# maschad/lodestar

Measured on AMD Instinct MI355X. Metric: BLS signature sets verified/sec (node), higher is better.
Workload: dtype u32; 1 GPU; C4 range-sync segment: 32 epochs = 1024 blocks x 98 sets (95 att k=128, sync k=512, 2 singles), 1M-validator table in HBM; sets=100352, pubkey_refs=12978176, table_validators=1048576, jobs=1024, inflight=3

## Files before the change

### include/bgv.h

```cpp
#ifndef BGV_H
#define BGV_H

#include <stdint.h>
#include <stddef.h>

#ifdef __cplusplus
extern "C" {
#endif

#define BGV_ABI_VERSION 4

enum bgv_status {
  BGV_OK = 0,
  BGV_E_INVALID_ARG = -1,
  BGV_E_HIP = -2,
  BGV_E_NO_DEVICE = -3,
  BGV_E_TABLE_RANGE = -4,
  BGV_E_EMPTY_SET = -5,
  BGV_E_BAD_PUBKEY = -6,
  BGV_E_STATE = -7,
};

enum bgv_set_code {
  BGV_SET_OK = 0,
// ... 123 lines not shown

typedef struct bgv_sm_agg {
  const uint8_t* take;
  const uint8_t* prev_sig96;
  uint8_t* agg_sig96;
  uint32_t* agg_count;
  int32_t* agg_code;
} bgv_sm_agg;
int bgv_verify_same_message_aggregate(bgv_ctx* ctx, const bgv_sm_batch* batch, const bgv_sm_agg* agg, uint8_t* set_valid,
                                      int32_t* set_code, bgv_sm_stats* stats);
int bgv_sm_agg_check(const bgv_sm_batch* batch, const bgv_sm_agg* agg);
int bgv_sm_agg_ms(bgv_ctx* ctx, float* ms);

typedef struct bgv_sma_batch {
  uint32_t n_sets;
  uint32_t n_groups;
  const uint32_t* group_offsets;
  const uint32_t* pk_offsets;
  const uint32_t* pk_indices;
  const uint8_t* raw_pks;
  uint32_t n_raw;
  const uint8_t* msgs;
  const uint8_t* sigs;
  const uint32_t* sig_len;
  const uint64_t* scalars;
  uint32_t on_device;
} bgv_sma_batch;

int bgv_verify_same_message_agg(bgv_ctx* ctx, const bgv_sma_batch* batch, uint8_t* set_valid, int32_t* set_code,
                                bgv_sm_stats* stats);
int bgv_sma_check(const bgv_sma_batch* batch);
int bgv_debug_same_message_agg(bgv_ctx* ctx, const bgv_sma_batch* batch, uint8_t* set_valid, int32_t* set_code,
                               bgv_sm_stats* stats, uint8_t* pk_set96, uint8_t* p_group96, uint8_t* s_group192,
                               uint8_t* h_group192);

#define BGV_MAX_INDEX_LISTS 8
int bgv_index_list_set(bgv_ctx* ctx, uint32_t list_id, const uint32_t* indices , uint32_t n);
int bgv_index_list_len(bgv_ctx* ctx, uint32_t list_id, uint32_t* n);

#define BGV_SRC_EXPLICIT 0xffffffffu
typedef struct bgv_set_src { uint32_t list, off, len, bits_off; } bgv_set_src;
typedef struct bgv_bits_batch {
  uint32_t n_sets, n_jobs;
  const uint32_t* job_offsets;
  const bgv_set_src* src;
  const uint8_t* bits;
  uint32_t bits_len;
  const uint32_t* pk_indices;
  uint32_t n_indices;
  const uint8_t* raw_pks;
  uint32_t n_raw;
  const uint8_t* msgs;
  const uint8_t* sigs;
  const uint32_t* sig_len;
  const uint64_t* scalars;
  uint32_t on_device;
} bgv_bits_batch;
int bgv_verify_bits(bgv_ctx* ctx, const bgv_bits_batch* batch, int32_t* job_result, int32_t* set_code, bgv_stats* stats);
int bgv_bits_check(const bgv_bits_batch* batch, const uint32_t* list_len );
int bgv_debug_bits_expand(bgv_ctx* ctx, const bgv_bits_batch* batch, uint32_t* pk_offsets ,
                          uint32_t* pk_indices, uint32_t cap, uint32_t* total);
int bgv_bits_expand_ms(bgv_ctx* ctx, float* ms);

int bgv_index_list_sums(bgv_ctx* ctx, uint32_t list_id, uint32_t enable);
int bgv_index_list_has_sums(bgv_ctx* ctx, uint32_t list_id, uint32_t* has);
int bgv_index_list_sums_ms(bgv_ctx* ctx, float* ms);
typedef struct bgv_bits_path {
  uint32_t sets_complement, keys_expanded, keys_gathered;
} bgv_bits_path;
int bgv_bits_path_stats(bgv_ctx* ctx, bgv_bits_path* out);
typedef struct bgv_hash_path {
  uint32_t sets, hashes, dedup;
} bgv_hash_path;
int bgv_hash_stats(bgv_ctx* ctx, bgv_hash_path* out);
typedef struct bgv_miller_path {
  uint32_t steps, slice_sets, items;
} bgv_miller_path;
int bgv_miller_path_stats(bgv_ctx* ctx, bgv_miller_path* out);
int bgv_pair_merge(bgv_ctx* ctx, int32_t mode);
typedef struct bgv_pair_path {
  uint32_t sets, pairs, merged, fallback;
} bgv_pair_path;
int bgv_pair_stats(bgv_ctx* ctx, bgv_pair_path* out);
int bgv_debug_pair_classes(bgv_ctx* ctx, const bgv_batch* batch, int32_t* job_result, int32_t* set_code, uint32_t* cls,
                           uint32_t* class_off, uint8_t* p_class96, uint8_t* job_fe, uint8_t* batch_fe);
int bgv_bits_plan(const bgv_bits_batch* batch, const uint32_t* list_len, const uint8_t* list_has_sums,
                  uint8_t* path , uint64_t* keys_gathered);
int bgv_debug_bits_keys(bgv_ctx* ctx, const bgv_bits_batch* batch, uint8_t* pk_agg96, uint8_t* path, int32_t* pk_code);
int bgv_debug_index_list_sums(bgv_ctx* ctx, uint32_t list_id, uint32_t first, uint32_t n, uint8_t* out96);

typedef struct bgv_smb_batch {
  uint32_t n_sets, n_groups;
  const uint32_t* group_offsets;
  const bgv_set_src* src;
  const uint8_t* bits;
  uint32_t bits_len;
  const uint32_t* pk_indices;
  uint32_t n_indices;
  const uint8_t* raw_pks;
  uint32_t n_raw;
  const uint8_t* msgs;
  const uint8_t* sigs;
  const uint32_t* sig_len;
  const uint64_t* scalars;
  uint32_t on_device;
} bgv_smb_batch;
int bgv_verify_same_message_bits(bgv_ctx* ctx, const bgv_smb_batch* batch, uint8_t* set_valid, int32_t* set_code,
                                 bgv_sm_stats* stats);
int bgv_smb_check(const bgv_smb_batch* batch, const uint32_t* list_len );
int bgv_debug_same_message_bits(bgv_ctx* ctx, const bgv_smb_batch* batch, uint8_t* set_valid, int32_t* set_code,
                                bgv_sm_stats* stats, uint8_t* pk_set96, uint8_t* path, uint8_t* p_group96,
                                uint8_t* s_group192, uint8_t* h_group192);

int bgv_partial(bgv_ctx* ctx, const bgv_batch* batch, uint8_t* miller576, int32_t* set_code, int32_t* job_result,
                int32_t* ok_out);
int bgv_partial_finish(bgv_ctx* ctx, int32_t* job_result, bgv_stats* stats);
int bgv_combine_final(bgv_ctx* ctx, const uint8_t* millers576, uint32_t n, int32_t* is_one);

typedef struct bgv_debug {
  uint8_t* sig_aff;
  uint8_t* h_aff;
  uint8_t* pk_agg;
  uint8_t* rpk_aff;
  uint8_t* s_aff;
  uint8_t* pair_fe;
  uint8_t* job_fe;
  uint8_t* batch_fe;
} bgv_debug;
int bgv_debug_stages(bgv_ctx* ctx, const bgv_batch* batch, int32_t* job_result, int32_t* set_code, bgv_debug* out);

int bgv_gen_keys(bgv_ctx* ctx, uint32_t first_index, uint32_t n, uint64_t seed);
int bgv_gen_sign(bgv_ctx* ctx, const bgv_batch* batch, uint8_t* sigs_out192);

#define BGV_FP_OPS_N 13
int bgv_debug_fp_ops(bgv_ctx* ctx, const uint32_t* ab_in, uint32_t n, uint32_t* out);
int bgv_debug_g2_decode(bgv_ctx* ctx, const uint8_t* sigs192, const uint32_t* sig_len, uint32_t n, uint8_t* out192,
                        int32_t* codes);

int bgv_bench_fpmul(bgv_ctx* ctx, uint32_t lanes, uint32_t iters, float* ms);
int bgv_bench_mad(bgv_ctx* ctx, uint32_t lanes, uint32_t iters, float* ms);

#ifdef __cplusplus
}
#endif
#endif
```

### lodestar_amd/csrc/bgv_api.hip

```cpp
#include <sys/random.h>
#include <string.h>
#include <stdio.h>
#include <stdarg.h>
#include <stdlib.h>
#include <atomic>
#include <chrono>
#include <optional>
#include <vector>
#include <string>

#include "bgv_internal.h"
#include "msm_g1.h"
#include "sig_agg.h"
#include "pair_merge.h"
#include "../../include/bgv.h"

using namespace bgv;

static thread_local std::string g_err;

static int fail(int code, const char* fmt, ...) {
  char buf[512];
  va_list ap;
  va_start(ap, fmt);
// ... 56 lines not shown
  uint8_t* pin_in = nullptr;
  uint8_t* pin_out = nullptr;
  size_t pin_in_cap = 0, pin_out_cap = 0;
  hipEvent_t ev_staged = nullptr;
  bool staged_pending = false;
  dbuf<uint8_t> raw_in, gen_out;
  dbuf<g1a> pk_tmp;
  dbuf<int32_t> pk_codes;
  std::vector<int32_t> pk_codes_host;
  std::vector<uint32_t> jo_host;
  uint32_t pk_total = 0;
  bool partial_pending = false;
  dev_batch part_d;
  dev_work part_w;
  dbuf<g1a> pk_agg;
  dbuf<fp12_t> dbg_fe, dbg_f;
  dbuf<uint8_t> dbg_out;
  dbuf<uint64_t> scalars;
  dbuf<g1a> raw_conv;
  dbuf<g2a> sig_aff, h_aff;
  dbuf<uint32_t> sig_inf, flags;
  dbuf<int32_t> sig_code, pk_code, job_code, job_result, set_code;
  dbuf<g1a> rpk_aff;
  dbuf<uint32_t> chunk_off, chunk_set;
  dbuf<g1j> pk_part;
  dbuf<g2j> rsig, q_part;
  dbuf<uint32_t> sig_grp;
  dbuf<fp2_t> lines;
  uint32_t lines_idle = 0;
  dbuf<fp12_t> f_step;
  bgv_miller_path miller_path = {};
  dbuf<fp12_t> f_set, f_job, f_batch, f_tmp, f_part;
  dbuf<uint32_t> set_job, s_inf, item_off, item_job;
  dbuf<g2a> s_aff;
  dbuf<g2j> msm_bucket, msm_win;
  dbuf<uint32_t> msm_mask;
  dbuf<uint32_t> sm_skip, sm_list;
  dbuf<int32_t> sm_zero, sm_seg_code;
  dbuf<g1j> sm_win;
  dbuf<g2a> sm_hg, sm_sg;
  dbuf<g1a> sm_pg;
  dbuf<uint8_t> sm_retry;
  dbuf<g1j> sma_pk;
  dbuf<int32_t> sma_pk_code;
  dbuf<g1a> sma_aff;
  dbuf<g2j> sag_seg;
  dbuf<uint32_t> sag_cnt;
  dbuf<int32_t> sag_code;
  dbuf<uint8_t> sag_out;
  dbuf<uint8_t> sag_valid;
  dbuf<g2a> sag_sig;
  hipEvent_t ev_sag[2] = {};
  bool sag_timed = false;
  uint32_t* idx_list[BGV_MAX_INDEX_LISTS] = {};
  uint32_t idx_list_n[BGV_MAX_INDEX_LISTS] = {};
  dbuf<uint32_t> bits_off, bits_idx;
  g1j* idx_sums[BGV_MAX_INDEX_LISTS] = {};
  float sums_build_ms = 0.f;
  uint32_t idx_list_max[BGV_MAX_INDEX_LISTS] = {};
  dbuf<pk_window> bits_win;
  bool bits_any_sums = false;
  bool bits_on_device = false;
  bgv_bits_path bits_path = {};
  uint32_t bits_n = 0;
  uint32_t bits_extra_chunks = 0;
  hipEvent_t ev_bits[2] = {};
  bool bits_timed = false;
  dbuf<uint32_t> msg_rep, msg_uniq, msg_tab, msg_cnt;
  msg_classes mc = {};
  bgv_hash_path hash_path = {};
  bool hash_pending = false;
  int32_t pair_merge = 0;
  bool pm_entry = false;
  bool pm_call = false;
  dbuf<uint64_t> pm_tab;
  dbuf<uint32_t> pm_slot, pm_slot_idx, pm_off, pm_cls, pm_head, pm_next, pm_job, pm_rep, pm_item_off, pm_item_job;
  dbuf<g1a> pm_p;
  dbuf<int32_t> pm_code;
  dbuf<g2a> pm_h;
  pair_classes pc = {};
  bgv_pair_path pair_path = {};
  bool pair_pending = false;
  bool pair_redo = false;
  dbuf<fp_t> mb_fp;
  dbuf<uint64_t> mb_u64;
};


int bgv_abi_version(void) { return BGV_ABI_VERSION; }
#ifndef BGV_SRC_HASH
#define BGV_SRC_HASH "unhashed"
#endif
const char* bgv_build_id(void) { return BGV_SRC_HASH; }
const char* bgv_last_error(void) { return g_err.c_str(); }

const char* bgv_set_code_name(int code) {
  switch (code) {
    case 0: return "BLST_SUCCESS";
    case 1: return "BLST_BAD_ENCODING";
    case 2: return "BLST_POINT_NOT_ON_CURVE";
    case 3: return "BLST_POINT_NOT_IN_GROUP";
    case 4: return "BLST_AGGR_TYPE_MISMATCH";
    case 5: return "BLST_VERIFY_FAIL";
    case 6: return "BLST_PK_IS_INFINITY";
    case 7: return "BLST_BAD_SCALAR";
    case 8: return "BLST_INVALID_SIZE";
    case 9: return "BGV_INDEX_RANGE";
    case 10: return "EMPTY_SIGNATURE_SET";
    default: return "BGV_UNKNOWN";
  }
}

const char* bgv_stage_name(int stage) {
  static const char* names[ST_COUNT] = {"sig_decode_subgroup", "hash_to_g2",       "pk_gather",
                                        "pk_aggregate_scale",  "sig_scale",        "sig_sum_tree",
                                        "miller_loop",         "miller_loop_jobs", "miller_product_tree",
                                        "batch_product",       "batch_final_exp",  "job_final_exp",
                                        "set_codes"};
  return (stage >= 0 && stage < ST_COUNT) ? names[stage] : "unknown";
}

void bgv_cfg_default(bgv_cfg* cfg) {
  if (!cfg) return;
  memset(cfg, 0, sizeof *cfg);
  cfg->struct_size = sizeof *cfg;
  cfg->split = cfg->miller = cfg->msm = cfg->prefold = cfg->lines = cfg->defer_pct = cfg->timing = cfg->clear_lanes = -1;
  cfg->miller_kv = cfg->hash_dedup = cfg->miller_steps = -1;
  cfg->job_lanes = cfg->pairs = cfg->cu_split = 0;
}

int bgv_open(int device, bgv_ctx** out) { return bgv_open_cfg(device, nullptr, out); }

int bgv_open_cfg(int device, const bgv_cfg* cfg, bgv_ctx** out) {
  if (!out) return fail(BGV_E_INVALID_ARG, "out is NULL");
  *out = nullptr;
  bgv_cfg k;
  bgv_cfg_default(&k);
  if (cfg) {
    if (cfg->struct_size != sizeof k) return fail(BGV_E_INVALID_ARG, "bgv_cfg.struct_size %u, expected %zu", cfg->struct_size, sizeof k);
    k = *cfg;
    auto lanes_ok = [](int v) { return v == 6 || v == 18 || v == 36; };
    if (k.miller != -1 && k.miller != 1 && k.miller != 2 && k.miller != 4 && !lanes_ok(k.miller)) return fail(BGV_E_INVALID_ARG, "bgv_cfg.miller %d", k.miller);
    if (k.job_lanes != 0 && !lanes_ok(k.job_lanes)) return fail(BGV_E_INVALID_ARG, "bgv_cfg.job_lanes %d", k.job_lanes);
    if (k.pairs < 0 || k.pairs == 3 || k.pairs > 4) return fail(BGV_E_INVALID_ARG, "bgv_cfg.pairs %d", k.pairs);
    if (k.msm < -1 || k.msm > 4) return fail(BGV_E_INVALID_ARG, "bgv_cfg.msm %d", k.msm);
    if (k.clear_lanes != -1 && k.clear_lanes != 1 && k.clear_lanes != 3 && k.clear_lanes != 9)
      return fail(BGV_E_INVALID_ARG, "bgv_cfg.clear_lanes %d", k.clear_lanes);
    if (k.miller_kv != -1 && k.miller_kv != 0 && k.miller_kv != 2 && k.miller_kv != 3 && k.miller_kv != 6 && k.miller_kv != 9)
      return fail(BGV_E_INVALID_ARG, "bgv_cfg.miller_kv %d", k.miller_kv);
    if (k.defer_pct < -1 || k.defer_pct > 100) return fail(BGV_E_INVALID_ARG, "bgv_cfg.defer_pct %d", k.defer_pct);
    auto tri_ok = [](int v) { return v >= -1 && v <= 1; };
    if (!tri_ok(k.split)) return fail(BGV_E_INVALID_ARG, "bgv_cfg.split %d", k.split);
    if (!tri_ok(k.prefold)) return fail(BGV_E_INVALID_ARG, "bgv_cfg.prefold %d", k.prefold);
    if (!tri_ok(k.lines)) return fail(BGV_E_INVALID_ARG, "bgv_cfg.lines %d", k.lines);
    if (!tri_ok(k.timing)) return fail(BGV_E_INVALID_ARG, "bgv_cfg.timing %d", k.timing);
    if (!tri_ok(k.hash_dedup)) return fail(BGV_E_INVALID_ARG, "bgv_cfg.hash_dedup %d", k.hash_dedup);
    if (!tri_ok(k.miller_steps)) return fail(BGV_E_INVALID_ARG, "bgv_cfg.miller_steps %d", k.miller_steps);
    if (k.cu_split < -64 || k.cu_split > 64) return fail(BGV_E_INVALID_ARG, "bgv_cfg.cu_split %d (|N| <= 64 CUs)", k.cu_split);
    if (k.pairs >= 2 && k.miller != -1 && k.miller != 1)
      return fail(BGV_E_INVALID_ARG, "bgv_cfg.pairs 2 needs the one-lane Miller loop (miller %d)", k.miller);
  }
  int n = 0;
  if (hipGetDeviceCount(&n) != hipSuccess || n <= 0) return fail(BGV_E_NO_DEVICE, "no HIP device visible");
  if (device < 0 || device >= n) return fail(BGV_E_NO_DEVICE, "device %d out of range (%d devices)", device, n);
  HIPCHK(hipSetDevice(device));
  std::vector<uint32_t> mask;
// ... 15 lines not shown
    }
  }
  bgv_ctx* c = new bgv_ctx();
  c->device = device;
  c->cfg = k;
  struct guard_t {
    bgv_ctx*& c;
    ~guard_t() { if (c) bgv_close(c); }
  } guard{c};
  int prio_lo = 0, prio_hi = 0;
  HIPCHK(hipDeviceGetStreamPriorityRange(&prio_lo, &prio_hi));
  if (k.cu_split == 0) {
    HIPCHK(hipStreamCreateWithPriority(&c->st, hipStreamNonBlocking, prio_lo));
    HIPCHK(hipStreamCreateWithPriority(&c->st_hash, hipStreamNonBlocking, prio_hi));
    HIPCHK(hipStreamCreateWithPriority(&c->st_pk, hipStreamNonBlocking, prio_hi));
    HIPCHK(hipStreamCreateWithPriority(&c->st_chk, hipStreamNonBlocking, prio_lo));
  } else {
    hipStream_t* sts[4] = {&c->st, &c->st_hash, &c->st_pk, &c->st_chk};
    for (hipStream_t* p : sts) HIPCHK(hipExtStreamCreateWithCUMask(p, (uint32_t)mask.size(), mask.data()));
  }
  for (auto& e : c->ev) HIPCHK(hipEventCreate(&e));
  for (auto& e : c->ev_end) HIPCHK(hipEventCreate(&e));
  HIPCHK(hipEventCreate(&c->ev_fork));
  HIPCHK(hipEventCreateWithFlags(&c->ev_staged, hipEventDisableTiming));
  for (auto& e : c->ev_dep) HIPCHK(hipEventCreateWithFlags(&e, hipEventDisableTiming));
  HIPCHK(hipEventCreateWithFlags(&c->ev_prep, hipEventDisableTiming));
  HIPCHK(hipEventCreateWithFlags(&c->ev_sigdec, hipEventDisableTiming));
  HIPCHK(hipEventCreateWithFlags(&c->ev_grp, hipEventDisableTiming));
  HIPCHK(hipEventCreateWithFlags(&c->ev_maps, hipEventDisableTiming));
  HIPCHK(hipEventCreateWithFlags(&c->ev_chk, hipEventDisableTiming));
  for (auto& e : c->ev_bits) HIPCHK(hipEventCreate(&e));
  for (auto& e : c->ev_sag) HIPCHK(hipEventCreate(&e));
  *out = c;
  c = nullptr;
  return BGV_OK;
}

int bgv_close(bgv_ctx* c) {
  if (!c) return BGV_OK;
  (void)hipSetDevice(c->device);
  (void)hipStreamSynchronize(c->st);
  (void)hipStreamSynchronize(c->st_hash);
  (void)hipStreamSynchronize(c->st_pk);
  (void)hipStreamSynchronize(c->st_chk);
  for (auto& e : c->ev) (void)hipEventDestroy(e);
  for (auto& e : c->ev_end) (void)hipEventDestroy(e);
  (void)hipEventDestroy(c->ev_fork);
  (void)hipEventDestroy(c->ev_staged);
  for (auto& e : c->ev_dep) (void)hipEventDestroy(e);
  (void)hipEventDestroy(c->ev_prep);
  (void)hipEventDestroy(c->ev_sigdec);
  (void)hipEventDestroy(c->ev_grp);
  (void)hipEventDestroy(c->ev_maps);
  (void)hipEventDestroy(c->ev_chk);
  for (auto& e : c->ev_bits) (void)hipEventDestroy(e);
  for (auto& e : c->ev_sag) (void)hipEventDestroy(e);
  for (auto& l : c->idx_list)
    if (l) (void)hipFree(l);
  for (auto& l : c->idx_sums)
    if (l) (void)hipFree(l);
  c->bits_off.release(); c->bits_idx.release(); c->bits_win.release();
  c->msg_rep.release(); c->msg_uniq.release(); c->msg_tab.release(); c->msg_cnt.release();
  c->pm_tab.release(); c->pm_slot.release(); c->pm_slot_idx.release(); c->pm_off.release(); c->pm_cls.release();
  c->pm_head.release(); c->pm_next.release(); c->pm_job.release(); c->pm_rep.release(); c->pm_item_off.release();
  c->pm_item_job.release(); c->pm_p.release(); c->pm_code.release(); c->pm_h.release();
  if (c->pin_in) (void)hipHostFree(c->pin_in);
  if (c->pin_out) (void)hipHostFree(c->pin_out);
  if (c->table) (void)hipFree(c->table);
  c->sk.release();
  c->stage_dev.release();
  c->raw_in.release(); c->gen_out.release(); c->pk_tmp.release(); c->pk_codes.release();
  c->pk_agg.release(); c->dbg_fe.release(); c->dbg_f.release(); c->dbg_out.release();
  c->scalars.release(); c->raw_conv.release();
  c->sig_aff.release(); c->h_aff.release(); c->sig_inf.release(); c->flags.release();
  c->sig_code.release(); c->pk_code.release(); c->job_code.release(); c->job_result.release(); c->set_code.release();
  c->rpk_aff.release(); c->chunk_off.release(); c->chunk_set.release(); c->pk_part.release(); c->rsig.release(); c->q_part.release(); c->sig_grp.release(); c->lines.release(); c->f_step.release(); c->f_set.release(); c->f_job.release(); c->f_batch.release(); c->f_tmp.release(); c->f_part.release();
  c->msm_bucket.release(); c->msm_win.release(); c->msm_mask.release();
  c->set_job.release(); c->s_inf.release(); c->item_off.release(); c->item_job.release(); c->s_aff.release();
  c->sm_skip.release(); c->sm_list.release(); c->sm_zero.release(); c->sm_seg_code.release(); c->sm_win.release();
  c->sm_hg.release(); c->sm_sg.release(); c->sm_pg.release(); c->sm_retry.release();
  c->sma_pk.release(); c->sma_pk_code.release(); c->sma_aff.release();
  c->sag_seg.release(); c->sag_cnt.release(); c->sag_code.release(); c->sag_out.release(); c->sag_valid.release();
  c->sag_sig.release();
  c->mb_fp.release(); c->mb_u64.release();
  (void)hipStreamDestroy(c->st);
  (void)hipStreamDestroy(c->st_hash);
  (void)hipStreamDestroy(c->st_pk);
  (void)hipStreamDestroy(c->st_chk);
  delete c;
  return BGV_OK;
}

static int ctx_drain(bgv_ctx* c) {
  HIPCHK(hipStreamSynchronize(c->st));
  HIPCHK(hipStreamSynchronize(c->st_hash));
  HIPCHK(hipStreamSynchronize(c->st_pk));
  HIPCHK(hipStreamSynchronize(c->st_chk));
  return 0;
}

static int sums_drop(bgv_ctx* c, uint32_t id) {
  if (!c->idx_sums[id]) return 0;
  if (int r = ctx_drain(c)) return r;
  (void)hipFree(c->idx_sums[id]);
  c->idx_sums[id] = nullptr;
  return 0;
}
static int sums_drop_all(bgv_ctx* c) {
  for (uint32_t k = 0; k < BGV_MAX_INDEX_LISTS; k++)
    if (int r = sums_drop(c, k)) return r;
  return 0;
}

static int table_reserve(bgv_ctx* c, uint32_t n) {
  if (n <= c->table_cap) return 0;
  uint32_t cap = c->table_cap ? c->table_cap : 1024;
  while (cap < n) cap = cap * 2u > cap ? cap * 2u : n;
  g1a* t = nullptr;
  HIPCHK(hipMalloc((void**)&t, (size_t)cap * sizeof(g1a)));
  HIPCHK(hipMemsetAsync(t, 0, (size_t)cap * sizeof(g1a), c->st));
  if (c->table) {
    HIPCHK(hipMemcpyAsync(t, c->table, (size_t)c->table_n * sizeof(g1a), hipMemcpyDeviceToDevice, c->st));
    HIPCHK(hipStreamSynchronize(c->st));
    HIPCHK(hipFree(c->table));
  }
  c->table = t;
  c->table_cap = cap;
  return 0;
}

static const uint32_t TABLE_MAX = 0x7fffffffu;

int bgv_pubkeys_set(bgv_ctx* c, uint32_t first, uint32_t n, const uint8_t* data, uint32_t fmt) {
  if (!c || (!data && n)) return fail(BGV_E_INVALID_ARG, "null argument");
  if (fmt != BGV_PK_COMPRESSED_48 && fmt != BGV_PK_UNCOMPRESSED_96) return fail(BGV_E_INVALID_ARG, "bad format %u", fmt);
  c->partial_pending = false;
  if (n == 0) return BGV_OK;
  if ((uint64_t)first + n > TABLE_MAX) return fail(BGV_E_TABLE_RANGE, "rows [%u, %llu) exceed the table limit 2^31 - 1", first, (unsigned long long)first + n);
  if (first > c->table_n)
    return fail(BGV_E_TABLE_RANGE, "row %u would leave a gap after the %u rows of the table (append-only, pubkeyCache.ts:56-77)", first, c->table_n);
  HIPCHK(hipSetDevice(c->device));
  if (int r = table_reserve(c, first + n)) return r;
  const size_t w = fmt == BGV_PK_COMPRESSED_48 ? 48 : 96;
  if (int r = c->raw_in.ensure((size_t)n * w)) return r;
  if (int r = c->pk_tmp.ensure(n)) return r;
  if (int r = c->pk_codes.ensure(n)) return r;
  HIPCHK(hipMemcpyAsync(c->raw_in.p, data, (size_t)n * w, hipMemcpyHostToDevice, c->st));
  if (fmt == BGV_PK_COMPRESSED_48) launch_table_from_compressed(c->st, c->raw_in.p, c->pk_tmp.p, n, c->pk_codes.p);
  else launch_table_from_uncompressed(c->st, c->raw_in.p, c->pk_tmp.p, n, c->pk_codes.p);
  HIPCHK(hipGetLastError());
  c->pk_codes_host.resize(n);
  HIPCHK(hipMemcpyAsync(c->pk_codes_host.data(), c->pk_codes.p, (size_t)n * 4, hipMemcpyDeviceToHost, c->st));
  HIPCHK(hipStreamSynchronize(c->st));
  for (uint32_t i = 0; i < n; i++)
    if (c->pk_codes_host[i] != 0)
      return fail(BGV_E_BAD_PUBKEY, "pubkey %u: BLST_ERROR: %s", first + i, bgv_set_code_name(c->pk_codes_host[i]));
  if (first < c->table_n)
    if (int r = sums_drop_all(c)) return r;
  HIPCHK(hipMemcpyAsync(c->table + first, c->pk_tmp.p, (size_t)n * sizeof(g1a), hipMemcpyDeviceToDevice, c->st));
  HIPCHK(hipStreamSynchronize(c->st));
  if (first + n > c->table_n) c->table_n = first + n;
  return BGV_OK;
}

int bgv_pubkeys_count(bgv_ctx* c, uint32_t* count) {
  if (!c || !count) return fail(BGV_E_INVALID_ARG, "null argument");
// ... 244 lines not shown
    d.prefold_log2 = on ? (d.span_log2 + 1) / 2 : 0u;
  }
  d.miller_coop = k.miller >= 0 ? (k.miller == 1 ? 0u : (uint32_t)k.miller)
                                : (n < MILLER18_MIN ? 36u : n < MILLER4_MIN ? 18u : n < MILLER2_MIN ? 4u
                                   : n < MILLER1_MIN ? 2u : 0u);
  {
    const uint32_t auto_kv = n >= KV6_MIN && n < KV3_MIN ? 6u : (n >= KV3_MIN && n < KV_MAX ? 3u : 0u);
    d.miller_kv = k.miller_kv >= 0 ? (uint32_t)k.miller_kv : auto_kv;
    if (!d.split) d.miller_kv = 0;
    if (d.miller_kv) d.pairs_per_item = 2;
    else if (d.miller_coop) d.pairs_per_item = 1;
  }
  d.job_lanes = k.job_lanes ? (uint32_t)k.job_lanes : 36u;
  if (scalars_staged) {
  } else if (scalars) {
    d.scalars = scalars;
  } else {
    uint32_t kn[11];
    random_bytes(kn, sizeof kn);
    if (int r = ensure_or_release_lines(c, c->scalars, n ? n : 1)) return r;
    launch_gen_scalars(c->st, kn, kn + 8, c->scalars.p, n);
    HIPCHK(hipGetLastError());
    d.scalars = c->scalars.p;
  }
  d.lines = (uint32_t)(!d.split && !d.miller_coop && (k.lines >= 0 ? k.lines : d.pairs_per_item >= 2));
  if (d.lines) {
    const size_t need = (size_t)3 * MILLER_STEPS * n * sizeof(fp2_t);
    size_t free_b = 0, total_b = 0;
    if (need > c->lines.cap * sizeof(fp2_t) &&
        (hipMemGetInfo(&free_b, &total_b) != hipSuccess || need > free_b / 4))
      d.lines = 0;
  }
  if (d.pairs_per_item == 4 && !d.lines) d.pairs_per_item = 2;
  {
    const bool can = !d.split && !d.miller_coop && !d.miller_kv && d.lines;
    const bool want = k.miller_steps >= 0 ? k.miller_steps != 0 : (k.pairs == 0 && d.pairs_per_item >= 2 && d.span_log2 <= 8);
    d.steps_slice = can && want ? STEPS_SLICE : 0u;
    if (d.steps_slice) {
      const size_t need = (size_t)miller_items_bound(d, d.steps_slice) * MILLER_STEPS * sizeof(fp12_t);
      size_t free_b = 0, total_b = 0;
      if (need > c->f_step.cap * sizeof(fp12_t) && (hipMemGetInfo(&free_b, &total_b) != hipSuccess || need > free_b / 4))
        d.steps_slice = 0;
    }
    const uint32_t per = d.steps_slice ? d.steps_slice : (d.miller_coop && !d.miller_kv ? 0u : d.pairs_per_item);
    uint32_t items = 0;
    if (per && c->jo_host.size() == (size_t)d.n_jobs + 1)
      for (uint32_t j = 0; j < d.n_jobs; j++) items += miller_item_count(c->jo_host[j + 1] - c->jo_host[j], per);
    c->miller_path = {d.steps_slice ? 1u : 0u, per, items};
  }
  return 0;
}

static int work_alloc_once(bgv_ctx* c, const dev_batch& d, dev_work& w);

static bool pair_merge_on(const bgv_ctx* c, const dev_batch& d) {
  return c->pm_call && !d.split && !d.miller_coop && !d.miller_kv && !d.steps_dbg && d.pairs_per_item >= 1 && d.n_jobs > 0 &&
         d.n_sets > 0 && d.n_sets <= (1u << 30);
}
static bool hash_dedup_on(const bgv_ctx* c, const dev_batch& d) {
  return !d.split && (c->cfg.hash_dedup == 1 || pair_merge_on(c, d)) && d.n_sets > 0 && d.n_sets <= (1u << 30);
}

static int work_alloc(bgv_ctx* c, const dev_batch& d, dev_work& w) {
  int r = work_alloc_once(c, d, w);
  if (r && !d.lines && c->lines.cap) {
    c->lines.release();
    c->f_step.release();
    c->lines_idle = 0;
    r = work_alloc_once(c, d, w);
  }
  return r;
}

static int work_alloc_once(bgv_ctx* c, const dev_batch& d, dev_work& w) {
  const uint32_t n = d.n_sets, J = d.n_jobs;
  const size_t ns = n ? n : 1, nj = J ? J : 1;
  int r = 0;
  if ((r = c->chunk_off.ensure(ns + 1)) || (r = c->chunk_set.ensure((size_t)d.chunk_bound + 1)) ||
      (r = c->pk_part.ensure((size_t)d.chunk_bound + 1)))
    return r;
  w.chunk_off = c->chunk_off.p; w.chunk_set = c->chunk_set.p; w.pk_part = c->pk_part.p;
  if ((r = c->sig_aff.ensure(ns)) || (r = c->h_aff.ensure(ns)) || (r = c->sig_inf.ensure(ns)) ||
      (r = c->sig_code.ensure(ns)) || (r = c->pk_code.ensure(ns)) || (r = c->rpk_aff.ensure(ns)) ||
      (r = c->rsig.ensure(ns)) || (r = c->f_set.ensure(ns + nj)) || (r = c->set_code.ensure(ns)) ||
      (r = c->set_job.ensure(ns)) || (r = c->item_off.ensure(nj + 1)) || (r = c->item_job.ensure(ns + nj + 1)) || (r = c->f_job.ensure(nj)) || (r = c->f_batch.ensure(nj)) || (r = c->f_tmp.ensure(nj / 8 + 1)) ||
      (r = c->s_aff.ensure(nj)) || (r = c->s_inf.ensure(nj)) || (r = c->job_code.ensure(nj)) ||
      (r = c->job_result.ensure(nj)) || (r = c->f_part.ensure(4)) || (r = c->flags.ensure(8)))
    return r;
  w.sig_aff = c->sig_aff.p; w.h_aff = c->h_aff.p; w.sig_inf = c->sig_inf.p; w.sig_code = c->sig_code.p;
  w.pk_code = c->pk_code.p; w.rpk_aff = c->rpk_aff.p; w.rsig = c->rsig.p; w.f_set = c->f_set.p;
  w.set_code = c->set_code.p; w.f_job = c->f_job.p; w.job_code = c->job_code.p; w.job_result = c->job_result.p;
  w.f_part = c->f_part.p; w.flags = c->flags.p;
  w.item_off = c->item_off.p; w.item_job = c->item_job.p;
  w.set_job = c->set_job.p; w.f_batch = c->f_batch.p; w.f_tmp = c->f_tmp.p; w.s_aff = c->s_aff.p; w.s_inf = c->s_inf.p;
  w.q_part = nullptr; w.sig_grp = nullptr; w.pk_agg = nullptr;
  if (d.split) {
    if ((r = c->q_part.ensure(2 * ns)) || (r = c->sig_grp.ensure(ns))) return r;
    w.q_part = c->q_part.p; w.sig_grp = c->sig_grp.p;
  } else if (d.defer_grp) {
    if ((r = c->sig_grp.ensure(ns))) return r;
    w.sig_grp = c->sig_grp.p;
  }
  static const uint32_t LINES_KEEP = 64;
  w.lines = nullptr;
  if (d.lines) {
    c->lines_idle = 0;
    if ((r = c->lines.ensure((size_t)3 * MILLER_STEPS * ns))) return r;
    w.lines = c->lines.p;
  } else if ((c->lines.cap || c->f_step.cap) && ++c->lines_idle >= LINES_KEEP) {
    c->lines.release();
    c->f_step.release();
    c->lines_idle = 0;
  }
  w.f_step = nullptr;
  if (d.steps_slice) {
    if ((r = c->f_step.ensure((size_t)miller_items_bound(d, d.steps_slice) * MILLER_STEPS))) return r;
    w.f_step = c->f_step.p;
  }
  c->mc = {};
  if (hash_dedup_on(c, d)) {
    size_t slots = 64;
    while (slots < 2 * ns) slots *= 2;
    if ((r = c->msg_rep.ensure(ns)) || (r = c->msg_uniq.ensure(ns)) || (r = c->msg_tab.ensure(slots)) || (r = c->msg_cnt.ensure(1)))
      return r;
    c->mc.n_sets = n;
    c->mc.mask = (uint32_t)(slots - 1);
    c->mc.msgs = d.msgs;
    c->mc.table = c->msg_tab.p; c->mc.rep = c->msg_rep.p; c->mc.uniq = c->msg_uniq.p; c->mc.n_uniq = c->msg_cnt.p;
    c->mc.h_aff = w.h_aff;
  }
  c->pc = {};
  if (pair_merge_on(c, d)) {
    size_t slots = 64;
    while (slots < 2 * ns) slots *= 2;
    if ((r = c->pm_tab.ensure(slots)) || (r = c->pm_slot_idx.ensure(slots)) || (r = c->pm_slot.ensure(ns)) ||
        (r = c->pm_off.ensure(nj + 1)) || (r = c->pm_cls.ensure(ns)) || (r = c->pm_head.ensure(ns)) ||
        (r = c->pm_next.ensure(ns)) || (r = c->pm_job.ensure(ns)) || (r = c->pm_rep.ensure(ns)) ||
        (r = c->pm_item_off.ensure(nj + 1)) || (r = c->pm_item_job.ensure(ns + nj + 1)) || (r = c->pm_p.ensure(ns)) ||
        (r = c->pm_code.ensure(ns)) || (r = c->pm_h.ensure(ns)))
      return r;
    pair_classes& p = c->pc;
    p.n_sets = n; p.n_jobs = J;
    p.mask = (uint32_t)(slots - 1);
    p.per = d.steps_slice ? d.steps_slice : d.pairs_per_item;
    p.job_off = d.job_off; p.rep = c->msg_rep.p;
    p.table = c->pm_tab.p; p.slot = c->pm_slot.p; p.slot_idx = c->pm_slot_idx.p; p.class_off = c->pm_off.p;
    p.cls = c->pm_cls.p; p.head = c->pm_head.p; p.next = c->pm_next.p; p.cls_job = c->pm_job.p; p.cls_rep = c->pm_rep.p;
    p.item_off = c->pm_item_off.p; p.item_job = c->pm_item_job.p;
    p.p_cls = c->pm_p.p; p.code_cls = c->pm_code.p; p.h_cls = c->pm_h.p;
    p.ident = c->flags.p + 1;
  }
  w.msm_bucket = nullptr; w.msm_mask = nullptr; w.msm_win = nullptr;
  if (d.msm == 2) {
    if ((r = c->msm_bucket.ensure(nj * 16 * 15)) || (r = c->msm_mask.ensure(nj * 16)) || (r = c->msm_win.ensure(nj * 16))) return r;
    w.msm_bucket = c->msm_bucket.p; w.msm_mask = c->msm_mask.p; w.msm_win = c->msm_win.p;
  } else if (d.msm == 4) {
    if ((r = c->msm_win.ensure(nj * 16))) return r;
    w.msm_win = c->msm_win.p;
  }
  return 0;
}

static int run_stages(bgv_ctx* c, const dev_batch& d, const dev_work& w, int from, int to) {
  const bool fork = from <= ST_SIG && to > ST_F_TREE;
  const bool timed = c->cfg.timing >= 0 ? c->cfg.timing != 0 : d.n_sets >= 65536;
  c->timed = timed;
  c->last_d = d;
  c->run_from = from;
  c->run_to = to;
  hipEvent_t* dep = timed ? c->ev_end : c->ev_dep;
  if (!timed && !(d.maps_early && from == 0)) HIPCHK(hipEventRecord(c->ev[from], c->st));
  const bool early_hash = fork && d.split && from <= ST_HASH && to > ST_HASH;
  const bool hashes = from <= ST_HASH && to > ST_HASH;
  const bool classes = hashes && c->mc.n_sets == d.n_sets && hash_dedup_on(c, d);
  if (hashes) {
    c->hash_path = {d.n_sets, d.n_sets, classes ? 1u : 0u};
    c->hash_pending = classes;
  }
  const bool merge = fork && from == 0 && classes && c->pc.n_sets == d.n_sets && pair_merge_on(c, d);
  dev_batch dv = d;
  dev_work wv = w;
  if (merge) {
    dv.job_off = c->pc.class_off;
    wv.rpk_aff = c->pc.p_cls; wv.pk_code = c->pc.code_cls; wv.h_aff = c->pc.h_cls;
    wv.set_job = c->pc.cls_job; wv.item_off = c->pc.item_off; wv.item_job = c->pc.item_job;
  }
  if (c->pm_entry && from <= ST_MILLER && to > ST_MILLER) {
    c->pair_path = {d.n_sets, d.n_sets, merge ? 1u : 0u, 0u};
    c->pair_pending = merge;
    c->pair_redo = false;
  }
  auto launch_one = [&](int s) -> int {
    hipStream_t st = c->st;
    if (s == ST_MILLER && d.lines) {
      if (merge) launch_pair_lines(fork ? c->st_hash : c->st, c->pc, w.lines);
      else launch_lines(fork ? c->st_hash : c->st, d, w);
      HIPCHK(hipGetLastError());
    }
    if (fork) {
      if (s == ST_HASH || s == ST_MILLER) st = c->st_hash;
      if (s == ST_PK || s == ST_PK_SCALE) st = c->st_pk;
      if (s == ST_S_TREE || s == ST_MILLER) HIPCHK(hipStreamWaitEvent(st, dep[ST_PK_SCALE], 0));
      if (s == ST_F_TREE) HIPCHK(hipStreamWaitEvent(st, dep[ST_MILLER], 0));
    }
    if (s == ST_HASH && d.maps_early && st != c->st_hash) HIPCHK(hipStreamWaitEvent(st, c->ev_maps, 0));
    if (timed) HIPCHK(hipEventRecord(c->ev[s], st));
    if (s == ST_F_TREE && d.defer_grp) {
      if (fork) HIPCHK(hipStreamWaitEvent(st, c->ev_grp, 0));
      launch_sig_fixup(st, d, w);
    }
    if (s == ST_HASH && classes) launch_hash_classes(st, c->mc);
    else if (merge && (s == ST_MILLER || s == ST_F_TREE)) launch_stage(st, s, dv, wv);
    else launch_stage(st, s, d, w);
    if (merge && s == ST_HASH) launch_pair_h(st, c->pc, w.h_aff);
    if (merge && s == ST_PK_SCALE) launch_pair_sum(st, c->pc, w.rpk_aff, w.pk_code);
    HIPCHK(hipGetLastError());
    if (timed) HIPCHK(hipEventRecord(c->ev_end[s], st));
    else if (fork && (s == ST_PK_SCALE || s == ST_HASH || s == ST_MILLER)) HIPCHK(hipEventRecord(c->ev_dep[s], st));
    if (d.defer_grp && s == ST_SIG && fork) HIPCHK(hipEventRecord(c->ev_sigdec, st));
    if (d.defer_grp && s == ST_PK_SCALE) {
      hipStream_t cs = st;
      if (fork && BGV_CHK_STREAM && d.split) {
        HIPCHK(hipEventRecord(c->ev_chk, st));
        cs = c->st_chk;
        HIPCHK(hipStreamWaitEvent(cs, c->ev_chk, 0));
      }
      if (fork) HIPCHK(hipStreamWaitEvent(cs, c->ev_sigdec, 0));
      launch_sig_check(cs, d, w);
      HIPCHK(hipGetLastError());
      if (fork) HIPCHK(hipEventRecord(c->ev_grp, cs));
    }
    return 0;
  };
  if (early_hash) {
    HIPCHK(hipEventRecord(c->ev_fork, c->st));
    HIPCHK(hipStreamWaitEvent(c->st_hash, c->ev_fork, 0));
    if (int r = launch_one(ST_HASH)) return r;
  }
  if (from <= ST_PK) {
    launch_prep(c->st, d, w);
    HIPCHK(hipGetLastError());
  }
  if (classes) {
    random_bytes(&c->mc.key, sizeof c->mc.key);
    HIPCHK(hipMemsetAsync(c->mc.table, 0xff, ((size_t)c->mc.mask + 1) * 4, c->st));
    HIPCHK(hipMemsetAsync(c->mc.n_uniq, 0, 4, c->st));
    launch_msg_dedup(c->st, c->mc);
    HIPCHK(hipGetLastError());
  }
  if (merge) {
    const pair_classes& p = c->pc;
    random_bytes(&c->pc.key, sizeof c->pc.key);
    HIPCHK(hipMemsetAsync(p.table, 0xff, ((size_t)p.mask + 1) * 8, c->st));
    HIPCHK(hipMemsetAsync(p.head, 0xff, (size_t)p.n_sets * 4, c->st));
    HIPCHK(hipMemsetAsync(p.class_off, 0, ((size_t)p.n_jobs + 1) * 4, c->st));
    HIPCHK(hipMemsetAsync(p.cls_job, 0, (size_t)p.n_sets * 4, c->st));
    HIPCHK(hipMemsetAsync(p.ident, 0, 4, c->st));
    launch_pair_classes(c->st, c->pc);
    HIPCHK(hipGetLastError());
  }
  if (fork) {
    HIPCHK(hipEventRecord(c->ev_prep, c->st));
    if (!early_hash) HIPCHK(hipStreamWaitEvent(c->st_hash, c->ev_prep, 0));
    HIPCHK(hipStreamWaitEvent(c->st_pk, c->ev_prep, 0));
  }
  for (int s = from; s < to; s++)
    if (!(early_hash && s == ST_HASH))
      if (int r = launch_one(s)) return r;
  HIPCHK(hipEventRecord(c->ev[to], c->st));
  return 0;
}

static void stats_layout(bgv_stats* s, const dev_batch& d) {
  s->split = d.split;
  s->miller_lanes = d.miller_coop ? d.miller_coop : 1u;
  s->pairs_per_item = d.pairs_per_item;
  s->msm = d.msm;
  s->lines = d.lines;
  s->defer_from = d.defer_grp ? d.defer_from : d.n_sets;
  s->clear_lanes = d.clear_lanes;
  s->miller_kv = d.miller_kv;
}

static int finish_results(bgv_ctx* c, const dev_batch& d, const dev_work& w, int32_t* job_result, int32_t* set_code,
                          bgv_stats* stats) {
  const size_t jr_off = 256, sc_off = jr_off + (((size_t)d.n_jobs * 4 + 255) & ~size_t(255));
  const bool want_sc = set_code && d.n_sets;
  if (int r = pinned_reserve(c->pin_out, c->pin_out_cap, sc_off + (want_sc ? (size_t)d.n_sets * 4 : 0))) return r;
  if (d.n_jobs) HIPCHK(hipMemcpyAsync(c->pin_out + jr_off, w.job_result, (size_t)d.n_jobs * 4, hipMemcpyDeviceToHost, c->st));
  if (want_sc) HIPCHK(hipMemcpyAsync(c->pin_out + sc_off, w.set_code, (size_t)d.n_sets * 4, hipMemcpyDeviceToHost, c->st));
  HIPCHK(hipMemcpyAsync(c->pin_out, w.flags, 4, hipMemcpyDeviceToHost, c->st));
  const bool want_uniq = c->hash_pending;
  if (want_uniq) HIPCHK(hipMemcpyAsync(c->pin_out + 64, c->mc.n_uniq, 4, hipMemcpyDeviceToHost, c->st));
  const bool want_pair = c->pair_pending;
  if (want_pair) {
    HIPCHK(hipMemcpyAsync(c->pin_out + 68, c->pc.class_off + c->pc.n_jobs, 4, hipMemcpyDeviceToHost, c->st));
    HIPCHK(hipMemcpyAsync(c->pin_out + 72, c->pc.ident, 4, hipMemcpyDeviceToHost, c->st));
  }
  HIPCHK(hipStreamSynchronize(c->st));
  c->staged_pending = false;
  uint32_t flag = 0;
  memcpy(&flag, c->pin_out, 4);
  if (want_pair) {
    uint32_t ident = 0;
    memcpy(&c->pair_path.pairs, c->pin_out + 68, 4);
    memcpy(&ident, c->pin_out + 72, 4);
    c->pair_redo = ident != 0;
    c->pair_pending = false;
  }
  if (want_uniq) {
    memcpy(&c->hash_path.hashes, c->pin_out + 64, 4);
    c->hash_pending = false;
  }
  if (d.n_jobs) memcpy(job_result, c->pin_out + jr_off, (size_t)d.n_jobs * 4);
  if (want_sc) memcpy(set_code, c->pin_out + sc_off, (size_t)d.n_sets * 4);
  if (stats) {
    memset(stats, 0, sizeof *stats);
    if (c->timed)
      for (int s = 0; s < ST_COUNT && s < BGV_N_STAGES; s++) HIPCHK(hipEventElapsedTime(&stats->stage_ms[s], c->ev[s], c->ev_end[s]));
    HIPCHK(hipEventElapsedTime(&stats->total_ms, c->ev[0], c->ev[ST_COUNT]));
    stats->n_sets = d.n_sets;
    stats->n_jobs = d.n_jobs;
    stats_layout(stats, d);
    uint32_t valid_jobs = 0, valid_sets = 0;
    const uint32_t* jo = c->jo_host.data();
    for (uint32_t j = 0; j < d.n_jobs; j++)
      if (job_result[j] >= 0) { valid_jobs++; valid_sets += jo[j + 1] - jo[j]; }
    stats->pubkeys_aggregated = c->pk_total;
    stats->batch_retries = (valid_jobs && !flag) ? 1u : 0u;
    stats->batch_sigs_success = flag ? valid_sets : 0u;
  }
  return 0;
}

int bgv_last_stats(bgv_ctx* c, bgv_stats* stats) {
  if (!c || !stats) return fail(BGV_E_INVALID_ARG, "null argument");
  memset(stats, 0, sizeof *stats);
  if (c->run_to <= c->run_from) return BGV_OK;
  HIPCHK(hipSetDevice(c->device));
  HIPCHK(hipEventSynchronize(c->ev[c->run_to]));
  if (c->timed)
    for (int s = c->run_from; s < c->run_to && s < BGV_N_STAGES; s++) HIPCHK(hipEventElapsedTime(&stats->stage_ms[s], c->ev[s], c->ev_end[s]));
  HIPCHK(hipEventElapsedTime(&stats->total_ms, c->ev[c->run_from], c->ev[c->run_to]));
  stats_layout(stats, c->last_d);
  return BGV_OK;
}

struct pair_entry {
  bgv_ctx* c;
  pair_entry(bgv_ctx* c_, bool may_merge) : c(c_) {
    c->pm_entry = true;
    c->pm_call = may_merge;
    c->pair_path = {};
    c->pair_pending = c->pair_redo = false;
  }
  ~pair_entry() { c->pm_entry = c->pm_call = false; }
};

static int run_and_finish(bgv_ctx* c, const dev_batch& d, const dev_work& w, int32_t* job_result, int32_t* set_code,
                          bgv_stats* stats) {
  if (int r = run_stages(c, d, w, 0, ST_COUNT)) return r;
  if (int r = finish_results(c, d, w, job_result, set_code, stats)) return r;
  if (!c->pair_redo) return 0;
  c->pm_call = false;
  if (int r = run_stages(c, d, w, 0, ST_COUNT)) return r;
  if (int r = finish_results(c, d, w, job_result, set_code, stats)) return r;
  c->pair_path.fallback = 1;
  return 0;
}

int bgv_verify(bgv_ctx* c, const bgv_batch* b, int32_t* job_result, int32_t* set_code, bgv_stats* stats) {
  if (!c || !b || (!job_result && b->n_jobs)) return fail(BGV_E_INVALID_ARG, "null argument");
  c->partial_pending = false;
  HIPCHK(hipSetDevice(c->device));
  active_guard ag(c->device);
  pair_entry pe(c, c->pair_merge != 0);
  dev_batch d;
  if (int r = prepare(c, b, d, true)) return r;
  dev_work w;
  if (int r = work_alloc(c, d, w)) return r;
  return run_and_finish(c, d, w, job_result, set_code, stats);
}

int bgv_pair_merge(bgv_ctx* c, int32_t mode) {
  if (!c) return fail(BGV_E_INVALID_ARG, "null ctx");
  if (mode != 0 && mode != 1) return fail(BGV_E_INVALID_ARG, "bgv_pair_merge mode %d", mode);
  c->pair_merge = mode;
  return BGV_OK;
}

int bgv_pair_stats(bgv_ctx* c, bgv_pair_path* out) {
  if (!c || !out) return fail(BGV_E_INVALID_ARG, "null argument");
  if (c->pair_pending) {
    HIPCHK(hipSetDevice(c->device));
    HIPCHK(hipMemcpyAsync(&c->pair_path.pairs, c->pc.class_off + c->pc.n_jobs, 4, hipMemcpyDeviceToHost, c->st));
    HIPCHK(hipStreamSynchronize(c->st));
    c->pair_pending = false;
  }
  *out = c->pair_path;
  return BGV_OK;
}

static_assert(sizeof(bgv_set_src) == sizeof(bits_src) && BGV_MAX_INDEX_LISTS == BITS_MAX_LISTS &&
                  BGV_SRC_EXPLICIT == BITS_SRC_EXPLICIT,
              "bits_expand.h mirrors include/bgv.h");

int bgv_index_list_set(bgv_ctx* c, uint32_t id, const uint32_t* idx, uint32_t n) {
  if (!c || (!idx && n)) return fail(BGV_E_INVALID_ARG, "null argument");
  if (id >= BGV_MAX_INDEX_LISTS) return fail(BGV_E_INVALID_ARG, "index list %u: ids are below %u", id, (unsigned)BGV_MAX_INDEX_LISTS);
  for (uint32_t i = 0; i < n; i++)
    if (idx[i] & 0x80000000u)
      return fail(BGV_E_INVALID_ARG, "index list %u: entry %u (0x%08x) has bit 31 set (lists hold table rows only)", id, i, idx[i]);
  HIPCHK(hipSetDevice(c->device));
  uint32_t* p = nullptr;
  if (n) {
    if (hipMalloc((void**)&p, (size_t)n * 4) != hipSuccess) return fail(BGV_E_HIP, "hipMalloc(%zu) failed", (size_t)n * 4);
    hipError_t e = hipMemcpyAsync(p, idx, (size_t)n * 4, hipMemcpyHostToDevice, c->st);
    if (e == hipSuccess) e = hipStreamSynchronize(c->st);
    if (e != hipSuccess) {
      (void)hipFree(p);
      return fail(BGV_E_HIP, "index list %u upload: %s", id, hipGetErrorString(e));
    }
  }
  if (c->idx_list[id]) {
    if (int r = ctx_drain(c)) { if (p) (void)hipFree(p); return r; }
    (void)hipFree(c->idx_list[id]);
    if (c->idx_sums[id]) (void)hipFree(c->idx_sums[id]);
    c->idx_sums[id] = nullptr;
  }
  c->idx_list[id] = p;
  c->idx_list_n[id] = n;
  uint32_t mx = 0;
  for (uint32_t i = 0; i < n; i++) mx = idx[i] > mx ? idx[i] : mx;
  c->idx_list_max[id] = mx;
  return BGV_OK;
}

int bgv_index_list_sums(bgv_ctx* c, uint32_t id, uint32_t enable) {
  if (!c) return fail(BGV_E_INVALID_ARG, "null argument");
  if (id >= BGV_MAX_INDEX_LISTS) return fail(BGV_E_INVALID_ARG, "index list %u: ids are below %u", id, (unsigned)BGV_MAX_INDEX_LISTS);
  HIPCHK(hipSetDevice(c->device));
  if (!enable) return sums_drop(c, id);
  if (!c->idx_list[id]) return fail(BGV_E_INVALID_ARG, "index list %u is not set", id);
  const uint32_t n = c->idx_list_n[id];
  if (c->idx_list_max[id] >= c->table_n)
    return fail(BGV_E_TABLE_RANGE, "index list %u holds row %u, the table has %u rows: a prefix over a row that does not exist cannot be built",
                id, c->idx_list_max[id], c->table_n);
  if (int r = sums_drop(c, id)) return r;
  g1j *S = nullptr, *tmp = nullptr;
  const size_t entries = (size_t)n + 1, n_tmp = sums_tmp_entries(n);
  if (hipMalloc((void**)&S, entries * sizeof(g1j)) != hipSuccess) return fail(BGV_E_HIP, "hipMalloc(%zu) failed", entries * sizeof(g1j));
  if (hipMalloc((void**)&tmp, n_tmp * sizeof(g1j)) != hipSuccess) {
    (void)hipFree(S);
    return fail(BGV_E_HIP, "hipMalloc(%zu) failed", n_tmp * sizeof(g1j));
  }
  c->bits_timed = false;
  c->sums_build_ms = 0.f;
  (void)hipEventRecord(c->ev_bits[0], c->st);
  launch_list_sums(c->st, c->table, c->table_n, c->idx_list[id], n, S, tmp);
  hipError_t e = hipGetLastError();
  (void)hipEventRecord(c->ev_bits[1], c->st);
  if (e == hipSuccess) e = hipStreamSynchronize(c->st);
  if (e == hipSuccess) (void)hipEventElapsedTime(&c->sums_build_ms, c->ev_bits[0], c->ev_bits[1]);
  (void)hipFree(tmp);
  if (e != hipSuccess) {
    (void)hipFree(S);
    return fail(BGV_E_HIP, "index list %u sums: %s", id, hipGetErrorString(e));
  }
  c->idx_sums[id] = S;
  return BGV_OK;
// ... 232 lines not shown
    launch_raw_pks(c->st, raw_dev, c->raw_conv.p, b->n_raw);
    d.raw_pks = c->raw_conv.p;
    if (c->bits_timed) HIPCHK(hipEventRecord(c->ev_bits[0], c->st));
    bits_launch_count(c->st, a);
    if (int r = bits_launch_expand(c, c->st, a, total)) return r;
    if (c->bits_timed) HIPCHK(hipEventRecord(c->ev_bits[1], c->st));
  } else {
    d.job_off = b->job_offsets;
    a.src = (const bits_src*)b->src;
    a.v.bits = b->bits;
    a.v.pk_indices = b->pk_indices;
    d.msgs = b->msgs; d.sigs = b->sigs; d.sig_len = b->sig_len;
    if (need_sigs)
      if (int r = early_maps(c, d, false)) return r;
    if (int r = ensure_or_release_lines(c, c->raw_conv, b->n_raw ? b->n_raw : 1)) return r;
    launch_raw_pks(c->st, b->raw_pks, c->raw_conv.p, b->n_raw);
    d.raw_pks = c->raw_conv.p;
    if (c->bits_timed) HIPCHK(hipEventRecord(c->ev_bits[0], c->st));
    bits_launch_count(c->st, a);
    HIPCHK(hipGetLastError());
    HIPCHK(hipMemcpyAsync(c->jo_host.data(), b->job_offsets, c->jo_host.size() * 4, hipMemcpyDeviceToHost, c->st));
    if (int r = bits_read_totals(c, c->st, a)) return r;
    if (int r = bits_launch_expand(c, c->st, a, c->bits_path.keys_gathered)) return r;
    if (c->bits_timed) HIPCHK(hipEventRecord(c->ev_bits[1], c->st));
  }
  HIPCHK(hipGetLastError());
  d.pk_off = c->bits_off.p;
  d.pk_idx = c->bits_idx.p;
  return 0;
}

static int bits_layout(bgv_ctx* c, dev_batch& d, const uint64_t* scalars, bool scalars_staged) {
  if (int r = prepare_layout(c, d, scalars, scalars_staged)) return r;
  if (d.win) d.chunk_bound = c->bits_path.keys_gathered / PK_CHUNK + d.n_sets + c->bits_extra_chunks;
  return 0;
}

int bgv_bits_path_stats(bgv_ctx* c, bgv_bits_path* out) {
  if (!c || !out) return fail(BGV_E_INVALID_ARG, "null argument");
  if (c->bits_any_sums && c->bits_on_device) {
    HIPCHK(hipSetDevice(c->device));
    HIPCHK(hipMemcpyAsync(&c->bits_path.sets_complement, c->bits_off.p + c->bits_n + 2, 4, hipMemcpyDeviceToHost, c->st));
    HIPCHK(hipStreamSynchronize(c->st));
  }
  *out = c->bits_path;
  return BGV_OK;
}

static void hash_path_clear(bgv_ctx* c) {
  if (!c) return;
  c->hash_path = {};
  c->hash_pending = false;
  c->pair_path = {};
  c->pair_pending = c->pair_redo = false;
}

int bgv_hash_stats(bgv_ctx* c, bgv_hash_path* out) {
  if (!c || !out) return fail(BGV_E_INVALID_ARG, "null argument");
  if (c->hash_pending) {
    HIPCHK(hipSetDevice(c->device));
    HIPCHK(hipMemcpyAsync(&c->hash_path.hashes, c->mc.n_uniq, 4, hipMemcpyDeviceToHost, c->st));
    HIPCHK(hipStreamSynchronize(c->st));
    c->hash_pending = false;
  }
  *out = c->hash_path;
  return BGV_OK;
}

int bgv_miller_path_stats(bgv_ctx* c, bgv_miller_path* out) {
  if (!c || !out) return fail(BGV_E_INVALID_ARG, "null argument");
  *out = c->miller_path;
  return BGV_OK;
}

int bgv_verify_bits(bgv_ctx* c, const bgv_bits_batch* b, int32_t* job_result, int32_t* set_code, bgv_stats* stats) {
  if (!c || !b || (!job_result && b->n_jobs)) return fail(BGV_E_INVALID_ARG, "null argument");
  c->partial_pending = false;
  HIPCHK(hipSetDevice(c->device));
  active_guard ag(c->device);
  pair_entry pe(c, c->pair_merge != 0);
  dev_batch d;
  if (int r = bits_front(c, b, d, true)) return r;
  if (int r = bits_layout(c, d, b->scalars, b->scalars && !b->on_device)) return r;
  dev_work w;
  if (int r = work_alloc(c, d, w)) return r;
  return run_and_finish(c, d, w, job_result, set_code, stats);
}

int bgv_bits_expand_ms(bgv_ctx* c, float* ms) {
  if (!c || !ms) return fail(BGV_E_INVALID_ARG, "null argument");
  *ms = 0.f;
  if (!c->bits_timed) return BGV_OK;
  HIPCHK(hipSetDevice(c->device));
  HIPCHK(hipEventSynchronize(c->ev_bits[1]));
  HIPCHK(hipEventElapsedTime(ms, c->ev_bits[0], c->ev_bits[1]));
  return BGV_OK;
}

int bgv_debug_bits_expand(bgv_ctx* c, const bgv_bits_batch* b, uint32_t* pk_offsets, uint32_t* pk_indices, uint32_t cap,
                          uint32_t* total) {
  if (!c || !b || !pk_offsets || !total || (!pk_indices && cap)) return fail(BGV_E_INVALID_ARG, "null argument");
  c->partial_pending = false;
  HIPCHK(hipSetDevice(c->device));
  dev_batch d;
  if (int r = bits_front(c, b, d, false, false)) return r;
  HIPCHK(hipMemcpyAsync(pk_offsets, d.pk_off, ((size_t)b->n_sets + 1) * 4, hipMemcpyDeviceToHost, c->st));
  const uint32_t t = c->pk_total;
  if (t && t <= cap) HIPCHK(hipMemcpyAsync(pk_indices, d.pk_idx, (size_t)t * 4, hipMemcpyDeviceToHost, c->st));
  HIPCHK(hipStreamSynchronize(c->st));
  c->staged_pending = false;
  *total = t;
  if (t > cap) return fail(BGV_E_INVALID_ARG, "the expansion holds %u indices, pk_indices has room for %u", t, cap);
  return BGV_OK;
}

int bgv_debug_bits_keys(bgv_ctx* c, const bgv_bits_batch* b, uint8_t* pk_agg96, uint8_t* path, int32_t* pk_code) {
  if (!c || !b) return fail(BGV_E_INVALID_ARG, "null argument");
  c->partial_pending = false;
  HIPCHK(hipSetDevice(c->device));
  dev_batch d;
  if (int r = bits_front(c, b, d, false)) return r;
  if (int r = bits_layout(c, d, nullptr, false)) return r;
  dev_work w;
  if (int r = work_alloc(c, d, w)) return r;
  const uint32_t n = d.n_sets;
  if (int r = c->pk_agg.ensure(n ? n : 1)) return r;
  w.pk_agg = c->pk_agg.p;
  if (int r = run_stages(c, d, w, ST_PK, ST_PK_SCALE + 1)) return r;
  if (int r = c->dbg_out.ensure((size_t)n * 96 + 1)) return r;
  launch_export_g1a(c->st, w.pk_agg, c->dbg_out.p, n);
  HIPCHK(hipGetLastError());
  std::vector<pk_window> win(d.win ? n : 0);
  if (n && pk_agg96) HIPCHK(hipMemcpyAsync(pk_agg96, c->dbg_out.p, (size_t)n * 96, hipMemcpyDeviceToHost, c->st));
  if (n && pk_code) HIPCHK(hipMemcpyAsync(pk_code, w.pk_code, (size_t)n * 4, hipMemcpyDeviceToHost, c->st));
  if (n && d.win) HIPCHK(hipMemcpyAsync(win.data(), d.win, (size_t)n * sizeof(pk_window), hipMemcpyDeviceToHost, c->st));
  HIPCHK(hipStreamSynchronize(c->st));
  c->staged_pending = false;
  if (path)
    for (uint32_t i = 0; i < n; i++) path[i] = d.win && win[i].hi ? 1 : 0;
  return BGV_OK;
}


template <class B>
static int sm_check_counts(const B* b) {
  if (!b) return fail(BGV_E_INVALID_ARG, "batch is NULL");
  if (b->n_sets == 0 && b->n_groups == 0) return BGV_OK;
  if (b->n_groups > b->n_sets) return fail(BGV_E_INVALID_ARG, "n_groups %u > n_sets %u (a group is never empty)", b->n_groups, b->n_sets);
  if (b->n_groups == 0) return fail(BGV_E_INVALID_ARG, "n_sets %u without a group", b->n_sets);
  return BGV_OK;
}

static int sm_check_groups(uint32_t n, uint32_t G, const uint32_t* go) {
  if (go[0] != 0 || go[G] != n) return fail(BGV_E_INVALID_ARG, "group_offsets must span [0, n_sets]");
  for (uint32_t g = 0; g < G; g++) {
    if (go[g + 1] < go[g]) return fail(BGV_E_INVALID_ARG, "group_offsets not monotone");
    if (go[g + 1] == go[g]) return fail(BGV_E_INVALID_ARG, "group %u is empty", g);
  }
  return BGV_OK;
}

static int scalars_nonzero(const uint64_t* sc, uint32_t n) {
  if (sc)
    for (uint32_t i = 0; i < n; i++)
      if (!sc[i]) return fail(BGV_E_INVALID_ARG, "scalars[%u] is zero", i);
  return BGV_OK;
// ... 551 lines not shown
  hash_path_clear(c);
  return r;
}

int bgv_verify_same_message(bgv_ctx* c, const bgv_sm_batch* b, uint8_t* set_valid, int32_t* set_code, bgv_sm_stats* stats) {
  return sm_done(c, sm_run(c, b, set_valid, set_code, stats, nullptr, nullptr, nullptr));
}

static int sm_agg_args(const bgv_sm_agg* agg) {
  if (!agg) return fail(BGV_E_INVALID_ARG, "agg is NULL");
  if (!agg->agg_sig96) return fail(BGV_E_INVALID_ARG, "agg_sig96 is NULL");
  return BGV_OK;
}

int bgv_sm_agg_check(const bgv_sm_batch* b, const bgv_sm_agg* agg) {
  if (int r = bgv_sm_check(b)) return r;
  return sm_agg_args(agg);
}

int bgv_verify_same_message_aggregate(bgv_ctx* c, const bgv_sm_batch* b, const bgv_sm_agg* agg, uint8_t* set_valid,
                                      int32_t* set_code, bgv_sm_stats* stats) {
  if (int r = sm_agg_args(agg)) return r;
  if (!c) return fail(BGV_E_INVALID_ARG, "null ctx");
  return sm_done(c, sm_run(c, b, set_valid, set_code, stats, nullptr, nullptr, nullptr, agg));
}

int bgv_sm_agg_ms(bgv_ctx* c, float* ms) {
  if (!c || !ms) return fail(BGV_E_INVALID_ARG, "null argument");
  *ms = 0.f;
  if (!c->sag_timed) return BGV_OK;
  HIPCHK(hipSetDevice(c->device));
  HIPCHK(hipEventSynchronize(c->ev_sag[1]));
  HIPCHK(hipEventElapsedTime(ms, c->ev_sag[0], c->ev_sag[1]));
  return BGV_OK;
}

int bgv_debug_same_message(bgv_ctx* c, const bgv_sm_batch* b, uint8_t* set_valid, int32_t* set_code, bgv_sm_stats* stats,
                           uint8_t* p_group96, uint8_t* s_group192, uint8_t* h_group192) {
  return sm_done(c, sm_run(c, b, set_valid, set_code, stats, p_group96, s_group192, h_group192));
}

int bgv_verify_same_message_agg(bgv_ctx* c, const bgv_sma_batch* b, uint8_t* set_valid, int32_t* set_code, bgv_sm_stats* stats) {
  return sm_done(c, sma_run(c, b, set_valid, set_code, stats, nullptr, nullptr, nullptr, nullptr));
}

int bgv_debug_same_message_agg(bgv_ctx* c, const bgv_sma_batch* b, uint8_t* set_valid, int32_t* set_code, bgv_sm_stats* stats,
                               uint8_t* pk_set96, uint8_t* p_group96, uint8_t* s_group192, uint8_t* h_group192) {
  return sm_done(c, sma_run(c, b, set_valid, set_code, stats, pk_set96, p_group96, s_group192, h_group192));
}

int bgv_verify_same_message_bits(bgv_ctx* c, const bgv_smb_batch* b, uint8_t* set_valid, int32_t* set_code, bgv_sm_stats* stats) {
  return sm_done(c, smb_run(c, b, set_valid, set_code, stats, nullptr, nullptr, nullptr, nullptr, nullptr));
}

int bgv_debug_same_message_bits(bgv_ctx* c, const bgv_smb_batch* b, uint8_t* set_valid, int32_t* set_code, bgv_sm_stats* stats,
                                uint8_t* pk_set96, uint8_t* path, uint8_t* p_group96, uint8_t* s_group192, uint8_t* h_group192) {
  return sm_done(c, smb_run(c, b, set_valid, set_code, stats, pk_set96, path, p_group96, s_group192, h_group192));
}

static void fp12_plain_to_bytes(uint8_t* out, const fp12_t& f) {
  const fp2_t* cs[6] = {&f.c0.c0, &f.c1.c0, &f.c0.c1, &f.c1.c1, &f.c0.c2, &f.c1.c2};
  for (int k = 0; k < 6; k++) {
    fp_to_be48(out + 96 * k, cs[k]->c0);
    fp_to_be48(out + 96 * k + 48, cs[k]->c1);
  }
}

static void fp12_plain_from_bytes(fp12_t& f, const uint8_t* in) {
  fp2_t* cs[6] = {&f.c0.c0, &f.c1.c0, &f.c0.c1, &f.c1.c1, &f.c0.c2, &f.c1.c2};
  for (int k = 0; k < 6; k++) {
    fp_from_be48(cs[k]->c0, in + 96 * k);
    fp_from_be48(cs[k]->c1, in + 96 * k + 48);
  }
}

int bgv_partial(bgv_ctx* c, const bgv_batch* b, uint8_t* miller576, int32_t* set_code, int32_t* job_result,
                int32_t* ok_out) {
  if (!c || !b || !miller576) return fail(BGV_E_INVALID_ARG, "null argument");
  c->partial_pending = false;
  HIPCHK(hipSetDevice(c->device));
  active_guard ag(c->device);
  dev_batch d;
  if (int r = prepare(c, b, d, true)) return r;
  dev_work w;
  pair_entry pe(c, c->pair_merge != 0);
  if (int r = work_alloc(c, d, w)) return r;
  fp12_t f;
  std::vector<int32_t> jc(d.n_jobs ? d.n_jobs : 1);
  bool fell_back = false;
  for (int pass = 0; pass < 2; pass++) {
    if (int r = run_stages(c, d, w, ST_SIG, ST_BATCH_FINAL)) return r;
    launch_stage(c->st, ST_SET_CODES, d, w);
    if (d.n_jobs) {
      launch_fp12_convert(c->st, w.f_batch, w.f_part, 1, false);
      HIPCHK(hipGetLastError());
      HIPCHK(hipMemcpyAsync(&f, w.f_part, sizeof f, hipMemcpyDeviceToHost, c->st));
    } else {
      memset(&f, 0, sizeof f);
      f.c0.c0.c0.l[0] = 1;
    }
    if (d.n_jobs) HIPCHK(hipMemcpyAsync(jc.data(), w.job_code, (size_t)d.n_jobs * 4, hipMemcpyDeviceToHost, c->st));
    if (set_code && d.n_sets) HIPCHK(hipMemcpyAsync(set_code, w.set_code, (size_t)d.n_sets * 4, hipMemcpyDeviceToHost, c->st));
    if (c->hash_pending) HIPCHK(hipMemcpyAsync(&c->hash_path.hashes, c->mc.n_uniq, 4, hipMemcpyDeviceToHost, c->st));
    uint32_t ident = 0;
    const bool want_pair = c->pair_pending;
    if (want_pair) {
      HIPCHK(hipMemcpyAsync(&c->pair_path.pairs, c->pc.class_off + c->pc.n_jobs, 4, hipMemcpyDeviceToHost, c->st));
      HIPCHK(hipMemcpyAsync(&ident, c->pc.ident, 4, hipMemcpyDeviceToHost, c->st));
    }
    HIPCHK(hipStreamSynchronize(c->st));
    c->hash_pending = false;
    c->pair_pending = false;
    c->staged_pending = false;
    if (!(want_pair && ident)) break;
    c->pm_call = false;
    fell_back = true;
  }
  if (fell_back) c->pair_path.fallback = 1;
  fp12_plain_to_bytes(miller576, f);
  int32_t ok = 1;
  for (uint32_t j = 0; j < d.n_jobs; j++) {
    if (jc[j] != 0) ok = 0;
    if (job_result) job_result[j] = jc[j] != 0 ? -jc[j] : 1;
  }
  if (ok_out) *ok_out = ok;
  c->part_d = d;
  c->part_w = w;
  c->partial_pending = true;
  return BGV_OK;
}

int bgv_partial_finish(bgv_ctx* c, int32_t* job_result, bgv_stats* stats) {
  if (!c) return fail(BGV_E_INVALID_ARG, "null ctx");
  if (!c->partial_pending) return fail(BGV_E_STATE, "bgv_partial_finish needs bgv_partial as the previous call on the context");
  const dev_batch& d = c->part_d;
  const dev_work& w = c->part_w;
  if (!job_result && d.n_jobs) return fail(BGV_E_INVALID_ARG, "null argument");
  c->partial_pending = false;
  HIPCHK(hipSetDevice(c->device));
  c->timed = false;
  c->run_from = 0;
  c->run_to = ST_COUNT;
  HIPCHK(hipEventRecord(c->ev[0], c->st));
  launch_stage(c->st, ST_BATCH_FINAL, d, w);
  launch_stage(c->st, ST_JOB_FINAL, d, w);
  HIPCHK(hipGetLastError());
  HIPCHK(hipEventRecord(c->ev[ST_COUNT], c->st));
  return finish_results(c, d, w, job_result, nullptr, stats);
}

int bgv_combine_final(bgv_ctx* c, const uint8_t* parts, uint32_t n, int32_t* is_one) {
  if (!c || (!parts && n) || !is_one) return fail(BGV_E_INVALID_ARG, "null argument");
  HIPCHK(hipSetDevice(c->device));
  std::vector<fp12_t> h(n ? n : 1);
  for (uint32_t k = 0; k < n; k++) fp12_plain_from_bytes(h[k], parts + 576u * k);
  if (int r = c->f_part.ensure(2 * (size_t)n + 65)) return r;
  if (int r = c->flags.ensure(8)) return r;
  if (n) HIPCHK(hipMemcpyAsync(c->f_part.p + n, h.data(), (size_t)n * sizeof(fp12_t), hipMemcpyHostToDevice, c->st));
  launch_fp12_convert(c->st, c->f_part.p + n, c->f_part.p, n, true);
  launch_combine_final(c->st, c->f_part.p, n, c->flags.p + 4);
  HIPCHK(hipGetLastError());
  uint32_t flag = 0;
  HIPCHK(hipMemcpyAsync(&flag, c->flags.p + 4, 4, hipMemcpyDeviceToHost, c->st));
  HIPCHK(hipStreamSynchronize(c->st));
  *is_one = flag ? 1 : 0;
  return BGV_OK;
}

int bgv_debug_stages(bgv_ctx* c, const bgv_batch* b, int32_t* job_result, int32_t* set_code, bgv_debug* o) {
  if (!c || !b || !o || (!job_result && b->n_jobs)) return fail(BGV_E_INVALID_ARG, "null argument");
  c->partial_pending = false;
  c->pair_path = {};
  c->pair_pending = c->pair_redo = false;
  HIPCHK(hipSetDevice(c->device));
  dev_batch d;
  if (int r = prepare(c, b, d, true)) return r;
  dev_work w;
  if (int r = work_alloc(c, d, w)) return r;
  const uint32_t n = d.n_sets, J = d.n_jobs;
  if (int r = c->pk_agg.ensure(n ? n : 1)) return r;
  w.pk_agg = c->pk_agg.p;
  d.steps_dbg = d.steps_slice ? 1u : 0u;
  if (int r = run_stages(c, d, w, 0, ST_F_TREE)) return r;
  if (d.defer_grp) launch_sig_fixup(c->st, d, w);
  if (int r = c->dbg_f.ensure((size_t)n + J + 1)) return r;
  if (n + J) HIPCHK(hipMemcpyAsync(c->dbg_f.p, w.f_set, (size_t)(n + J) * sizeof(fp12_t), hipMemcpyDeviceToDevice, c->st));
  if (int r = run_stages(c, d, w, ST_F_TREE, ST_COUNT)) return r;
  if (d.steps_dbg && n) HIPCHK(hipMemcpyAsync(c->dbg_f.p, w.f_set, (size_t)n * sizeof(fp12_t), hipMemcpyDeviceToDevice, c->st));
  const uint32_t n_fe = n + 2 * J + 1;
  if (int r = c->dbg_fe.ensure(n_fe)) return r;
  launch_final_exp_many(c->st, c->dbg_f.p, c->dbg_fe.p, n + J);
  launch_final_exp_many(c->st, w.f_job, c->dbg_fe.p + n + J, J);
  if (J) launch_final_exp_many(c->st, w.f_batch, c->dbg_fe.p + n + 2 * J, 1);
  launch_fp12_convert(c->st, c->dbg_fe.p, c->dbg_fe.p, n_fe, false);
  HIPCHK(hipGetLastError());
  struct part { uint8_t* host; size_t bytes; } parts[8];
  int np = 0;
  size_t off = 0;
  auto add = [&](uint8_t* host, size_t bytes) -> uint8_t* {
    const size_t o2 = off;
    off += (bytes + 255) & ~size_t(255);
    parts[np++] = {host, bytes};
    return (uint8_t*)o2;
  };
  uint8_t* o_sig = add(o->sig_aff, (size_t)n * 192);
  uint8_t* o_h = add(o->h_aff, (size_t)n * 192);
  uint8_t* o_pk = add(o->pk_agg, (size_t)n * 96);
  uint8_t* o_rpk = add(o->rpk_aff, (size_t)n * 96);
  uint8_t* o_s = add(o->s_aff, (size_t)J * 192);
  if (int r = c->dbg_out.ensure(off ? off : 1)) return r;
  uint8_t* base = c->dbg_out.p;
  launch_export_g2a(c->st, w.sig_aff, base + (size_t)o_sig, n);
  launch_export_g2a(c->st, w.h_aff, base + (size_t)o_h, n);
  launch_export_g1a(c->st, w.pk_agg, base + (size_t)o_pk, n);
  launch_export_g1a(c->st, w.rpk_aff, base + (size_t)o_rpk, n);
  launch_export_g2a(c->st, w.s_aff, base + (size_t)o_s, J);
  HIPCHK(hipGetLastError());
  size_t pos = 0;
  for (int k = 0; k < np; k++) {
    if (parts[k].host && parts[k].bytes) HIPCHK(hipMemcpyAsync(parts[k].host, base + pos, parts[k].bytes, hipMemcpyDeviceToHost, c->st));
    pos += (parts[k].bytes + 255) & ~size_t(255);
  }
  std::vector<fp12_t> fe(n_fe);
  HIPCHK(hipMemcpyAsync(fe.data(), c->dbg_fe.p, (size_t)n_fe * sizeof(fp12_t), hipMemcpyDeviceToHost, c->st));
  if (int r = finish_results(c, d, w, job_result, set_code, nullptr)) return r;
  if (o->pair_fe)
    for (uint32_t k = 0; k < n + J; k++) fp12_plain_to_bytes(o->pair_fe + 576u * k, fe[k]);
// ... 184 lines not shown
```

### lodestar_amd/csrc/bgv_internal.h

```cpp
#pragma once
#include "pairing.h"
#include "rng.h"
#include "bits_expand.h"

namespace bgv {

enum : int32_t {
  C_INDEX_RANGE = 9,
  C_EMPTY_JOB = 10,
};

struct pk_window {
  const g1j* lo;
  const g1j* hi;
};

struct dev_batch {
  uint32_t n_sets, n_jobs, n_raw, table_n;
  uint32_t span_log2;
  uint32_t chunk_bound;
  uint32_t miller_coop;
  uint32_t job_lanes;
  uint32_t pairs_per_item;
  uint32_t msm;
  uint32_t split;
  uint32_t clear_lanes;
  uint32_t miller_kv;
  uint32_t maps_early;
  uint32_t prefold_log2;
  uint32_t lines;
  uint32_t defer_from;
  uint32_t defer_grp;
  uint32_t steps_slice;
  uint32_t steps_dbg;
  const uint32_t* job_off;
  const uint32_t* pk_off;
  const uint32_t* pk_idx;
  const g1a* raw_pks;
  const g1a* table;
  const uint8_t* msgs;
  const uint8_t* sigs;
  const uint32_t* sig_len;
  const uint64_t* scalars;
  const pk_window* win;
};

struct dev_work {
  g2a* sig_aff;
  uint32_t* sig_inf;
  int32_t* sig_code;
  g2a* h_aff;
  g2j* q_part;
  uint32_t* sig_grp;
  g2j* msm_bucket;
  uint32_t* msm_mask;
  g2j* msm_win;
  uint32_t* chunk_off;
  uint32_t* chunk_set;
  g1j* pk_part;
  g1a* rpk_aff;
  g1a* pk_agg;
  int32_t* pk_code;
  g2j* rsig;
  uint32_t* set_job;
  uint32_t* item_off;
  uint32_t* item_job;
  g2a* s_aff;
  uint32_t* s_inf;
  fp2_t* lines;
  fp12_t* f_step;
  fp12_t* f_set;
  fp12_t* f_job;
  fp12_t* f_batch;
  fp12_t* f_tmp;
  int32_t* job_code;
  int32_t* job_result;
  int32_t* set_code;
  fp12_t* f_part;
  uint32_t* flags;
};

enum Stage {
  ST_SIG = 0,
  ST_HASH,
  ST_PK,
  ST_PK_SCALE,
  ST_SIG_SCALE,
  ST_S_TREE,
  ST_MILLER,
  ST_MILLER_JOBS,
  ST_F_TREE,
  ST_BATCH_PROD,
  ST_BATCH_FINAL,
  ST_JOB_FINAL,
  ST_SET_CODES,
  ST_COUNT
};

#ifdef __HIPCC__
BGV_HD bool g1a_is_zero(const g1a& p) { return fp_is_zero(p.x) && fp_is_zero(p.y); }

__device__ __forceinline__ void load_pk(g1a& out, const dev_batch& b, uint32_t idx, bool& range_err) {
  if (idx & 0x80000000u) {
    const uint32_t r = idx & 0x7fffffffu;
    if (r >= b.n_raw) { range_err = true; fp_set_zero(out.x); fp_set_zero(out.y); return; }
    out = b.raw_pks[r];
  } else {
    if (idx >= b.table_n) { range_err = true; fp_set_zero(out.x); fp_set_zero(out.y); return; }
    out = b.table[idx];
  }
}
#endif

constexpr uint32_t PK_CHUNK = 32;

void launch_pk_gather(hipStream_t st, const dev_batch& b, const dev_work& w);
void launch_raw_pks(hipStream_t st, const uint8_t* raw, g1a* out, uint32_t n);
void launch_table_from_compressed(hipStream_t st, const uint8_t* in, g1a* out, uint32_t n, int32_t* codes);
void launch_table_from_uncompressed(hipStream_t st, const uint8_t* in, g1a* out, uint32_t n, int32_t* codes);
void launch_table_export(hipStream_t st, const g1a* tab, uint8_t* out, uint32_t n);
void launch_pk_validate(hipStream_t st, const uint8_t* in, uint32_t n, int32_t* codes);
void launch_hash_maps(hipStream_t st, const dev_batch& b, const dev_work& w);
void launch_prep(hipStream_t st, const dev_batch& b, const dev_work& w);
void launch_stage(hipStream_t st, int stage, const dev_batch& b, const dev_work& w);
void launch_miller(hipStream_t st, const dev_batch& b, const dev_work& w);
void launch_lines(hipStream_t st, const dev_batch& b, const dev_work& w);
void launch_miller_steps(hipStream_t st, const dev_batch& b, const dev_work& w);
inline uint32_t miller_items_bound(const dev_batch& b, uint32_t per) { return b.n_sets / per + b.n_jobs; }
void launch_miller_duo(hipStream_t st, const dev_batch& b, const dev_work& w);
void launch_miller_quad(hipStream_t st, const dev_batch& b, const dev_work& w);
void launch_sig_check(hipStream_t st, const dev_batch& b, const dev_work& w);
void launch_sig_fixup(hipStream_t st, const dev_batch& b, const dev_work& w);
void launch_sig_split_coop(hipStream_t st, const dev_batch& b, const dev_work& w);
void launch_hash_clear_coop(hipStream_t st, const dev_batch& b, const dev_work& w);
void launch_hash_clear_trio(hipStream_t st, const dev_batch& b, const dev_work& w);
void launch_s_level_coop(hipStream_t st, const dev_batch& b, const dev_work& w, uint32_t s);
void launch_msm_job_coop(hipStream_t st, const dev_batch& b, const dev_work& w);
void launch_pk_coop(hipStream_t st, const dev_batch& b, const dev_work& w);
void launch_miller_kv(hipStream_t st, const dev_batch& b, const dev_work& w);
void launch_fp12_tail(hipStream_t st, int stage, const dev_batch& b, const dev_work& w);
void launch_combine_final(hipStream_t st, const fp12_t* parts, uint32_t n, uint32_t* flag);
void launch_final_exp_many(hipStream_t st, const fp12_t* in, fp12_t* out, uint32_t n);
void launch_export_g1a(hipStream_t st, const g1a* in, uint8_t* out96, uint32_t n);
void launch_export_g2a(hipStream_t st, const g2a* in, uint8_t* out192, uint32_t n);
void launch_fp12_convert(hipStream_t st, const fp12_t* in, fp12_t* out, uint32_t n, bool to_mont);
void launch_gen_keys(hipStream_t st, g1a* table, uint32_t* sk, uint32_t first, uint32_t n, uint64_t seed);
void launch_gen_sign(hipStream_t st, const dev_batch& b, const uint32_t* sk, uint8_t* out);
void launch_fp_ops(hipStream_t st, const fp_t* ab, fp_t* out, uint32_t n);
void launch_g2_decode_dbg(hipStream_t st, const uint8_t* sigs192, const uint32_t* sig_len, uint8_t* out192, int32_t* codes,
                         uint32_t n);
void launch_bench_fpmul(hipStream_t st, fp_t* io, uint32_t lanes, uint32_t iters);
void launch_gen_scalars(hipStream_t st, const uint32_t key[8], const uint32_t nonce[3], uint64_t* out, uint32_t n);
void launch_bench_mad(hipStream_t st, uint64_t* io, uint32_t lanes, uint32_t iters);

enum : int32_t {
  C_SEG_DEAD = 10,
  C_SEG_RETRY = 11,
};
struct sm_view {
  uint32_t n_sets, n_segs, n_groups, n_raw, table_n;
  const uint32_t* seg_off;
  const uint32_t* seg_group;
  const uint32_t* pk_idx;
  const g1a* raw_pks;
  const g1a* table;
  const uint64_t* scalars;
  const int32_t* sig_code;
  const uint32_t* sig_inf;
  uint32_t* skip;
  int32_t* set_code;
  g1j* win;
  g1a* p_seg;
  int32_t* seg_code;
  const g2a* h_group;
  g2a* h_seg;
  int32_t* pk_code_v;
  int32_t* job_code_v;
  const g2a* s_seg;
  const uint32_t* s_inf;
  const g1j* pk_set;
  const int32_t* pk_set_code;
};
struct sm_retry {
  uint32_t n;
  const uint32_t* list;
  const uint32_t* list_group;
  const uint32_t* pk_idx;
  const uint8_t* msgs;
  const uint8_t* sigs;
  const uint32_t* sig_len;
  const uint64_t* scalars;
  uint32_t* o_iota;
  uint32_t* o_idx;
  uint8_t* o_msgs;
  uint8_t* o_sigs;
  uint32_t* o_len;
  uint64_t* o_scalars;
};
void launch_sm_classify(hipStream_t st, const sm_view& v);
void launch_sm_g1_sum(hipStream_t st, const sm_view& v);
void launch_sm_apply(hipStream_t st, const sm_view& v);
void launch_sm_group_sums(hipStream_t st, const sm_view& v, const uint32_t* group_seg, g1a* p_group, g2a* s_group);
void launch_sm_retry_gather(hipStream_t st, const sm_retry& r);
void launch_sma_set_sum(hipStream_t st, const dev_batch& b, const dev_work& w, g1j* pk_set, int32_t* pk_set_code);
void launch_sma_classify(hipStream_t st, const sm_view& v);
void launch_sma_g1_sum(hipStream_t st, const sm_view& v);
void launch_sma_pk_aff(hipStream_t st, const g1j* pk_set, g1a* out, uint32_t n);
void launch_sma_retry_gather(hipStream_t st, const sm_retry& r, const g1j* pk_set, g1a* o_pk);
struct sig_agg_view;
void launch_sm_sig_agg(hipStream_t st, const sig_agg_view& v);

struct bits_args {
  uint32_t n_sets;
  const bits_src* src;
  bits_view v;
  uint32_t* pk_off;
  uint32_t* pk_idx;
  uint32_t cap;
  pk_window* win;
  uint32_t* tally;
};
void launch_bits_count(hipStream_t st, const bits_args& a);
void launch_bits_expand(hipStream_t st, const bits_args& a);
// ... 29 lines not shown
```

### lodestar_amd/csrc/bgv_kernels.hip

```cpp
#ifndef BGV_FPMUL_CALL
#define BGV_FPMUL_CALL 1
#endif
#ifndef BGV_FP2_INLINE
#define BGV_FP2_INLINE 1
#endif
#ifndef BGV_FP6_INLINE
#define BGV_FP6_INLINE 1
#endif
#ifndef BGV_POINT_INLINE
#define BGV_POINT_INLINE 1
#endif
#ifndef BGV_MILLER_WAVES
#define BGV_MILLER_WAVES 1
#endif
#ifndef BGV_MILLER_LDS_F
#define BGV_MILLER_LDS_F 1
#endif
#ifndef BGV_KERNELS_FP2_LEAF
#define BGV_KERNELS_FP2_LEAF 0
#endif
#ifndef BGV_FP2_LEAF
#define BGV_FP2_LEAF BGV_KERNELS_FP2_LEAF
#endif
#include "bgv_internal.h"
// ... 131 lines not shown
  int32_t code;
  if (len == 96u) code = g2_decompress(a, inf, s);
  else if (len == 192u) code = g2_deserialize(a, inf, s);
  else code = C_INVALID_SIZE;
  if (code == C_OK && !inf && !(b.defer_grp && i >= b.defer_from)) {
    g2j j;
    jac_from_aff(j, a);
    if (!g2_in_subgroup(j)) code = C_POINT_NOT_IN_GROUP;
  }
  if (code != C_OK || inf) { a.x = fp2_zero(); a.y = fp2_zero(); }
  w.sig_aff[i] = a;
  w.sig_inf[i] = inf ? 1u : 0u;
  w.sig_code[i] = code;
}

__global__ void __launch_bounds__(64, BGV_SIG_WAVES) k_sig_dec(dev_batch b, dev_work w) {
  const uint32_t i = gtid();
  if (i >= b.n_sets) return;
  const uint32_t len = b.sig_len[i];
  const uint8_t* s = b.sigs + 192u * i;
  g2a a;
  bool inf = false;
  int32_t code;
  if (len == 96u) code = g2_decompress(a, inf, s);
  else if (len == 192u) code = g2_deserialize(a, inf, s);
  else code = C_INVALID_SIZE;
  if (code != C_OK || inf) { a.x = fp2_zero(); a.y = fp2_zero(); }
  w.sig_aff[i] = a;
  w.sig_inf[i] = inf ? 1u : 0u;
  w.sig_code[i] = code;
}

__global__ void __launch_bounds__(64, BGV_SIG_WAVES) k_sig_split(dev_batch b, dev_work w) {
  const uint32_t nb = (b.n_sets + 63u) / 64u;
  const bool check = blockIdx.x < nb;
  const uint32_t i = (check ? blockIdx.x : blockIdx.x - nb) * 64u + threadIdx.x + (check && b.defer_grp ? b.defer_from : 0u);
  if (i >= b.n_sets) return;
  const bool live = w.sig_code[i] == C_OK && !w.sig_inf[i];
  if (check) {
    uint32_t ok = 1u;
    if (live) {
      g2j j;
      jac_from_aff(j, w.sig_aff[i]);
      ok = g2_in_subgroup(j) ? 1u : 0u;
    }
    w.sig_grp[i] = ok;
  } else {
    g2j r;
    if (!live) {
      jac_set_inf(r);
    } else {
      g2j s;
      jac_from_aff(s, w.sig_aff[i]);
      jac_mul_u64_w4(r, s, b.scalars[i]);
    }
    w.rsig[i] = r;
  }
}

__global__ void BGV_BULK k_sig_fix(dev_batch b, dev_work w) {
  const uint32_t i = gtid();
  if (i >= b.n_sets || (b.defer_grp && i < b.defer_from)) return;
  if (w.sig_code[i] == C_OK && !w.sig_grp[i]) {
    w.sig_code[i] = C_POINT_NOT_IN_GROUP;
    g2a z;
    z.x = fp2_zero();
    z.y = fp2_zero();
    w.sig_aff[i] = z;
  }
}

__global__ void BGV_BULK k_job_recode(dev_batch b, dev_work w) {
  const uint32_t j = gtid();
  if (j >= b.n_jobs) return;
  const int32_t was = w.job_code[j];
  const uint32_t beg = b.job_off[j], end = b.job_off[j + 1];
  int32_t code = C_OK;
  for (uint32_t i = beg; i < end && code == C_OK; i++) code = w.sig_code[i];
  for (uint32_t i = beg; i < end && code == C_OK; i++) code = w.pk_code[i];
  if (end == beg) code = C_EMPTY_JOB;
  if (code == was) return;
  w.job_code[j] = code;
  if (was != C_OK) return;
  g2a z;
  z.x = fp2_zero();
  z.y = fp2_zero();
  w.s_aff[j] = z;
  w.s_inf[j] = 1u;
  fp12_t one;
  fp12_one(one);
  w.f_set[b.n_sets + j] = one;
}

#ifndef BGV_COOP_G2
#define BGV_COOP_G2 1
#endif
#ifndef BGV_MSM_JOB_COOP
#define BGV_MSM_JOB_COOP 1
#endif
#ifndef BGV_PK_COOP
#define BGV_PK_COOP 1
#endif
#ifndef PK_COOP_MAX
#define PK_COOP_MAX 9000u
#endif
#ifndef BGV_MSM_JOB_COOP_BULK
#define BGV_MSM_JOB_COOP_BULK 0
#endif

__global__ void __launch_bounds__(64, BGV_HASH_WAVES) k_hash_map(dev_batch b, dev_work w) {
  const uint32_t t = gtid();
  if (t >= 2u * b.n_sets) return;
  const uint32_t i = t >> 1;
  uint8_t m[32];
#pragma unroll
  for (int k = 0; k < 32; k++) m[k] = b.msgs[32u * i + k];
  g2j q;
  hash_to_g2_map(q, m, t & 1u);
  w.q_part[t] = q;
}

__global__ void __launch_bounds__(64, BGV_HASH_WAVES) k_hash_clear(dev_batch b, dev_work w) {
  const uint32_t i = gtid();
  if (i >= b.n_sets) return;
  g2j h;
  hash_to_g2_finish(h, w.q_part[2u * i], w.q_part[2u * i + 1u]);
  g2a ha;
  jac_to_aff(ha, h);
  w.h_aff[i] = ha;
}

__global__ void __launch_bounds__(64, BGV_HASH_WAVES) k_hash(dev_batch b, dev_work w) {
  const uint32_t i = gtid();
  if (i >= b.n_sets) return;
  uint8_t m[32];
#pragma unroll
  for (int k = 0; k < 32; k++) m[k] = b.msgs[32u * i + k];
  g2j h;
  hash_to_g2(h, m);
  g2a ha;
  jac_to_aff(ha, h);
  w.h_aff[i] = ha;
}


__global__ void BGV_BULK k_chunk_count(dev_batch b, dev_work w) {
  const uint32_t i = gtid();
  if (i >= b.n_sets) return;
  const uint32_t lo = b.pk_off[i], hi = b.pk_off[i + 1];
  const uint32_t k = hi > lo ? hi - lo : 0u;
  const uint32_t wnd = b.win && hi >= lo && b.win[i].hi ? 1u : 0u;
  w.chunk_off[i] = (k + PK_CHUNK - 1) / PK_CHUNK + wnd;
}

__global__ void __launch_bounds__(1024) k_scan(uint32_t* a, uint32_t n) {
  __shared__ uint32_t wsum[16];
  const uint32_t t = threadIdx.x, lane = t & 63u, wid = t >> 6;
  uint32_t carry = 0;
  for (uint32_t base = 0; base < n; base += 1024u) {
    const uint32_t i = base + t;
    const uint32_t v = i < n ? a[i] : 0u;
    uint32_t x = v;
#pragma unroll
    for (uint32_t d = 1; d < 64; d <<= 1) {
      const uint32_t y = __shfl_up(x, d, 64);
      if (lane >= d) x += y;
// ... 16 lines not shown
  }
  if (t == 0) a[n] = carry;
}

__global__ void BGV_BULK k_chunk_set(dev_batch b, dev_work w) {
  const uint32_t i = gtid();
  if (i >= b.n_sets) return;
  const uint32_t end = min(w.chunk_off[i + 1], b.chunk_bound);
  for (uint32_t c = w.chunk_off[i]; c < end; c++) w.chunk_set[c] = i;
}


__global__ void __launch_bounds__(64, BGV_PK_WAVES) k_pk(dev_batch b, dev_work w) {
  const uint32_t i = gtid();
  if (i >= b.n_sets) return;
  g1j acc;
  jac_set_inf(acc);
  const uint32_t c0 = w.chunk_off[i], c1 = w.chunk_off[i + 1];
  bool range_err = c1 > b.chunk_bound || b.pk_off[i + 1] < b.pk_off[i];
  for (uint32_t c = c0; c < c1 && !range_err; c++) {
    const g1j p = w.pk_part[c];
    if (!jac_is_inf(p) && fp_is_zero(p.x)) range_err = true;
    jac_add(acc, acc, p);
  }
  int32_t code = C_OK;
  if (range_err) code = C_INDEX_RANGE;
  else if (jac_is_inf(acc)) code = C_PK_IS_INFINITY;
  g1a out;
  if (w.pk_agg) {
    if (code != C_OK || !jac_to_aff(out, acc)) { fp_set_zero(out.x); fp_set_zero(out.y); }
    w.pk_agg[i] = out;
  }
  if (code == C_OK) {
    g1j rp;
    jac_mul_u64_w4(rp, acc, b.scalars[i]);
    jac_to_aff(out, rp);
  } else {
    fp_set_zero(out.x);
    fp_set_zero(out.y);
  }
  w.rpk_aff[i] = out;
  w.pk_code[i] = code;
}

__global__ void __launch_bounds__(64, BGV_SCALE_WAVES) k_sig_scale(dev_batch b, dev_work w) {
  const uint32_t i = gtid();
  if (i >= b.n_sets) return;
  g2j r;
  if (w.sig_code[i] != C_OK || w.sig_inf[i]) {
    jac_set_inf(r);
  } else {
    g2j s;
    jac_from_aff(s, w.sig_aff[i]);
    jac_mul_u64_w4(r, s, b.scalars[i]);
  }
  w.rsig[i] = r;
}


__global__ void BGV_BULK k_msm_bucket(dev_batch b, dev_work w) {
  const uint32_t t = gtid();
  if (t >= b.n_jobs * 16u) return;
  const uint32_t j = t >> 4, win = t & 15u;
  g2j* bk = w.msm_bucket + (size_t)t * 15u;
  uint32_t mask = 0;
  for (uint32_t i = b.job_off[j]; i < b.job_off[j + 1]; i++) {
    if (w.sig_code[i] != C_OK || w.sig_inf[i]) continue;
    const uint32_t d = (uint32_t)(b.scalars[i] >> (4u * win)) & 15u;
    if (d == 0) continue;
    const g2a s = w.sig_aff[i];
    g2j acc;
    if ((mask >> d) & 1u) {
      acc = bk[d - 1];
      jac_add_aff(acc, acc, s);
    } else {
      jac_from_aff(acc, s);
      mask |= 1u << d;
    }
    bk[d - 1] = acc;
  }
  w.msm_mask[t] = mask;
}

__global__ void BGV_BULK k_msm_window(dev_batch b, dev_work w) {
  const uint32_t t = gtid();
  if (t >= b.n_jobs * 16u) return;
  const g2j* bk = w.msm_bucket + (size_t)t * 15u;
  const uint32_t mask = w.msm_mask[t];
  g2j run, tot;
  jac_set_inf(run);
  jac_set_inf(tot);
  for (uint32_t d = 15; d >= 1; d--) {
    if ((mask >> d) & 1u) {
      const g2j v = bk[d - 1];
      jac_add(run, run, v);
    }
    jac_add(tot, tot, run);
  }
  w.msm_win[t] = tot;
}

__device__ __forceinline__ void shfl_down16(g2j& r, const g2j& v, uint32_t st) {
  const uint32_t* src = (const uint32_t*)&v;
  uint32_t* dst = (uint32_t*)&r;
#pragma unroll
  for (int k = 0; k < (int)(sizeof(g2j) / 4); k++) dst[k] = (uint32_t)__shfl_down((int)src[k], st, 16);
}

__global__ void BGV_BULK k_msm_digit(dev_batch b, dev_work w) {
  const uint32_t t = gtid();
  const uint32_t j = t >> 8, win = (t >> 4) & 15u, d = t & 15u;
  if (j >= b.n_jobs) return;
  const uint32_t beg = b.job_off[j], end = b.job_off[j + 1];
  g2j acc;
  jac_set_inf(acc);
  bool first = true;
  uint32_t i = beg;
  for (;;) {
    while (i < end) {
      const bool live = w.sig_code[i] == C_OK && !w.sig_inf[i];
      const uint32_t dig = (uint32_t)(b.scalars[i] >> (4u * win)) & 15u;
      if (live && d != 0 && dig == d) break;
      i++;
    }
    if (!__any(i < end)) break;
    if (i < end) {
      const g2a s = w.sig_aff[i];
      if (first) jac_from_aff(acc, s);
      else jac_add_aff(acc, acc, s);
      first = false;
      i++;
    }
  }
  const g2j base = acc;
  for (int bit = 2; bit >= 0; bit--) {
    if (d >> (bit + 1)) {
      jac_dbl(acc, acc);
      if ((d >> bit) & 1u) jac_add(acc, acc, base);
    }
  }
  for (uint32_t st = 8; st >= 1; st >>= 1) {
    g2j o;
    shfl_down16(o, acc, st);
    if (d < st) jac_add(acc, acc, o);
  }
  if (d == 0) w.msm_win[16u * j + win] = acc;
}

__global__ void BGV_BULK k_msm_job(dev_batch b, dev_work w) {
  const uint32_t t = gtid();
  const uint32_t j = t >> 4, win = t & 15u;
  if (j >= b.n_jobs) return;
  const uint32_t beg = b.job_off[j], end = b.job_off[j + 1];
  int32_t code = C_OK;
  for (uint32_t i = beg; i < end && code == C_OK; i++) code = w.sig_code[i];
  for (uint32_t i = beg; i < end && code == C_OK; i++) code = w.pk_code[i];
  if (end == beg) code = C_EMPTY_JOB;
  g2j s;
  jac_set_inf(s);
  if (code == C_OK) {
    s = w.msm_win[16u * j + win];
    for (uint32_t k = 0; k < 4u * win; k++) jac_dbl(s, s);
  }
  for (uint32_t st = 8; st >= 1; st >>= 1) {
    g2j o;
    shfl_down16(o, s, st);
    if (win < st) jac_add(s, s, o);
  }
  if (win != 0) return;
  g2a sa;
  sa.x = fp2_zero();
  sa.y = fp2_zero();
  uint32_t inf = 1;
  if (code == C_OK) inf = jac_to_aff(sa, s) ? 0u : 1u;
  w.s_aff[j] = sa;
  w.s_inf[j] = inf;
  w.job_code[j] = code;
}

constexpr uint32_t MSM_LANES = 256;
__global__ void __launch_bounds__(MSM_LANES, 1) k_msm_fused(dev_batch b, dev_work w, uint32_t chunk) {
  __shared__ g2j pts[128];
  extern __shared__ g2a sg[];
  __shared__ uint8_t order[16][256];
  __shared__ uint32_t cnt[16][16], start[16][17];
  const uint32_t j = blockIdx.x, tid = threadIdx.x, win = tid >> 4, dig = tid & 15u;
  const uint32_t beg = b.job_off[j], end = b.job_off[j + 1];
  g2j acc;
  jac_set_inf(acc);
  bool first = true;
  for (uint32_t c0 = beg; c0 < end; c0 += chunk) {
    const uint32_t n = min(end - c0, chunk);
    cnt[win][dig] = 0u;
    __syncthreads();
    const bool live = tid < n && w.sig_code[c0 + tid] == C_OK && !w.sig_inf[c0 + tid];
    const uint64_t r = tid < n ? b.scalars[c0 + tid] : 0ull;
    if (live) sg[tid] = w.sig_aff[c0 + tid];
    if (live)
      for (uint32_t ww = 0; ww < 16; ww++) atomicAdd(&cnt[ww][(uint32_t)(r >> (4u * ww)) & 15u], 1u);
    __syncthreads();
    if (dig == 0) {
      uint32_t a = 0;
      for (uint32_t d = 0; d < 16; d++) { start[win][d] = a; a += cnt[win][d]; }
      start[win][16] = a;
    }
    __syncthreads();
    cnt[win][dig] = 0u;
    __syncthreads();
    if (live)
      for (uint32_t ww = 0; ww < 16; ww++) {
        const uint32_t d = (uint32_t)(r >> (4u * ww)) & 15u;
        order[ww][start[ww][d] + atomicAdd(&cnt[ww][d], 1u)] = (uint8_t)tid;
      }
    __syncthreads();
    if (dig != 0) {
      const uint32_t k0 = start[win][dig], k1 = start[win][dig + 1];
      for (uint32_t k = k0; k < k1; k++) {
        const g2a s = sg[order[win][k]];
        if (first) jac_from_aff(acc, s);
        else jac_add_aff(acc, acc, s);
        first = false;
      }
    }
    __syncthreads();
  }
  if (dig > 1 && !jac_is_inf(acc)) {
    const g2j base = acc;
    const int top = 31 - __clz((int)dig);
    for (int bit = top - 1; bit >= 0; bit--) {
      jac_dbl(acc, acc);
      if ((dig >> bit) & 1u) jac_add(acc, acc, base);
    }
  }
  for (uint32_t st = 8; st >= 1; st >>= 1) {
    if (dig >= st && dig < 2u * st) pts[8u * win + dig - st] = acc;
    __syncthreads();
    if (dig < st) {
      g2j o = pts[8u * win + dig];
      jac_add(acc, acc, o);
    }
    __syncthreads();
  }
  if (dig == 0)
    for (uint32_t k = 0; k < 4u * win; k++) jac_dbl(acc, acc);
  for (uint32_t st = 8; st >= 1; st >>= 1) {
    if (dig == 0 && win >= st && win < 2u * st) pts[win - st] = acc;
    __syncthreads();
    if (dig == 0 && win < st) {
      g2j o = pts[win];
      jac_add(acc, acc, o);
    }
    __syncthreads();
  }
  if (tid == 0) {
    g2a sa;
    if (!jac_to_aff(sa, acc)) { sa.x = fp2_zero(); sa.y = fp2_zero(); }
    w.s_aff[j] = sa;
    w.s_inf[j] = jac_is_inf(acc) ? 1u : 0u;
  }
}

__global__ void BGV_BULK k_job_code(dev_batch b, dev_work w) {
  const uint32_t j = gtid();
  if (j >= b.n_jobs) return;
  const uint32_t beg = b.job_off[j], end = b.job_off[j + 1];
  int32_t code = C_OK;
  for (uint32_t i = beg; i < end && code == C_OK; i++) code = w.sig_code[i];
  for (uint32_t i = beg; i < end && code == C_OK; i++) code = w.pk_code[i];
  if (end == beg) code = C_EMPTY_JOB;
  w.job_code[j] = code;
  if (code != C_OK) {
    g2a z;
    z.x = fp2_zero();
    z.y = fp2_zero();
    w.s_aff[j] = z;
    w.s_inf[j] = 1u;
  }
}

__global__ void BGV_BULK k_set_job(dev_batch b, dev_work w) {
  const uint32_t j = gtid();
  if (j >= b.n_jobs) return;
  for (uint32_t i = b.job_off[j]; i < b.job_off[j + 1]; i++) w.set_job[i] = j;
}

constexpr uint32_t S_COOP_MAX = 16384;
__global__ void BGV_BULK k_s_level(dev_batch b, dev_work w, uint32_t s) {
  const uint32_t i = gtid();
  if (i >= b.n_sets) return;
  const uint32_t j = w.set_job[i];
  const uint32_t beg = b.job_off[j], end = b.job_off[j + 1];
  if (((i - beg) % (2 * s)) != 0 || i + s >= end) return;
  g2j a = w.rsig[i];
  const g2j c = w.rsig[i + s];
  jac_add(a, a, c);
  w.rsig[i] = a;
}

__global__ void BGV_BULK k_job_s(dev_batch b, dev_work w, uint32_t span) {
  const uint32_t j = gtid();
  if (j >= b.n_jobs) return;
  const uint32_t beg = b.job_off[j], end = b.job_off[j + 1];
  int32_t code = C_OK;
  for (uint32_t i = beg; i < end && code == C_OK; i++) code = w.sig_code[i];
  for (uint32_t i = beg; i < end && code == C_OK; i++) code = w.pk_code[i];
  if (end == beg) code = C_EMPTY_JOB;
  g2a sa;
  sa.x = fp2_zero();
  sa.y = fp2_zero();
  uint32_t inf = 1;
  if (code == C_OK) {
    g2j s = w.rsig[beg];
    for (uint32_t i = beg + span; i < end; i += span) {
      const g2j r = w.rsig[i];
      jac_add(s, s, r);
    }
    inf = jac_to_aff(sa, s) ? 0u : 1u;
  }
  w.s_aff[j] = sa;
  w.s_inf[j] = inf;
  w.job_code[j] = code;
}

__global__ void BGV_BULK k_item_count(dev_batch b, dev_work w) {
  const uint32_t j = gtid();
  if (j >= b.n_jobs) return;
  const uint32_t lo = b.job_off[j], hi = b.job_off[j + 1];
  w.item_off[j] = hi > lo ? miller_item_count(hi - lo, b.steps_slice ? b.steps_slice : b.pairs_per_item) : 0u;
}

__global__ void BGV_BULK k_item_job(dev_batch b, dev_work w) {
  const uint32_t j = gtid();
  if (j >= b.n_jobs) return;
  for (uint32_t t = w.item_off[j]; t < w.item_off[j + 1]; t++) w.item_job[t] = j;
}


template <int SUB, int HALF>
__global__ void __launch_bounds__(64, BGV_WAVES) k_miller_coop(dev_batch b, dev_work w, uint32_t first, uint32_t count) {
  using cfg = coop_cfg<SUB, HALF>;
  __shared__ coop_grp_t<SUB, HALF> sm[cfg::GROUPS];
  const uint32_t lane = threadIdx.x, grp = lane / cfg::LANES;
  const uint32_t r = lane % cfg::LANES;
  const uint32_t k = r / (SUB * HALF), h = (r / SUB) % HALF, q = r % SUB;
  const uint32_t t = first + blockIdx.x * cfg::GROUPS + grp;
  const bool in_range = grp < cfg::GROUPS && t < first + count;
  bool active = in_range;
  if (in_range) {
    g1a P;
    g2a Q;
    if (t < b.n_sets) {
      active = w.pk_code[t] == C_OK;
      P = w.rpk_aff[t];
      Q = w.h_aff[t];
    } else {
      const uint32_t j = t - b.n_sets;
      active = w.job_code[j] == C_OK && !w.s_inf[j];
      P.x = G1_X_MONT;
      P.y = G1_NEG_Y_MONT;
      Q = w.s_aff[j];
    }
    if (active && k == 0 && q == 0 && h == 0) {
      coop_grp_t<SUB, HALF>& g = sm[grp];
      g.T[0] = Q.x;
      g.T[1] = Q.y;
      g.T[2] = fp2_one();
      g.Q[0] = Q.x;
      g.Q[1] = Q.y;
      g.px.c0 = P.x;
      fp_set_zero(g.px.c1);
      g.py.c0 = P.y;
      fp_set_zero(g.py.c1);
    }
  }
  __syncthreads();
  coop_miller<SUB, HALF>(sm[grp < cfg::GROUPS ? grp : 0], k, h, q, active);
  if (in_range && q == 0 && h == 0) {
    fp2_t v;
    if (active) v = sm[grp].f[k];
    else v = k == 0 ? fp2_one() : fp2_zero();
    fp2_t* dst = reinterpret_cast<fp2_t*>(&w.f_set[t]) + (k & 1) * 3 + (k >> 1);
    *dst = v;
  }
}

struct chacha_key { uint32_t key[8], nonce[3]; };
__global__ void __launch_bounds__(64) k_gen_scalars(chacha_key k, uint64_t* out, uint32_t n) {
  const uint32_t i = gtid();
  if (i >= n) return;
  out[i] = batch_scalar(k.key, i, k.nonce);
}

__global__ void BGV_BULK k_set_codes(dev_batch b, dev_work w) {
  const uint32_t i = gtid();
  if (i >= b.n_sets) return;
  const int32_t c = w.sig_code[i];
  w.set_code[i] = c != C_OK ? c : w.pk_code[i];
}

__global__ void BGV_BULK k_fp12_convert(const fp12_t* in, fp12_t* out, uint32_t n, uint32_t to_mont) {
  const uint32_t i = gtid();
  if (i >= n) return;
  const fp_t* a = (const fp_t*)&in[i];
  fp_t* r = (fp_t*)&out[i];
  for (int k = 0; k < 12; k++) {
    fp_t t = a[k];
    if (to_mont) fp_to_mont(t, t);
    else fp_from_mont(t, t);
    r[k] = t;
  }
}

BGV_CONST uint32_t FR_R[8] = {0x00000001u, 0xffffffffu, 0xfffe5bfeu, 0x53bda402u,
                              0x09a1d805u, 0x3339d808u, 0x299d7d48u, 0x73eda753u};

BGV_HD bool u256_ge_r(const uint32_t a[8]) {
  for (int i = 7; i >= 0; i--) {
    if (a[i] > FR_R[i]) return true;
    if (a[i] < FR_R[i]) return false;
  }
  return true;
}

BGV_HD void u256_sub_r(uint32_t a[8]) {
  uint32_t borrow = 0;
  for (int i = 0; i < 8; i++) {
    uint64_t d = (uint64_t)a[i] - FR_R[i] - borrow;
    a[i] = (uint32_t)d;
    borrow = (uint32_t)(d >> 63);
  }
}

BGV_HD void fr_add(uint32_t a[8], const uint32_t b[8]) {
  uint32_t c = 0;
  for (int i = 0; i < 8; i++) {
    uint64_t s = (uint64_t)a[i] + b[i] + c;
    a[i] = (uint32_t)s;
    c = (uint32_t)(s >> 32);
  }
  if (u256_ge_r(a)) u256_sub_r(a);
// ... 104 lines not shown
  if (i >= n) return;
  const uint32_t len = sig_len[i];
  const uint8_t* s = sigs192 + 192u * i;
  g2a a;
  bool inf = false;
  int32_t code;
  if (len == 96u) code = g2_decompress(a, inf, s);
  else if (len == 192u) code = g2_deserialize(a, inf, s);
  else code = C_INVALID_SIZE;
  if (code != C_OK || inf) { a.x = fp2_zero(); a.y = fp2_zero(); }
  const fp_t* c[4] = {&a.x.c0, &a.x.c1, &a.y.c0, &a.y.c1};
  for (int k = 0; k < 4; k++) {
    fp_t t;
    fp_from_mont(t, *c[k]);
    fp_to_be48(out192 + 192u * i + 48 * k, t);
  }
  codes[i] = code;
}

__global__ void __launch_bounds__(256) k_bench_fpmul(fp_t* io, uint32_t iters) {
  const uint32_t i = gtid();
  fp_t x = io[2 * i], y = io[2 * i + 1];
  for (uint32_t k = 0; k < iters; k++) fp_mul(x, x, y);
  io[2 * i] = x;
}

__global__ void __launch_bounds__(256) k_bench_mad(uint64_t* io, uint32_t iters) {
  const uint32_t i = gtid();
  uint64_t a0 = io[i], a1 = a0 + 1, a2 = a0 + 2, a3 = a0 + 3, a4 = a0 + 4, a5 = a0 + 5, a6 = a0 + 6, a7 = a0 + 7;
  const uint32_t m = (uint32_t)a0 | 1u;
  for (uint32_t k = 0; k < iters; k++) {
    a0 = (uint64_t)(uint32_t)a0 * m + (a0 >> 32);
    a1 = (uint64_t)(uint32_t)a1 * m + (a1 >> 32);
    a2 = (uint64_t)(uint32_t)a2 * m + (a2 >> 32);
    a3 = (uint64_t)(uint32_t)a3 * m + (a3 >> 32);
    a4 = (uint64_t)(uint32_t)a4 * m + (a4 >> 32);
    a5 = (uint64_t)(uint32_t)a5 * m + (a5 >> 32);
    a6 = (uint64_t)(uint32_t)a6 * m + (a6 >> 32);
    a7 = (uint64_t)(uint32_t)a7 * m + (a7 >> 32);
  }
  io[i] = a0 ^ a1 ^ a2 ^ a3 ^ a4 ^ a5 ^ a6 ^ a7;
}

static inline dim3 grid64(uint32_t n) { return dim3((n + 63u) / 64u); }

#define BGV_LAUNCH(k, n, ...)                                                 \
  do {                                                                        \
    if ((n) > 0) hipLaunchKernelGGL(k, grid64(n), dim3(64), 0, st, __VA_ARGS__); \
  } while (0)

void launch_raw_pks(hipStream_t st, const uint8_t* raw, g1a* out, uint32_t n) { BGV_LAUNCH(k_raw_pks, n, raw, out, n); }
void launch_table_from_compressed(hipStream_t st, const uint8_t* in, g1a* out, uint32_t n, int32_t* codes) {
  BGV_LAUNCH(k_table_from_compressed, n, in, out, n, codes);
}
void launch_table_from_uncompressed(hipStream_t st, const uint8_t* in, g1a* out, uint32_t n, int32_t* codes) {
  BGV_LAUNCH(k_table_from_uncompressed, n, in, out, n, codes);
}
void launch_export_g1a(hipStream_t st, const g1a* in, uint8_t* out96, uint32_t n) { BGV_LAUNCH(k_export_g1a, n, in, out96, n); }
void launch_export_g2a(hipStream_t st, const g2a* in, uint8_t* out192, uint32_t n) { BGV_LAUNCH(k_export_g2a, n, in, out192, n); }
void launch_pk_validate(hipStream_t st, const uint8_t* in, uint32_t n, int32_t* codes) {
  BGV_LAUNCH(k_pk_validate, n, in, n, codes);
}
void launch_table_export(hipStream_t st, const g1a* tab, uint8_t* out, uint32_t n) {
  BGV_LAUNCH(k_table_export, n, tab, out, n);
}
void launch_hash_maps(hipStream_t st, const dev_batch& b, const dev_work& w) {
  BGV_LAUNCH(k_hash_map, 2u * b.n_sets, b, w);
}

void launch_scan(hipStream_t st, uint32_t* a, uint32_t n) { hipLaunchKernelGGL(k_scan, dim3(1), dim3(1024), 0, st, a, n); }

void launch_prep(hipStream_t st, const dev_batch& b, const dev_work& w) {
  BGV_LAUNCH(k_chunk_count, b.n_sets, b, w);
  if (b.n_sets) hipLaunchKernelGGL(k_scan, dim3(1), dim3(1024), 0, st, w.chunk_off, b.n_sets);
  BGV_LAUNCH(k_chunk_set, b.n_sets, b, w);
  if (!b.miller_coop || b.miller_kv) {
    BGV_LAUNCH(k_item_count, b.n_jobs, b, w);
    if (b.n_jobs) hipLaunchKernelGGL(k_scan, dim3(1), dim3(1024), 0, st, w.item_off, b.n_jobs);
    BGV_LAUNCH(k_item_job, b.n_jobs, b, w);
  }
}

static void launch_miller_coop(hipStream_t st, uint32_t lanes, const dev_batch& b, const dev_work& w, uint32_t first,
                               uint32_t count) {
  if (!count) return;
  if (lanes == 6) {
    constexpr uint32_t G = coop_cfg<1, 1>::GROUPS;
    hipLaunchKernelGGL((k_miller_coop<1, 1>), dim3((count + G - 1) / G), dim3(64), 0, st, b, w, first, count);
  } else if (lanes == 18) {
    constexpr uint32_t G = coop_cfg<3, 1>::GROUPS;
    hipLaunchKernelGGL((k_miller_coop<3, 1>), dim3((count + G - 1) / G), dim3(64), 0, st, b, w, first, count);
  } else {
    constexpr uint32_t G = coop_cfg<3, 2>::GROUPS;
    hipLaunchKernelGGL((k_miller_coop<3, 2>), dim3((count + G - 1) / G), dim3(64), 0, st, b, w, first, count);
  }
}

void launch_sig_check(hipStream_t st, const dev_batch& b, const dev_work& w) {
  const uint32_t nd = (b.n_sets - b.defer_from + 63u) / 64u;
  if (nd) hipLaunchKernelGGL(k_sig_split, dim3(nd), dim3(64), 0, st, b, w);
}

void launch_sig_fixup(hipStream_t st, const dev_batch& b, const dev_work& w) {
  BGV_LAUNCH(k_sig_fix, b.n_sets, b, w);
  BGV_LAUNCH(k_job_recode, b.n_jobs, b, w);
}

void launch_stage(hipStream_t st, int stage, const dev_batch& b, const dev_work& w) {
  const uint32_t span = 1u << b.span_log2;
  switch (stage) {
    case ST_SIG:
      if (b.split && !b.msm) {
        BGV_LAUNCH(k_sig_dec, b.n_sets, b, w);
        if (b.n_sets) {
          if (BGV_COOP_G2)
            launch_sig_split_coop(st, b, w);
          else
            hipLaunchKernelGGL(k_sig_split, dim3(2u * ((b.n_sets + 63u) / 64u)), dim3(64), 0, st, b, w);
        }
        BGV_LAUNCH(k_sig_fix, b.n_sets, b, w);
      } else if (b.defer_grp && b.defer_from == 0) {
        BGV_LAUNCH(k_sig_dec, b.n_sets, b, w);
      } else {
        BGV_LAUNCH(k_sig, b.n_sets, b, w);
      }
      break;
    case ST_HASH:
      if (b.split) {
        if (!b.maps_early) BGV_LAUNCH(k_hash_map, 2u * b.n_sets, b, w);
        if (b.clear_lanes == 3) {
          launch_hash_clear_trio(st, b, w);
        } else if (BGV_COOP_G2 && b.clear_lanes != 1) {
          launch_hash_clear_coop(st, b, w);
        } else {
          BGV_LAUNCH(k_hash_clear, b.n_sets, b, w);
        }
      } else {
        BGV_LAUNCH(k_hash, b.n_sets, b, w);
      }
      break;
    case ST_PK:
      launch_pk_gather(st, b, w);
      break;
    case ST_PK_SCALE:
      if (b.split && BGV_PK_COOP && b.n_sets < PK_COOP_MAX) launch_pk_coop(st, b, w);
      else BGV_LAUNCH(k_pk, b.n_sets, b, w);
      break;
    case ST_SIG_SCALE:
      if (b.split && !b.msm) break;
      if (b.msm == 2) {
        BGV_LAUNCH(k_msm_bucket, b.n_jobs * 16u, b, w);
      } else if (b.msm == 4) {
        BGV_LAUNCH(k_msm_digit, b.n_jobs * 256u, b, w);
      } else if (b.msm == 1) {
        if (b.n_jobs) {
          const uint32_t chunk = 1u << min(b.span_log2, 8u);
          hipLaunchKernelGGL(k_msm_fused, dim3(b.n_jobs), dim3(MSM_LANES), chunk * sizeof(g2a), st, b, w, chunk);
        }
      } else {
        BGV_LAUNCH(k_sig_scale, b.n_sets, b, w);
      }
      break;
    case ST_S_TREE:
      BGV_LAUNCH(k_set_job, b.n_jobs, b, w);
      if (b.msm == 2 || b.msm == 4) {
        if (b.msm == 2) BGV_LAUNCH(k_msm_window, b.n_jobs * 16u, b, w);
        if ((b.msm == 4 && BGV_MSM_JOB_COOP) || (b.msm == 2 && BGV_MSM_JOB_COOP_BULK))
          launch_msm_job_coop(st, b, w);
        else
          BGV_LAUNCH(k_msm_job, b.n_jobs * 16u, b, w);
        break;
      }
      if (b.msm == 1) {
        BGV_LAUNCH(k_job_code, b.n_jobs, b, w);
        break;
      }
      for (uint32_t s = 1; s < span; s *= 2) {
        if (BGV_COOP_G2 && b.n_sets < S_COOP_MAX) launch_s_level_coop(st, b, w, s);
        else BGV_LAUNCH(k_s_level, b.n_sets, b, w, s);
      }
      BGV_LAUNCH(k_job_s, b.n_jobs, b, w, span);
      break;
    case ST_MILLER:
      if (b.miller_kv) {
        launch_miller_kv(st, b, w);
        break;
      }
      if (b.miller_coop == 2) {
        launch_miller_duo(st, b, w);
        break;
      }
      if (b.miller_coop == 4) {
        launch_miller_quad(st, b, w);
        break;
      }
      if (b.miller_coop) {
        if (b.n_sets)
          launch_miller_coop(st, b.miller_coop, b, w, 0u, b.n_sets);
        break;
      }
      if (b.steps_slice) launch_miller_steps(st, b, w);
      else launch_miller(st, b, w);
      break;
    case ST_MILLER_JOBS:
      if (b.n_jobs)
        launch_miller_coop(st, b.job_lanes, b, w, b.n_sets, b.n_jobs);
      break;
    case ST_F_TREE:
      launch_fp12_tail(st, stage, b, w);
      break;
    case ST_BATCH_PROD:
      launch_fp12_tail(st, stage, b, w);
      break;
    case ST_BATCH_FINAL:
    case ST_JOB_FINAL: launch_fp12_tail(st, stage, b, w); break;
    case ST_SET_CODES: BGV_LAUNCH(k_set_codes, b.n_sets, b, w); break;
    default: break;
  }
}

void launch_fp12_convert(hipStream_t st, const fp12_t* in, fp12_t* out, uint32_t n, bool to_mont) {
  BGV_LAUNCH(k_fp12_convert, n, in, out, n, to_mont ? 1u : 0u);
}
void launch_gen_scalars(hipStream_t st, const uint32_t key[8], const uint32_t nonce[3], uint64_t* out, uint32_t n) {
  chacha_key k;
  for (int i = 0; i < 8; i++) k.key[i] = key[i];
  for (int i = 0; i < 3; i++) k.nonce[i] = nonce[i];
  BGV_LAUNCH(k_gen_scalars, n, k, out, n);
}
void launch_gen_keys(hipStream_t st, g1a* table, uint32_t* sk, uint32_t first, uint32_t n, uint64_t seed) {
  BGV_LAUNCH(k_gen_keys, n, table, sk, first, n, seed);
}
void launch_gen_sign(hipStream_t st, const dev_batch& b, const uint32_t* sk, uint8_t* out) {
  BGV_LAUNCH(k_gen_sign, b.n_sets, b, sk, out);
}
void launch_g2_decode_dbg(hipStream_t st, const uint8_t* sigs192, const uint32_t* sig_len, uint8_t* out192, int32_t* codes,
                         uint32_t n) {
  BGV_LAUNCH(k_g2_decode_dbg, n, sigs192, sig_len, out192, codes, n);
}
void launch_fp_ops(hipStream_t st, const fp_t* ab, fp_t* out, uint32_t n) {
  if (n) hipLaunchKernelGGL(k_fp_ops, dim3((n + 63u) / 64u), dim3(64), 0, st, ab, out, n);
}
void launch_bench_fpmul(hipStream_t st, fp_t* io, uint32_t lanes, uint32_t iters) {
  hipLaunchKernelGGL(k_bench_fpmul, dim3(lanes / 256), dim3(256), 0, st, io, iters);
}
void launch_bench_mad(hipStream_t st, uint64_t* io, uint32_t lanes, uint32_t iters) {
  hipLaunchKernelGGL(k_bench_mad, dim3(lanes / 256), dim3(256), 0, st, io, iters);
}

}
```

### lodestar_amd/csrc/bgv_tail.hip

```cpp
#ifndef BGV_FPMUL_CALL
#define BGV_FPMUL_CALL 0
#endif
#include "bgv_internal.h"
#include "fp12_coop.h"

namespace bgv {

#ifndef BGV_TREE_WAVES
#define BGV_TREE_WAVES 2
#endif
#define BGV_TREE_LB __launch_bounds__(64, BGV_TREE_WAVES)

__device__ __forceinline__ static uint32_t tree_gtid() { return blockIdx.x * blockDim.x + threadIdx.x; }
#define gtid tree_gtid

__global__ void BGV_TREE_LB k_f_level(dev_batch b, dev_work w, uint32_t s) {
  const uint32_t i = gtid();
  if (i >= b.n_sets) return;
  const uint32_t j = w.set_job[i];
  const uint32_t beg = b.job_off[j], end = b.job_off[j + 1];
  if (((i - beg) % (2 * s)) != 0 || i + s >= end) return;
  fp12_t a = w.f_set[i];
  fp12_mul(a, a, w.f_set[i + s]);
  w.f_set[i] = a;
}

__global__ void BGV_TREE_LB k_job_f(dev_batch b, dev_work w, uint32_t span) {
  const uint32_t j = gtid();
  if (j >= b.n_jobs) return;
  const uint32_t beg = b.job_off[j], end = b.job_off[j + 1];
  fp12_t f;
  if (w.job_code[j] != C_OK) {
    fp12_one(f);
  } else {
    f = w.f_set[beg];
    for (uint32_t i = beg + span; i < end; i += span) fp12_mul(f, f, w.f_set[i]);
    fp12_mul(f, f, w.f_set[b.n_sets + j]);
  }
  w.f_job[j] = f;
  w.f_batch[j] = f;
}

#define COOP_LB __launch_bounds__(COOP_THREADS, 2)

__device__ __forceinline__ static uint32_t fold_step(const dev_batch& b) { return b.pairs_per_item ? b.pairs_per_item : 1u; }

__global__ void COOP_LB k_job_prefold(dev_batch b, dev_work w) {
  __shared__ cscratch s;
  __shared__ wfp12 acc, x;
  const uint32_t j = blockIdx.y, G = 1u << b.prefold_log2;
  const uint32_t beg = b.job_off[j], end = b.job_off[j + 1];
  const uint32_t g0 = beg + blockIdx.x * G;
  if (w.job_code[j] != C_OK || g0 + 1 >= end) return;
  const uint32_t g1 = min(end, g0 + G);
  c_load(&acc, w.f_set[g0]);
  for (uint32_t i = g0 + fold_step(b); i < g1; i += fold_step(b)) {
    c_load(&x, w.f_set[i]);
    c_mul(&acc, &acc, &x, &s);
  }
  c_store(w.f_set[g0], &acc);
}

__global__ void COOP_LB k_job_fold(dev_batch b, dev_work w, uint32_t stride) {
  __shared__ cscratch s;
  __shared__ wfp12 acc, x;
  const uint32_t j = blockIdx.x;
  const uint32_t beg = b.job_off[j], end = b.job_off[j + 1];
  if (w.job_code[j] != C_OK) {
    c_set_one(&acc);
  } else {
    c_load(&acc, w.f_set[b.n_sets + j]);
    for (uint32_t i = beg; i < end; i += stride) {
      c_load(&x, w.f_set[i]);
      c_mul(&acc, &acc, &x, &s);
    }
  }
  c_store(w.f_job[j], &acc);
  c_store(w.f_batch[j], &acc);
}

__global__ void COOP_LB k_job_chain(dev_batch b, dev_work w) {
  __shared__ cscratch s;
  __shared__ wfp12 acc, x, y;
  __shared__ uint32_t bad_pk;
  const uint32_t j = blockIdx.x;
  const uint32_t beg = b.job_off[j], end = b.job_off[j + 1];
  const uint32_t t0 = w.item_off[j], t1 = w.item_off[j + 1];
  const bool rejected = w.job_code[j] != C_OK;
  bool run = !rejected && t1 > t0;
  if (b.steps_dbg) {
    if (threadIdx.x == 0) bad_pk = 0u;
    __syncthreads();
    if (miller_job_rejected_pk(w.pk_code, beg, end, threadIdx.x, COOP_THREADS)) bad_pk = 1u;
    __syncthreads();
    run = t1 > t0 && !bad_pk;
  }
  if (!run) {
    c_set_one(&acc);
  } else {
    uint32_t k = 0;
    for (int bit = 62; bit >= 0; bit--) {
      const int sub = ((BLS_X_ABS >> bit) & 1ull) ? 2 : 1;
      for (int a = 0; a < sub; a++, k++) {
        c_load(&x, w.f_step[(size_t)t0 * MILLER_STEPS + k]);
        for (uint32_t t = t0 + 1; t < t1; t++) {
          c_load(&y, w.f_step[(size_t)t * MILLER_STEPS + k]);
          c_mul(&x, &x, &y, &s);
        }
        if (k == 0) {
          c_copy(&acc, &x);
        } else {
          if (a == 0) c_mul(&acc, &acc, &acc, &s);
          c_mul(&acc, &acc, &x, &s);
        }
      }
    }
    c_conj(&acc, &acc);
  }
  if (b.steps_dbg && end > beg) {
    c_store(w.f_set[beg], &acc);
    c_set_one(&y);
    for (uint32_t i = beg + 1; i < end; i++) c_store(w.f_set[i], &y);
  }
  if (rejected) {
    c_set_one(&acc);
  } else {
    c_load(&x, w.f_set[b.n_sets + j]);
    c_mul(&acc, &acc, &x, &s);
  }
  c_store(w.f_job[j], &acc);
  c_store(w.f_batch[j], &acc);
}

constexpr uint32_t FOLD_FAN = 8;
__global__ void COOP_LB k_fold(const fp12_t* src, uint32_t n, fp12_t* dst) {
  __shared__ cscratch s;
  __shared__ wfp12 acc, x;
  const uint32_t beg = blockIdx.x * FOLD_FAN, end = min(n, beg + FOLD_FAN);
  c_load(&acc, src[beg]);
  for (uint32_t i = beg + 1; i < end; i++) {
    c_load(&x, src[i]);
    c_mul(&acc, &acc, &x, &s);
  }
  c_store(dst[blockIdx.x], &acc);
}

__global__ void COOP_LB k_batch_final(dev_batch b, dev_work w) {
  __shared__ cscratch s;
  if (b.n_jobs == 0) {
    if (threadIdx.x == 0) w.flags[0] = 0u;
    return;
  }
  const bool one = c_final_exp_is_one(w.f_batch[0], &s);
  if (threadIdx.x == 0) w.flags[0] = one ? 1u : 0u;
}

__global__ void COOP_LB k_job_final(dev_batch b, dev_work w) {
  __shared__ cscratch s;
  const uint32_t j = blockIdx.x;
  const int32_t code = w.job_code[j];
  int32_t res;
  if (code != C_OK) {
    res = -code;
  } else if (w.flags[0]) {
    res = 1;
  } else {
    res = c_final_exp_is_one(w.f_job[j], &s) ? 1 : 0;
  }
  if (threadIdx.x == 0) w.job_result[j] = res;
}

__global__ void COOP_LB k_combine_final(const fp12_t* parts, uint32_t n, uint32_t* flag) {
  __shared__ cscratch s;
  __shared__ wfp12 acc, x;
  __shared__ fp12_t g;
  c_set_one(&acc);
  for (uint32_t k = 0; k < n; k++) {
    c_load(&x, parts[k]);
    c_mul(&acc, &acc, &x, &s);
  }
  c_store(g, &acc);
  const bool one = c_final_exp_is_one(g, &s);
  if (threadIdx.x == 0) flag[0] = one ? 1u : 0u;
}

__global__ void COOP_LB k_final_exp_many(const fp12_t* in, fp12_t* out) {
  __shared__ cscratch s;
  __shared__ fp12_t r;
  c_final_exp(&r, in[blockIdx.x], &s);
  if (threadIdx.x == 0) out[blockIdx.x] = r;
}

#undef gtid

void launch_fp12_tail(hipStream_t st, int stage, const dev_batch& b, const dev_work& w) {
  const uint32_t span = 1u << b.span_log2;
  auto grid = [](uint32_t n) { return dim3((n + 63u) / 64u); };
  const dim3 ct(COOP_THREADS);
  if (stage == ST_F_TREE) {
    if (!b.n_jobs) return;
    if (b.steps_slice) {
      hipLaunchKernelGGL(k_job_chain, dim3(b.n_jobs), ct, 0, st, b, w);
      return;
    }
    if (span <= 256) {
      uint32_t stride = b.pairs_per_item ? b.pairs_per_item : 1u;
      if (b.prefold_log2) {
        stride = 1u << b.prefold_log2;
        hipLaunchKernelGGL(k_job_prefold, dim3((span + stride - 1) / stride, b.n_jobs), ct, 0, st, b, w);
      }
      hipLaunchKernelGGL(k_job_fold, dim3(b.n_jobs), ct, 0, st, b, w, stride);
      return;
    }
    if (b.n_sets)
      for (uint32_t s = 1; s < span; s *= 2) hipLaunchKernelGGL(k_f_level, grid(b.n_sets), dim3(64), 0, st, b, w, s);
    hipLaunchKernelGGL(k_job_f, grid(b.n_jobs), dim3(64), 0, st, b, w, span);
  } else if (stage == ST_BATCH_PROD) {
    uint32_t n = b.n_jobs;
    fp12_t* src = w.f_batch;
    while (n > FOLD_FAN) {
      fp12_t* dst = src == w.f_batch ? w.f_tmp : w.f_batch;
      const uint32_t groups = (n + FOLD_FAN - 1) / FOLD_FAN;
      hipLaunchKernelGGL(k_fold, dim3(groups), ct, 0, st, src, n, dst);
      src = dst;
      n = groups;
    }
    if (n > 1 || (n == 1 && src != w.f_batch)) hipLaunchKernelGGL(k_fold, dim3(1), ct, 0, st, src, n, w.f_batch);
  } else if (stage == ST_BATCH_FINAL) {
    hipLaunchKernelGGL(k_batch_final, dim3(1), ct, 0, st, b, w);
  } else if (stage == ST_JOB_FINAL) {
    if (b.n_jobs) hipLaunchKernelGGL(k_job_final, dim3(b.n_jobs), ct, 0, st, b, w);
  }
}

void launch_final_exp_many(hipStream_t st, const fp12_t* in, fp12_t* out, uint32_t n) {
  if (n) hipLaunchKernelGGL(k_final_exp_many, dim3(n), dim3(COOP_THREADS), 0, st, in, out);
}

void launch_combine_final(hipStream_t st, const fp12_t* parts, uint32_t n, uint32_t* flag) {
  hipLaunchKernelGGL(k_combine_final, dim3(1), dim3(COOP_THREADS), 0, st, parts, n, flag);
}

}
```

### lodestar_amd/native.py

```python
from __future__ import annotations

import ctypes
import os
import threading

import numpy as np

HERE = os.path.dirname(os.path.abspath(__file__))
LIB_PATH = os.environ.get("BGV_LIB", os.path.join(HERE, "libbgv.so"))

BGV_OK = 0
BGV_E_INVALID_ARG = -1
BGV_E_HIP = -2
BGV_E_NO_DEVICE = -3
BGV_E_TABLE_RANGE = -4
BGV_E_EMPTY_SET = -5
BGV_E_BAD_PUBKEY = -6
BGV_E_STATE = -7
ABI_VERSION = 4

SET_CODE_NAMES = {
    0: "BLST_SUCCESS",
    1: "BLST_BAD_ENCODING",
    2: "BLST_POINT_NOT_ON_CURVE",
    3: "BLST_POINT_NOT_IN_GROUP",
    4: "BLST_AGGR_TYPE_MISMATCH",
    5: "BLST_VERIFY_FAIL",
    6: "BLST_PK_IS_INFINITY",
    7: "BLST_BAD_SCALAR",
    8: "BLST_INVALID_SIZE",
    9: "BGV_INDEX_RANGE",
    10: "EMPTY_SIGNATURE_SET",
}

PK_COMPRESSED_48 = 0
PK_UNCOMPRESSED_96 = 1
N_STAGES = 16

EXPORTS = [
    "bgv_abi_version", "bgv_build_id", "bgv_set_code_name", "bgv_stage_name", "bgv_last_error", "bgv_open", "bgv_open_cfg",
    "bgv_cfg_default", "bgv_close",
    "bgv_pubkeys_set", "bgv_pubkeys_count", "bgv_pubkeys_get", "bgv_pubkeys_validate", "bgv_verify", "bgv_last_stats",
    "bgv_partial", "bgv_partial_finish", "bgv_combine_final", "bgv_debug_stages", "bgv_gen_keys", "bgv_gen_sign", "bgv_bench_fpmul",
    "bgv_bench_mad", "bgv_debug_fp_ops", "bgv_debug_g2_decode",
    "bgv_verify_same_message", "bgv_sm_check", "bgv_debug_same_message",
    "bgv_verify_same_message_agg", "bgv_sma_check", "bgv_debug_same_message_agg",
    "bgv_index_list_set", "bgv_index_list_len", "bgv_verify_bits", "bgv_bits_check", "bgv_debug_bits_expand",
    "bgv_bits_expand_ms",
    "bgv_index_list_sums", "bgv_index_list_has_sums", "bgv_bits_path_stats", "bgv_bits_plan", "bgv_debug_bits_keys",
    "bgv_debug_index_list_sums", "bgv_index_list_sums_ms",
    "bgv_verify_same_message_bits", "bgv_smb_check", "bgv_debug_same_message_bits",
    "bgv_hash_stats", "bgv_miller_path_stats",
    "bgv_verify_same_message_aggregate", "bgv_sm_agg_check", "bgv_sm_agg_ms",
    "bgv_pair_merge", "bgv_pair_stats", "bgv_debug_pair_classes",
]
MAX_INDEX_LISTS = 8
SRC_EXPLICIT = 0xFFFFFFFF
SET_SRC_DTYPE = np.dtype([("list", "<u4"), ("off", "<u4"), ("len", "<u4"), ("bits_off", "<u4")])
FP_OPS_N = 13


class BgvNativeError(RuntimeError):
    def __init__(self, status: int, msg: str):
        super().__init__(f"bgv status {status}: {msg}")
        self.status = status


class BgvBatch(ctypes.Structure):
    _fields_ = [
        ("n_sets", ctypes.c_uint32),
        ("n_jobs", ctypes.c_uint32),
        ("job_offsets", ctypes.c_void_p),
        ("pk_offsets", ctypes.c_void_p),
        ("pk_indices", ctypes.c_void_p),
        ("raw_pks", ctypes.c_void_p),
        ("n_raw", ctypes.c_uint32),
        ("msgs", ctypes.c_void_p),
        ("sigs", ctypes.c_void_p),
        ("sig_len", ctypes.c_void_p),
        ("scalars", ctypes.c_void_p),
        ("on_device", ctypes.c_uint32),
    ]


class BgvStats(ctypes.Structure):
    _fields_ = [
        ("stage_ms", ctypes.c_float * N_STAGES),
        ("total_ms", ctypes.c_float),
        ("batch_retries", ctypes.c_uint32),
        ("batch_sigs_success", ctypes.c_uint32),
        ("n_sets", ctypes.c_uint32),
        ("n_jobs", ctypes.c_uint32),
        ("pubkeys_aggregated", ctypes.c_uint64),
        ("split", ctypes.c_uint32),
        ("miller_lanes", ctypes.c_uint32),
        ("pairs_per_item", ctypes.c_uint32),
        ("msm", ctypes.c_uint32),
        ("lines", ctypes.c_uint32),
        ("defer_from", ctypes.c_uint32),
        ("clear_lanes", ctypes.c_uint32),
        ("miller_kv", ctypes.c_uint32),
    ]
    LAYOUT = ("split", "miller_lanes", "pairs_per_item", "msm", "lines", "defer_from", "clear_lanes", "miller_kv")

    def as_dict(self, lib=None):
        names = [lib.stage_name(i) for i in range(N_STAGES)] if lib else [str(i) for i in range(N_STAGES)]
        return {
            "stage_ms": dict(zip(names, [float(x) for x in self.stage_ms])),
            "total_ms": float(self.total_ms),
            "batch_retries": int(self.batch_retries),
            "batch_sigs_success": int(self.batch_sigs_success),
            "n_sets": int(self.n_sets),
            "n_jobs": int(self.n_jobs),
            "pubkeys_aggregated": int(self.pubkeys_aggregated),
            "layout": self.layout(),
        }

    def layout(self) -> dict:
        return {k: int(getattr(self, k)) for k in self.LAYOUT}


class BgvSmBatch(ctypes.Structure):
    _fields_ = [
        ("n_sets", ctypes.c_uint32),
        ("n_groups", ctypes.c_uint32),
        ("group_offsets", ctypes.c_void_p),
        ("pk_indices", ctypes.c_void_p),
        ("raw_pks", ctypes.c_void_p),
        ("n_raw", ctypes.c_uint32),
        ("msgs", ctypes.c_void_p),
        ("sigs", ctypes.c_void_p),
        ("sig_len", ctypes.c_void_p),
        ("scalars", ctypes.c_void_p),
        ("on_device", ctypes.c_uint32),
    ]


# ... 38 lines not shown
    ]


class BgvSmbBatch(ctypes.Structure):
    _fields_ = [
        ("n_sets", ctypes.c_uint32),
        ("n_groups", ctypes.c_uint32),
        ("group_offsets", ctypes.c_void_p),
        ("src", ctypes.c_void_p),
        ("bits", ctypes.c_void_p),
        ("bits_len", ctypes.c_uint32),
        ("pk_indices", ctypes.c_void_p),
        ("n_indices", ctypes.c_uint32),
        ("raw_pks", ctypes.c_void_p),
        ("n_raw", ctypes.c_uint32),
        ("msgs", ctypes.c_void_p),
        ("sigs", ctypes.c_void_p),
        ("sig_len", ctypes.c_void_p),
        ("scalars", ctypes.c_void_p),
        ("on_device", ctypes.c_uint32),
    ]


class BgvSmStats(ctypes.Structure):
    _fields_ = [(k, ctypes.c_uint32) for k in
                ("n_sets", "n_groups", "n_segments", "hashes", "pairs", "groups_retried", "sets_retried")] + [
        ("total_ms", ctypes.c_float)]

    def as_dict(self) -> dict:
        return {k: (float(getattr(self, k)) if k == "total_ms" else int(getattr(self, k))) for k, _ in self._fields_}


class BgvCfg(ctypes.Structure):
    _fields_ = [("struct_size", ctypes.c_uint32)] + [
        (k, ctypes.c_int32) for k in
        ("split", "miller", "job_lanes", "msm", "pairs", "prefold", "lines", "defer_pct", "timing", "clear_lanes",
         "miller_kv", "cu_split", "miller_steps", "hash_dedup")]
    AUTO = {"split": -1, "miller": -1, "job_lanes": 0, "msm": -1, "pairs": 0, "prefold": -1, "lines": -1,
            "defer_pct": -1, "timing": -1, "clear_lanes": -1, "miller_kv": -1, "cu_split": 0, "miller_steps": -1,
            "hash_dedup": -1}

    @classmethod
    def make(cls, **over) -> "BgvCfg":
        bad = set(over) - set(cls.AUTO)
        if bad:
            raise ValueError(f"unknown bgv_cfg fields {sorted(bad)}")
        c = cls(struct_size=ctypes.sizeof(cls), **{**cls.AUTO, **over})
        return c


class BgvDebug(ctypes.Structure):
    _fields_ = [(k, ctypes.c_void_p) for k in
                ("sig_aff", "h_aff", "pk_agg", "rpk_aff", "s_aff", "pair_fe", "job_fe", "batch_fe")]


_lib = None
_lib_lock = threading.Lock()

ROOT = os.path.dirname(HERE)


def source_files(root: str = ROOT) -> list[str]:
    csrc = os.path.join(root, "lodestar_amd", "csrc")
    names = sorted(f for f in os.listdir(csrc) if f.endswith((".h", ".hip")))
    return [os.path.join("lodestar_amd", "csrc", f) for f in names] + [os.path.join("include", "bgv.h")]


class BgvBitsPath(ctypes.Structure):
    _fields_ = [("sets_complement", ctypes.c_uint32), ("keys_expanded", ctypes.c_uint32), ("keys_gathered", ctypes.c_uint32)]

    def as_dict(self) -> dict:
        return {k: int(getattr(self, k)) for k, _ in self._fields_}


class BgvHashPath(ctypes.Structure):
    _fields_ = [("sets", ctypes.c_uint32), ("hashes", ctypes.c_uint32), ("dedup", ctypes.c_uint32)]

    def as_dict(self) -> dict:
        return {k: int(getattr(self, k)) for k, _ in self._fields_}


class BgvMillerPath(ctypes.Structure):
    _fields_ = [("steps", ctypes.c_uint32), ("slice_sets", ctypes.c_uint32), ("items", ctypes.c_uint32)]

    def as_dict(self) -> dict:
        return {k: int(getattr(self, k)) for k, _ in self._fields_}


class BgvPairPath(ctypes.Structure):
    _fields_ = [("sets", ctypes.c_uint32), ("pairs", ctypes.c_uint32), ("merged", ctypes.c_uint32),
                ("fallback", ctypes.c_uint32)]

    def as_dict(self) -> dict:
        return {k: int(getattr(self, k)) for k, _ in self._fields_}


def source_hash(root: str = ROOT) -> str:
    import hashlib

    h = hashlib.sha256()
    for rel in source_files(root):
        with open(os.path.join(root, rel), "rb") as f:
            data = f.read()
        h.update(rel.replace(os.sep, "/").encode() + b"\0" + len(data).to_bytes(8, "little") + data)
    return h.hexdigest()


def check_build_id(lib_id: str, root: str = ROOT) -> None:
    try:
        want = source_hash(root)
    except OSError as e:
        import warnings
        warnings.warn(f"libbgv.so build id not checked: sources not readable ({e})", RuntimeWarning, stacklevel=2)
        return
    if lib_id != want and not lib_id.startswith(want + "+"):
        raise BgvNativeError(BGV_E_INVALID_ARG,
                             f"libbgv.so was built from other sources (id {lib_id[:16]}, tree {want[:16]}): "
                             "rebuild with __graft_entry__.build()")


def load_library(path: str = LIB_PATH) -> ctypes.CDLL:
    global _lib
    with _lib_lock:
        if _lib is not None:
            return _lib
        if not os.path.exists(path):
            raise BgvNativeError(BGV_E_NO_DEVICE, f"{path} not built (run __graft_entry__.build())")
        try:
            import torch
        except ImportError:
            pass
        try:
            lib = ctypes.CDLL(path)
            build_id_fn = lib.bgv_build_id
        except (OSError, AttributeError) as e:
            raise BgvNativeError(BGV_E_INVALID_ARG, f"{path}: not a loadable libbgv.so of this ABI ({e}): rebuild") from e
        build_id_fn.argtypes = []
        build_id_fn.restype = ctypes.c_char_p
        check_build_id(build_id_fn().decode())
        P = ctypes.c_void_p
        u32, i32, u64 = ctypes.c_uint32, ctypes.c_int32, ctypes.c_uint64
        sig = {
            "bgv_abi_version": ([], ctypes.c_int),
            "bgv_set_code_name": ([ctypes.c_int], ctypes.c_char_p),
            "bgv_stage_name": ([ctypes.c_int], ctypes.c_char_p),
            "bgv_last_error": ([], ctypes.c_char_p),
            "bgv_open": ([ctypes.c_int, ctypes.POINTER(P)], ctypes.c_int),
            "bgv_open_cfg": ([ctypes.c_int, ctypes.POINTER(BgvCfg), ctypes.POINTER(P)], ctypes.c_int),
            "bgv_cfg_default": ([ctypes.POINTER(BgvCfg)], None),
            "bgv_close": ([P], ctypes.c_int),
            "bgv_pubkeys_set": ([P, u32, u32, P, u32], ctypes.c_int),
            "bgv_pubkeys_count": ([P, ctypes.POINTER(u32)], ctypes.c_int),
            "bgv_pubkeys_get": ([P, u32, u32, P], ctypes.c_int),
            "bgv_pubkeys_validate": ([P, P, u32, P], ctypes.c_int),
            "bgv_verify": ([P, ctypes.POINTER(BgvBatch), P, P, ctypes.POINTER(BgvStats)], ctypes.c_int),
            "bgv_partial": ([P, ctypes.POINTER(BgvBatch), P, P, P, ctypes.POINTER(i32)], ctypes.c_int),
            "bgv_partial_finish": ([P, P, ctypes.POINTER(BgvStats)], ctypes.c_int),
            "bgv_last_stats": ([P, ctypes.POINTER(BgvStats)], ctypes.c_int),
            "bgv_debug_stages": ([P, ctypes.POINTER(BgvBatch), P, P, ctypes.POINTER(BgvDebug)], ctypes.c_int),
            "bgv_combine_final": ([P, P, u32, ctypes.POINTER(i32)], ctypes.c_int),
            "bgv_gen_keys": ([P, u32, u32, u64], ctypes.c_int),
            "bgv_gen_sign": ([P, ctypes.POINTER(BgvBatch), P], ctypes.c_int),
            "bgv_bench_fpmul": ([P, u32, u32, ctypes.POINTER(ctypes.c_float)], ctypes.c_int),
            "bgv_bench_mad": ([P, u32, u32, ctypes.POINTER(ctypes.c_float)], ctypes.c_int),
            "bgv_debug_fp_ops": ([P, P, u32, P], ctypes.c_int),
            "bgv_debug_g2_decode": ([P, P, P, u32, P, P], ctypes.c_int),
            "bgv_verify_same_message": ([P, ctypes.POINTER(BgvSmBatch), P, P, ctypes.POINTER(BgvSmStats)], ctypes.c_int),
            "bgv_sm_check": ([ctypes.POINTER(BgvSmBatch)], ctypes.c_int),
            "bgv_debug_same_message": ([P, ctypes.POINTER(BgvSmBatch), P, P, ctypes.POINTER(BgvSmStats), P, P, P], ctypes.c_int),
            "bgv_verify_same_message_agg": ([P, ctypes.POINTER(BgvSmaBatch), P, P, ctypes.POINTER(BgvSmStats)], ctypes.c_int),
            "bgv_sma_check": ([ctypes.POINTER(BgvSmaBatch)], ctypes.c_int),
            "bgv_debug_same_message_agg": ([P, ctypes.POINTER(BgvSmaBatch), P, P, ctypes.POINTER(BgvSmStats), P, P, P, P],
                                           ctypes.c_int),
            "bgv_index_list_set": ([P, u32, P, u32], ctypes.c_int),
            "bgv_index_list_len": ([P, u32, ctypes.POINTER(u32)], ctypes.c_int),
            "bgv_verify_bits": ([P, ctypes.POINTER(BgvBitsBatch), P, P, ctypes.POINTER(BgvStats)], ctypes.c_int),
            "bgv_bits_check": ([ctypes.POINTER(BgvBitsBatch), P], ctypes.c_int),
            "bgv_debug_bits_expand": ([P, ctypes.POINTER(BgvBitsBatch), P, P, u32, ctypes.POINTER(u32)], ctypes.c_int),
            "bgv_bits_expand_ms": ([P, ctypes.POINTER(ctypes.c_float)], ctypes.c_int),
            "bgv_index_list_sums": ([P, u32, u32], ctypes.c_int),
            "bgv_index_list_has_sums": ([P, u32, ctypes.POINTER(u32)], ctypes.c_int),
            "bgv_index_list_sums_ms": ([P, ctypes.POINTER(ctypes.c_float)], ctypes.c_int),
            "bgv_bits_path_stats": ([P, ctypes.POINTER(BgvBitsPath)], ctypes.c_int),
            "bgv_hash_stats": ([P, ctypes.POINTER(BgvHashPath)], ctypes.c_int),
            "bgv_miller_path_stats": ([P, ctypes.POINTER(BgvMillerPath)], ctypes.c_int),
            "bgv_pair_merge": ([P, ctypes.c_int32], ctypes.c_int),
            "bgv_pair_stats": ([P, ctypes.POINTER(BgvPairPath)], ctypes.c_int),
            "bgv_debug_pair_classes": ([P, ctypes.POINTER(BgvBatch), P, P, P, P, P, P, P], ctypes.c_int),
            "bgv_bits_plan": ([ctypes.POINTER(BgvBitsBatch), P, P, P, ctypes.POINTER(ctypes.c_uint64)], ctypes.c_int),
            "bgv_debug_bits_keys": ([P, ctypes.POINTER(BgvBitsBatch), P, P, P], ctypes.c_int),
            "bgv_debug_index_list_sums": ([P, u32, u32, u32, P], ctypes.c_int),
            "bgv_verify_same_message_bits": ([P, ctypes.POINTER(BgvSmbBatch), P, P, ctypes.POINTER(BgvSmStats)], ctypes.c_int),
            "bgv_smb_check": ([ctypes.POINTER(BgvSmbBatch), P], ctypes.c_int),
            "bgv_debug_same_message_bits": ([P, ctypes.POINTER(BgvSmbBatch), P, P, ctypes.POINTER(BgvSmStats), P, P, P, P, P],
                                            ctypes.c_int),
            "bgv_verify_same_message_aggregate": ([P, ctypes.POINTER(BgvSmBatch), ctypes.POINTER(BgvSmAgg), P, P,
                                                   ctypes.POINTER(BgvSmStats)], ctypes.c_int),
            "bgv_sm_agg_check": ([ctypes.POINTER(BgvSmBatch), ctypes.POINTER(BgvSmAgg)], ctypes.c_int),
            "bgv_sm_agg_ms": ([P, ctypes.POINTER(ctypes.c_float)], ctypes.c_int),
        }
        for name, (args, res) in sig.items():
            fn = getattr(lib, name)
            fn.argtypes = args
            fn.restype = res
        if lib.bgv_abi_version() != ABI_VERSION:
            raise BgvNativeError(BGV_E_INVALID_ARG, f"{path}: ABI {lib.bgv_abi_version()}, expected {ABI_VERSION} (rebuild)")
        _lib = lib
        return lib


def _ptr(a) -> int | None:
    if a is None:
        return None
    if isinstance(a, np.ndarray):
        return a.ctypes.data
    return int(a.data_ptr())


def _sync_producers(*objs) -> None:
    seen = set()
    for o in objs:
        vals = o.values() if isinstance(o, dict) else (o,)
        for a in vals:
            if a is None or isinstance(a, (np.ndarray, bytes, bytearray, int, float, str)):
                continue
            dev = getattr(a, "device", None)
            if dev is None or getattr(dev, "type", "") != "cuda":
                continue
            key = getattr(dev, "index", None)
            if key in seen:
                continue
            seen.add(key)
            import torch
            torch.cuda.current_stream(dev).synchronize()


G2_IDENTITY_96 = bytes([0xC0]) + bytes(95)


def sm_agg_check(arrays: dict, take=None, prev=None, on_device: bool = False, agg_sig=True) -> tuple[int, str]:
    lib = load_library()
    b = Device.make_sm_batch(arrays, on_device, sync_inputs=False)
    out = np.zeros((max(b.n_groups, 1), 96), np.uint8)
    a = BgvSmAgg(take=_ptr(take), prev_sig96=_ptr(prev), agg_sig96=out.ctypes.data if agg_sig else None)
    st = lib.bgv_sm_agg_check(ctypes.byref(b), ctypes.byref(a))
    return st, ("" if st == BGV_OK else lib.bgv_last_error().decode())


def sma_check(arrays: dict, on_device: bool = False) -> tuple[int, str]:
    lib = load_library()
    b = Device.make_sma_batch(arrays, on_device, sync_inputs=False)
    st = lib.bgv_sma_check(ctypes.byref(b))
    return st, ("" if st == BGV_OK else lib.bgv_last_error().decode())


def _count(a, width: int = 1) -> int:
    if a is None:
        return 0
    n = a.size if isinstance(a, np.ndarray) else a.numel()
    return int(n) // width


def make_bits_batch(arrays: dict, on_device: bool = False, sync_inputs: bool = True) -> BgvBitsBatch:
    b = BgvBitsBatch()
    b.n_sets = int(arrays["n_sets"])
    b.n_jobs = int(arrays["n_jobs"])
    b.job_offsets = _ptr(arrays["job_offsets"])
    b.src = _ptr(arrays["src"])
    b.bits = _ptr(arrays.get("bits"))
    b.bits_len = int(arrays["bits_len"]) if "bits_len" in arrays else _count(arrays.get("bits"))
# ... 248 lines not shown
        self._check(self.lib.bgv_verify_same_message_agg(self.h, ctypes.byref(b), ok.ctypes.data, sc.ctypes.data,
                                                         ctypes.byref(self.last_sm_stats)))
        return ok[: b.n_sets].astype(bool), sc[: b.n_sets]

    def debug_same_message_agg(self, arrays: dict, on_device: bool = False) -> dict:
        b = self.make_sma_batch(arrays, on_device)
        n, G = b.n_sets, b.n_groups
        ok = np.zeros(max(n, 1), dtype=np.uint8)
        sc = np.zeros(max(n, 1), dtype=np.int32)
        ps = np.zeros((max(n, 1), 96), np.uint8)
        pg = np.zeros((max(G, 1), 96), np.uint8)
        sg = np.zeros((max(G, 1), 192), np.uint8)
        hg = np.zeros((max(G, 1), 192), np.uint8)
        self.last_sm_stats = BgvSmStats()
        self._check(self.lib.bgv_debug_same_message_agg(self.h, ctypes.byref(b), ok.ctypes.data, sc.ctypes.data,
                                                        ctypes.byref(self.last_sm_stats), ps.ctypes.data, pg.ctypes.data,
                                                        sg.ctypes.data, hg.ctypes.data))
        return {"set_valid": ok[:n].astype(bool), "set_code": sc[:n], "pk_set": ps[:n], "p_group": pg[:G],
                "s_group": sg[:G], "h_group": hg[:G], "stats": self.last_sm_stats.as_dict()}

    make_smb_batch = staticmethod(make_smb_batch)

    def verify_same_message_bits(self, arrays: dict, on_device: bool = False, sync_inputs: bool = True):
        b = make_smb_batch(arrays, on_device, sync_inputs)
        ok = np.zeros(max(b.n_sets, 1), dtype=np.uint8)
        sc = np.zeros(max(b.n_sets, 1), dtype=np.int32)
        self.last_sm_stats = BgvSmStats()
        self._check(self.lib.bgv_verify_same_message_bits(self.h, ctypes.byref(b), ok.ctypes.data, sc.ctypes.data,
                                                          ctypes.byref(self.last_sm_stats)))
        return ok[: b.n_sets].astype(bool), sc[: b.n_sets]

    def debug_same_message_bits(self, arrays: dict, on_device: bool = False) -> dict:
        b = make_smb_batch(arrays, on_device)
        n, G = b.n_sets, b.n_groups
        ok = np.zeros(max(n, 1), dtype=np.uint8)
        sc = np.zeros(max(n, 1), dtype=np.int32)
        ps = np.zeros((max(n, 1), 96), np.uint8)
        path = np.zeros(max(n, 1), np.uint8)
        pg = np.zeros((max(G, 1), 96), np.uint8)
        sg = np.zeros((max(G, 1), 192), np.uint8)
        hg = np.zeros((max(G, 1), 192), np.uint8)
        self.last_sm_stats = BgvSmStats()
        self._check(self.lib.bgv_debug_same_message_bits(self.h, ctypes.byref(b), ok.ctypes.data, sc.ctypes.data,
                                                         ctypes.byref(self.last_sm_stats), ps.ctypes.data, path.ctypes.data,
                                                         pg.ctypes.data, sg.ctypes.data, hg.ctypes.data))
        return {"set_valid": ok[:n].astype(bool), "set_code": sc[:n], "pk_set": ps[:n], "path": path[:n], "p_group": pg[:G],
                "s_group": sg[:G], "h_group": hg[:G], "stats": self.last_sm_stats.as_dict()}

    def index_list_set(self, list_id: int, indices) -> None:
        arr = np.ascontiguousarray(indices, dtype=np.uint32)
        self._check(self.lib.bgv_index_list_set(self.h, list_id, arr.ctypes.data if arr.size else None, arr.size))

    def index_list_len(self, list_id: int) -> int:
        n = ctypes.c_uint32()
        self._check(self.lib.bgv_index_list_len(self.h, list_id, ctypes.byref(n)))
        return n.value

    def index_list_sums(self, list_id: int, enable: bool = True) -> None:
        self._check(self.lib.bgv_index_list_sums(self.h, list_id, 1 if enable else 0))

    def index_list_sums_ms(self) -> float:
        ms = ctypes.c_float()
        self._check(self.lib.bgv_index_list_sums_ms(self.h, ctypes.byref(ms)))
        return ms.value

    def index_list_has_sums(self, list_id: int) -> bool:
        has = ctypes.c_uint32()
        self._check(self.lib.bgv_index_list_has_sums(self.h, list_id, ctypes.byref(has)))
        return bool(has.value)

    def hash_stats(self) -> dict:
        out = BgvHashPath()
        self._check(self.lib.bgv_hash_stats(self.h, ctypes.byref(out)))
        return out.as_dict()

    def pair_merge(self, on) -> None:
        self._check(self.lib.bgv_pair_merge(self.h, int(on)))

    def pair_stats(self) -> dict:
        out = BgvPairPath()
        self._check(self.lib.bgv_pair_stats(self.h, ctypes.byref(out)))
        return out.as_dict()

    def debug_pair_classes(self, arrays: dict, on_device: bool = False) -> dict:
        b = self.make_batch(arrays, on_device)
        n, J = b.n_sets, b.n_jobs
        jr = np.zeros(max(J, 1), np.int32)
        sc = np.zeros(max(n, 1), np.int32)
        cls = np.zeros(max(n, 1), np.uint32)
        off = np.zeros(J + 1, np.uint32)
        pc = np.zeros((max(n, 1), 96), np.uint8)
        jfe = np.zeros((max(J, 1), 576), np.uint8)
        bfe = np.zeros(576, np.uint8)
        self._check(self.lib.bgv_debug_pair_classes(self.h, ctypes.byref(b), jr.ctypes.data, sc.ctypes.data, cls.ctypes.data,
                                                    off.ctypes.data, pc.ctypes.data, jfe.ctypes.data, bfe.ctypes.data))
        return {"job_result": jr[:J], "set_code": sc[:n], "cls": cls[:n], "class_off": off, "p_class": pc[: int(off[J])],
                "job_fe": jfe[:J], "batch_fe": bfe}

    def miller_path(self) -> dict:
        out = BgvMillerPath()
        self._check(self.lib.bgv_miller_path_stats(self.h, ctypes.byref(out)))
        return out.as_dict()

    def bits_path_stats(self) -> dict:
        out = BgvBitsPath()
        self._check(self.lib.bgv_bits_path_stats(self.h, ctypes.byref(out)))
        return out.as_dict()

    bits_plan = staticmethod(bits_plan)

    def debug_bits_keys(self, arrays: dict, on_device: bool = False):
        b = make_bits_batch(arrays, on_device)
        n = b.n_sets
        pk = np.zeros((max(n, 1), 96), np.uint8)
        path = np.zeros(max(n, 1), np.uint8)
        code = np.zeros(max(n, 1), np.int32)
        self._check(self.lib.bgv_debug_bits_keys(self.h, ctypes.byref(b), pk.ctypes.data, path.ctypes.data, code.ctypes.data))
        return pk[:n], path[:n], code[:n]

    def debug_index_list_sums(self, list_id: int, first: int, n: int) -> np.ndarray:
        out = np.zeros((max(n, 1), 96), np.uint8)
        self._check(self.lib.bgv_debug_index_list_sums(self.h, list_id, first, n, out.ctypes.data))
        return out[:n]

    make_bits_batch = staticmethod(make_bits_batch)

    def verify_bits(self, arrays: dict, on_device: bool = False, want_set_codes: bool = True, sync_inputs: bool = True):
        b = make_bits_batch(arrays, on_device, sync_inputs)
        jr = np.zeros(max(b.n_jobs, 1), dtype=np.int32)
        sc = np.zeros(max(b.n_sets, 1), dtype=np.int32) if want_set_codes else None
        self._check(self.lib.bgv_verify_bits(self.h, ctypes.byref(b), jr.ctypes.data,
                                             sc.ctypes.data if sc is not None else None, ctypes.byref(self.last_stats)))
        return jr[: b.n_jobs], (sc[: b.n_sets] if sc is not None else None)

    def debug_bits_expand(self, arrays: dict, on_device: bool = False, cap: int | None = None):
        b = make_bits_batch(arrays, on_device)
        po = np.zeros(b.n_sets + 1, np.uint32)
        total = ctypes.c_uint32()
        if cap is None:
            st = self.lib.bgv_debug_bits_expand(self.h, ctypes.byref(b), po.ctypes.data, None, 0, ctypes.byref(total))
            if st != BGV_OK and not (st == BGV_E_INVALID_ARG and total.value > 0):
                self._check(st)
            cap = total.value
        idx = np.zeros(max(cap, 1), np.uint32)
        self._check(self.lib.bgv_debug_bits_expand(self.h, ctypes.byref(b), po.ctypes.data, idx.ctypes.data, cap,
                                                   ctypes.byref(total)))
        return po, idx[: total.value]

    def bits_expand_ms(self) -> float:
        ms = ctypes.c_float()
        self._check(self.lib.bgv_bits_expand_ms(self.h, ctypes.byref(ms)))
        return ms.value

    def partial(self, arrays: dict, on_device: bool = False, sync_inputs: bool = True):
        b = self.make_batch(arrays, on_device, sync_inputs)
        out = np.zeros(576, dtype=np.uint8)
        sc = np.zeros(max(b.n_sets, 1), dtype=np.int32)
        jr = np.zeros(max(b.n_jobs, 1), dtype=np.int32)
        ok = ctypes.c_int32()
        self._check(self.lib.bgv_partial(self.h, ctypes.byref(b), out.ctypes.data, sc.ctypes.data, jr.ctypes.data,
                                         ctypes.byref(ok)))
        self._partial_jobs = b.n_jobs
        self._check(self.lib.bgv_last_stats(self.h, ctypes.byref(self.last_stats)))
        return out.tobytes(), sc[: b.n_sets], jr[: b.n_jobs], bool(ok.value)

    def partial_finish(self) -> np.ndarray:
# ... 61 lines not shown
```

Measured before the change: 3.408 million sets/s.

## Add batch-first tail: fold signature MSM windows and Miller steps across all jobs

Adds an optimistic batch tail mode. It sums the MSM windows of all jobs into one combined signature point and computes a single pairing term for it. It also multiplies the per-step Miller values of all items together before one shared squaring chain, so the per-job work (k_msm_job, per-job Miller, k_job_chain) is skipped when every job is valid. If the batch check fails, the per-job path is rerun under device flags, which adds cost on failing batches and makes the control flow more complex. The mode defaults to -1, which counts as enabled when the msm==2 and step-slice conditions hold.

```diff
diff --git a/include/bgv.h b/include/bgv.h
--- a/include/bgv.h
+++ b/include/bgv.h
@@ -229,6 +229,11 @@
   uint32_t sets, pairs, merged, fallback;
 } bgv_pair_path;
 int bgv_pair_stats(bgv_ctx* ctx, bgv_pair_path* out);
+int bgv_batch_tail(bgv_ctx* ctx, int32_t mode);
+typedef struct bgv_tail_path {
+  uint32_t batch_first, retried;
+} bgv_tail_path;
+int bgv_tail_stats(bgv_ctx* ctx, bgv_tail_path* out);
 int bgv_debug_pair_classes(bgv_ctx* ctx, const bgv_batch* batch, int32_t* job_result, int32_t* set_code, uint32_t* cls,
                            uint32_t* class_off, uint8_t* p_class96, uint8_t* job_fe, uint8_t* batch_fe);
 int bgv_bits_plan(const bgv_bits_batch* batch, const uint32_t* list_len, const uint8_t* list_has_sums,
diff --git a/lodestar_amd/csrc/batch_tail.h b/lodestar_amd/csrc/batch_tail.h
--- /dev/null
+++ b/lodestar_amd/csrc/batch_tail.h
@@ -0,0 +1,14 @@
+#pragma once
+#include <stddef.h>
+#include <stdint.h>
+
+namespace bgv {
+
+constexpr uint32_t FOLD_FAN = 8;
+constexpr uint32_t WIN_FAN = 4;
+
+constexpr uint32_t tail_groups(uint32_t n, uint32_t fan) { return (n + fan - 1u) / fan; }
+constexpr size_t tail_region1(uint32_t n, uint32_t fan) { return tail_groups(n, fan); }
+constexpr size_t tail_entries(uint32_t n, uint32_t fan) { return (size_t)tail_groups(n, fan) + tail_groups(tail_groups(n, fan), fan); }
+
+}
diff --git a/lodestar_amd/csrc/bgv_api.hip b/lodestar_amd/csrc/bgv_api.hip
--- a/lodestar_amd/csrc/bgv_api.hip
+++ b/lodestar_amd/csrc/bgv_api.hip
@@ -162,6 +162,12 @@
   bgv_pair_path pair_path = {};
   bool pair_pending = false;
   bool pair_redo = false;
+  int32_t batch_tail = -1;
+  dbuf<g2j> win_tmp;
+  dbuf<fp12_t> f_fold;
+  dev_batch tail_d = {};
+  dev_work tail_w = {};
+  bgv_tail_path tail_path = {};
   dbuf<fp_t> mb_fp;
   dbuf<uint64_t> mb_u64;
 };
@@ -343,6 +349,7 @@
   c->sma_pk.release(); c->sma_pk_code.release(); c->sma_aff.release();
   c->sag_seg.release(); c->sag_cnt.release(); c->sag_code.release(); c->sag_out.release(); c->sag_valid.release();
   c->sag_sig.release();
+  c->win_tmp.release(); c->f_fold.release();
   c->mb_fp.release(); c->mb_u64.release();
   (void)hipStreamDestroy(c->st);
   (void)hipStreamDestroy(c->st_hash);
@@ -753,9 +760,9 @@
   w.chunk_off = c->chunk_off.p; w.chunk_set = c->chunk_set.p; w.pk_part = c->pk_part.p;
   if ((r = c->sig_aff.ensure(ns)) || (r = c->h_aff.ensure(ns)) || (r = c->sig_inf.ensure(ns)) ||
       (r = c->sig_code.ensure(ns)) || (r = c->pk_code.ensure(ns)) || (r = c->rpk_aff.ensure(ns)) ||
-      (r = c->rsig.ensure(ns)) || (r = c->f_set.ensure(ns + nj)) || (r = c->set_code.ensure(ns)) ||
+      (r = c->rsig.ensure(ns)) || (r = c->f_set.ensure(ns + nj + 1)) || (r = c->set_code.ensure(ns)) ||
       (r = c->set_job.ensure(ns)) || (r = c->item_off.ensure(nj + 1)) || (r = c->item_job.ensure(ns + nj + 1)) || (r = c->f_job.ensure(nj)) || (r = c->f_batch.ensure(nj)) || (r = c->f_tmp.ensure(nj / 8 + 1)) ||
-      (r = c->s_aff.ensure(nj)) || (r = c->s_inf.ensure(nj)) || (r = c->job_code.ensure(nj)) ||
+      (r = c->s_aff.ensure(nj + 1)) || (r = c->s_inf.ensure(nj + 1)) || (r = c->job_code.ensure(nj)) ||
       (r = c->job_result.ensure(nj)) || (r = c->f_part.ensure(4)) || (r = c->flags.ensure(8)))
     return r;
   w.sig_aff = c->sig_aff.p; w.h_aff = c->h_aff.p; w.sig_inf = c->sig_inf.p; w.sig_code = c->sig_code.p;
@@ -821,6 +828,13 @@
     p.p_cls = c->pm_p.p; p.code_cls = c->pm_code.p; p.h_cls = c->pm_h.p;
     p.ident = c->flags.p + 1;
   }
+  w.win_tmp = nullptr; w.f_fold = nullptr;
+  if (d.batch_tail) {
+    if ((r = c->win_tmp.ensure(16 * tail_entries(J, WIN_FAN))) ||
+        (r = c->f_fold.ensure(tail_entries(miller_items_bound(d, d.steps_slice), FOLD_FAN) * MILLER_STEPS)))
+      return r;
+    w.win_tmp = c->win_tmp.p; w.f_fold = c->f_fold.p;
+  }
   w.msm_bucket = nullptr; w.msm_mask = nullptr; w.msm_win = nullptr;
   if (d.msm == 2) {
     if ((r = c->msm_bucket.ensure(nj * 16 * 15)) || (r = c->msm_mask.ensure(nj * 16)) || (r = c->msm_win.ensure(nj * 16))) return r;
@@ -861,6 +875,8 @@
     c->pair_pending = merge;
     c->pair_redo = false;
   }
+  c->tail_d = dv;
+  c->tail_w = wv;
   auto launch_one = [&](int s) -> int {
     hipStream_t st = c->st;
     if (s == ST_MILLER && d.lines) {
@@ -874,15 +890,21 @@
       if (s == ST_S_TREE || s == ST_MILLER) HIPCHK(hipStreamWaitEvent(st, dep[ST_PK_SCALE], 0));
       if (s == ST_F_TREE) HIPCHK(hipStreamWaitEvent(st, dep[ST_MILLER], 0));
     }
+
     if (s == ST_HASH && d.maps_early && st != c->st_hash) HIPCHK(hipStreamWaitEvent(st, c->ev_maps, 0));
     if (timed) HIPCHK(hipEventRecord(c->ev[s], st));
-    if (s == ST_F_TREE && d.defer_grp) {
+    if (s == ST_F_TREE && d.defer_grp && !d.batch_tail) {
       if (fork) HIPCHK(hipStreamWaitEvent(st, c->ev_grp, 0));
       launch_sig_fixup(st, d, w);
     }
     if (s == ST_HASH && classes) launch_hash_classes(st, c->mc);
-    else if (merge && (s == ST_MILLER || s == ST_F_TREE)) launch_stage(st, s, dv, wv);
+    else if (merge && (s == ST_MILLER || s == ST_F_TREE || (s == ST_BATCH_FINAL && d.batch_tail))) launch_stage(st, s, dv, wv);
     else launch_stage(st, s, d, w);
+    if (s == ST_MILLER_JOBS && d.defer_grp && d.batch_tail) {
+      if (fork) HIPCHK(hipStreamWaitEvent(st, c->ev_grp, 0));
+      launch_sig_fixup(st, d, w);
+      launch_batch_sig_redo(st, d, w);
+    }
     if (merge && s == ST_HASH) launch_pair_h(st, c->pc, w.h_aff);
     if (merge && s == ST_PK_SCALE) launch_pair_sum(st, c->pc, w.rpk_aff, w.pk_code);
     HIPCHK(hipGetLastError());
@@ -972,6 +994,7 @@
   c->staged_pending = false;
   uint32_t flag = 0;
   memcpy(&flag, c->pin_out, 4);
+  c->tail_path = {d.batch_tail ? 1u : 0u, d.batch_tail && d.n_jobs && !flag ? 1u : 0u};
   if (want_pair) {
     uint32_t ident = 0;
     memcpy(&c->pair_path.pairs, c->pin_out + 68, 4);
@@ -1040,6 +1063,10 @@
   return 0;
 }
 
+static void tail_entry(const bgv_ctx* c, dev_batch& d) {
+  d.batch_tail = c->batch_tail != 0 && d.steps_slice && d.msm == 2 && !d.steps_dbg && d.n_jobs ? 1u : 0u;
+}
+
 int bgv_verify(bgv_ctx* c, const bgv_batch* b, int32_t* job_result, int32_t* set_code, bgv_stats* stats) {
   if (!c || !b || (!job_result && b->n_jobs)) return fail(BGV_E_INVALID_ARG, "null argument");
   c->partial_pending = false;
@@ -1048,6 +1075,7 @@
   pair_entry pe(c, c->pair_merge != 0);
   dev_batch d;
   if (int r = prepare(c, b, d, true)) return r;
+  tail_entry(c, d);
   dev_work w;
   if (int r = work_alloc(c, d, w)) return r;
   return run_and_finish(c, d, w, job_result, set_code, stats);
@@ -1057,6 +1085,19 @@
   if (!c) return fail(BGV_E_INVALID_ARG, "null ctx");
   if (mode != 0 && mode != 1) return fail(BGV_E_INVALID_ARG, "bgv_pair_merge mode %d", mode);
   c->pair_merge = mode;
+  return BGV_OK;
+}
+
+int bgv_batch_tail(bgv_ctx* c, int32_t mode) {
+  if (!c) return fail(BGV_E_INVALID_ARG, "null ctx");
+  if (mode < -1 || mode > 1) return fail(BGV_E_INVALID_ARG, "bgv_batch_tail mode %d", mode);
+  c->batch_tail = mode;
+  return BGV_OK;
+}
+
+int bgv_tail_stats(bgv_ctx* c, bgv_tail_path* out) {
+  if (!c || !out) return fail(BGV_E_INVALID_ARG, "null argument");
+  *out = c->tail_path;
   return BGV_OK;
 }
 
@@ -1455,6 +1496,7 @@
   dev_batch d;
   if (int r = bits_front(c, b, d, true)) return r;
   if (int r = bits_layout(c, d, b->scalars, b->scalars && !b->on_device)) return r;
+  tail_entry(c, d);
   dev_work w;
   if (int r = work_alloc(c, d, w)) return r;
   return run_and_finish(c, d, w, job_result, set_code, stats);
@@ -2172,6 +2214,7 @@
   active_guard ag(c->device);
   dev_batch d;
   if (int r = prepare(c, b, d, true)) return r;
+  tail_entry(c, d);
   dev_work w;
   pair_entry pe(c, c->pair_merge != 0);
   if (int r = work_alloc(c, d, w)) return r;
@@ -2216,6 +2259,7 @@
   if (ok_out) *ok_out = ok;
   c->part_d = d;
   c->part_w = w;
+  c->tail_path = {d.batch_tail ? 1u : 0u, 0u};
   c->partial_pending = true;
   return BGV_OK;
 }
@@ -2232,7 +2276,8 @@
   c->run_from = 0;
   c->run_to = ST_COUNT;
   HIPCHK(hipEventRecord(c->ev[0], c->st));
-  launch_stage(c->st, ST_BATCH_FINAL, d, w);
+  if (d.batch_tail) launch_stage(c->st, ST_BATCH_FINAL, c->tail_d, c->tail_w);
+  else launch_stage(c->st, ST_BATCH_FINAL, d, w);
   launch_stage(c->st, ST_JOB_FINAL, d, w);
   HIPCHK(hipGetLastError());
   HIPCHK(hipEventRecord(c->ev[ST_COUNT], c->st));
diff --git a/lodestar_amd/csrc/bgv_internal.h b/lodestar_amd/csrc/bgv_internal.h
--- a/lodestar_amd/csrc/bgv_internal.h
+++ b/lodestar_amd/csrc/bgv_internal.h
@@ -2,6 +2,7 @@
 #include "pairing.h"
 #include "rng.h"
 #include "bits_expand.h"
+#include "batch_tail.h"
 
 namespace bgv {
 
@@ -33,6 +34,7 @@
   uint32_t defer_grp;
   uint32_t steps_slice;
   uint32_t steps_dbg;
+  uint32_t batch_tail;
   const uint32_t* job_off;
   const uint32_t* pk_off;
   const uint32_t* pk_idx;
@@ -65,10 +67,12 @@
   uint32_t* set_job;
   uint32_t* item_off;
   uint32_t* item_job;
+  g2j* win_tmp;
   g2a* s_aff;
   uint32_t* s_inf;
   fp2_t* lines;
   fp12_t* f_step;
+  fp12_t* f_fold;
   fp12_t* f_set;
   fp12_t* f_job;
   fp12_t* f_batch;
@@ -79,6 +83,7 @@
   fp12_t* f_part;
   uint32_t* flags;
 };
+constexpr uint32_t FLAG_CODES_KEPT = 2;
 
 enum Stage {
   ST_SIG = 0,
@@ -139,6 +144,8 @@
 void launch_pk_coop(hipStream_t st, const dev_batch& b, const dev_work& w);
 void launch_miller_kv(hipStream_t st, const dev_batch& b, const dev_work& w);
 void launch_fp12_tail(hipStream_t st, int stage, const dev_batch& b, const dev_work& w);
+void launch_batch_sig_redo(hipStream_t st, const dev_batch& b, const dev_work& w);
+void launch_job_chain_retry(hipStream_t st, const dev_batch& b, const dev_work& w);
 void launch_combine_final(hipStream_t st, const fp12_t* parts, uint32_t n, uint32_t* flag);
 void launch_final_exp_many(hipStream_t st, const fp12_t* in, fp12_t* out, uint32_t n);
 void launch_export_g1a(hipStream_t st, const g1a* in, uint8_t* out96, uint32_t n);
diff --git a/lodestar_amd/csrc/bgv_kernels.hip b/lodestar_amd/csrc/bgv_kernels.hip
--- a/lodestar_amd/csrc/bgv_kernels.hip
+++ b/lodestar_amd/csrc/bgv_kernels.hip
@@ -237,6 +237,7 @@
   if (code == was) return;
   w.job_code[j] = code;
   if (was != C_OK) return;
+  if (b.batch_tail) w.flags[FLAG_CODES_KEPT] = 0u;
   g2a z;
   z.x = fp2_zero();
   z.y = fp2_zero();
@@ -419,9 +420,30 @@
   w.msm_mask[t] = mask;
 }
 
+__device__ __forceinline__ void job_code16(const dev_batch& b, const dev_work& w, uint32_t j, uint32_t l) {
+  const uint32_t beg = b.job_off[j], end = b.job_off[j + 1];
+  uint32_t bad_sig = 0xffffffffu, bad_pk = 0xffffffffu;
+  for (uint32_t i = beg + l; i < end; i += 16u) {
+    if (bad_sig == 0xffffffffu && w.sig_code[i] != C_OK) bad_sig = i;
+    if (bad_pk == 0xffffffffu && w.pk_code[i] != C_OK) bad_pk = i;
+  }
+  for (uint32_t st = 8; st >= 1; st >>= 1) {
+    bad_sig = min(bad_sig, (uint32_t)__shfl_down((int)bad_sig, st, 16));
+    bad_pk = min(bad_pk, (uint32_t)__shfl_down((int)bad_pk, st, 16));
+  }
+  if (l != 0) return;
+  int32_t code = C_OK;
+  if (bad_sig != 0xffffffffu) code = w.sig_code[bad_sig];
+  else if (bad_pk != 0xffffffffu) code = w.pk_code[bad_pk];
+  if (end == beg) code = C_EMPTY_JOB;
+  w.job_code[j] = code;
+  if (j == 0) w.flags[FLAG_CODES_KEPT] = 1u;
+}
+
 __global__ void BGV_BULK k_msm_window(dev_batch b, dev_work w) {
   const uint32_t t = gtid();
   if (t >= b.n_jobs * 16u) return;
+  if (b.batch_tail) job_code16(b, w, t >> 4, t & 15u);
   const g2j* bk = w.msm_bucket + (size_t)t * 15u;
   const uint32_t mask = w.msm_mask[t];
   g2j run, tot;
@@ -484,21 +506,29 @@
   if (d == 0) w.msm_win[16u * j + win] = acc;
 }
 
-__global__ void BGV_BULK k_msm_job(dev_batch b, dev_work w) {
+enum : uint32_t { MSM_JOB_ALL = 0, MSM_JOB_HORNER = 1, MSM_JOB_BATCH = 2 };
+__global__ void BGV_BULK k_msm_job(dev_batch b, dev_work w, uint32_t mode, const g2j* win_src, const uint32_t* skip) {
+  if (skip && *skip) return;
   const uint32_t t = gtid();
-  const uint32_t j = t >> 4, win = t & 15u;
-  if (j >= b.n_jobs) return;
-  const uint32_t beg = b.job_off[j], end = b.job_off[j + 1];
+  uint32_t j = t >> 4;
+  const uint32_t win = t & 15u;
+  if (j >= (mode == MSM_JOB_BATCH ? 1u : b.n_jobs)) return;
   int32_t code = C_OK;
-  for (uint32_t i = beg; i < end && code == C_OK; i++) code = w.sig_code[i];
-  for (uint32_t i = beg; i < end && code == C_OK; i++) code = w.pk_code[i];
-  if (end == beg) code = C_EMPTY_JOB;
+  if (mode == MSM_JOB_ALL) {
+    const uint32_t beg = b.job_off[j], end = b.job_off[j + 1];
+    for (uint32_t i = beg; i < end && code == C_OK; i++) code = w.sig_code[i];
+    for (uint32_t i = beg; i < end && code == C_OK; i++) code = w.pk_code[i];
+    if (end == beg) code = C_EMPTY_JOB;
+  } else if (mode == MSM_JOB_HORNER) {
+    code = w.job_code[j];
+  }
   g2j s;
   jac_set_inf(s);
   if (code == C_OK) {
-    s = w.msm_win[16u * j + win];
+    s = mode == MSM_JOB_BATCH ? win_src[win] : w.msm_win[16u * j + win];
     for (uint32_t k = 0; k < 4u * win; k++) jac_dbl(s, s);
   }
+  if (mode == MSM_JOB_BATCH) j = b.n_jobs;
   for (uint32_t st = 8; st >= 1; st >>= 1) {
     g2j o;
     shfl_down16(o, s, st);
@@ -512,7 +542,23 @@
   if (code == C_OK) inf = jac_to_aff(sa, s) ? 0u : 1u;
   w.s_aff[j] = sa;
   w.s_inf[j] = inf;
-  w.job_code[j] = code;
+  if (mode == MSM_JOB_ALL) w.job_code[j] = code;
+}
+
+__global__ void BGV_BULK k_win_fold(dev_work w, const g2j* src, uint32_t n, g2j* dst, uint32_t level0, const uint32_t* skip) {
+  if (skip && *skip) return;
+  const uint32_t t = gtid();
+  const uint32_t g = t >> 4, win = t & 15u;
+  if (g >= (n + WIN_FAN - 1) / WIN_FAN) return;
+  const uint32_t end = min(n, WIN_FAN * g + WIN_FAN);
+  g2j acc;
+  jac_set_inf(acc);
+  for (uint32_t j = WIN_FAN * g; j < end; j++) {
+    if (level0 && w.job_code[j] != C_OK) continue;
+    const g2j v = src[16u * j + win];
+    jac_add(acc, acc, v);
+  }
+  dst[16u * g + win] = acc;
 }
 
 constexpr uint32_t MSM_LANES = 256;
@@ -674,8 +720,10 @@
 
 
 template <int SUB, int HALF>
-__global__ void __launch_bounds__(64, BGV_WAVES) k_miller_coop(dev_batch b, dev_work w, uint32_t first, uint32_t count) {
+__global__ void __launch_bounds__(64, BGV_WAVES) k_miller_coop(dev_batch b, dev_work w, uint32_t first, uint32_t count,
+                                                                      const uint32_t* skip) {
   using cfg = coop_cfg<SUB, HALF>;
+  if (skip && *skip) return;
   __shared__ coop_grp_t<SUB, HALF> sm[cfg::GROUPS];
   const uint32_t lane = threadIdx.x, grp = lane / cfg::LANES;
   const uint32_t r = lane % cfg::LANES;
@@ -692,7 +740,7 @@
       Q = w.h_aff[t];
     } else {
       const uint32_t j = t - b.n_sets;
-      active = w.job_code[j] == C_OK && !w.s_inf[j];
+      active = (j >= b.n_jobs || w.job_code[j] == C_OK) && !w.s_inf[j];
       P.x = G1_X_MONT;
       P.y = G1_NEG_Y_MONT;
       Q = w.s_aff[j];
@@ -963,17 +1011,17 @@
 }
 
 static void launch_miller_coop(hipStream_t st, uint32_t lanes, const dev_batch& b, const dev_work& w, uint32_t first,
-                               uint32_t count) {
+                               uint32_t count, const uint32_t* skip = nullptr) {
   if (!count) return;
   if (lanes == 6) {
     constexpr uint32_t G = coop_cfg<1, 1>::GROUPS;
-    hipLaunchKernelGGL((k_miller_coop<1, 1>), dim3((count + G - 1) / G), dim3(64), 0, st, b, w, first, count);
+    hipLaunchKernelGGL((k_miller_coop<1, 1>), dim3((count + G - 1) / G), dim3(64), 0, st, b, w, first, count, skip);
   } else if (lanes == 18) {
     constexpr uint32_t G = coop_cfg<3, 1>::GROUPS;
-    hipLaunchKernelGGL((k_miller_coop<3, 1>), dim3((count + G - 1) / G), dim3(64), 0, st, b, w, first, count);
+    hipLaunchKernelGGL((k_miller_coop<3, 1>), dim3((count + G - 1) / G), dim3(64), 0, st, b, w, first, count, skip);
   } else {
     constexpr uint32_t G = coop_cfg<3, 2>::GROUPS;
-    hipLaunchKernelGGL((k_miller_coop<3, 2>), dim3((count + G - 1) / G), dim3(64), 0, st, b, w, first, count);
+    hipLaunchKernelGGL((k_miller_coop<3, 2>), dim3((count + G - 1) / G), dim3(64), 0, st, b, w, first, count, skip);
   }
 }
 
@@ -985,6 +1033,27 @@
 void launch_sig_fixup(hipStream_t st, const dev_batch& b, const dev_work& w) {
   BGV_LAUNCH(k_sig_fix, b.n_sets, b, w);
   BGV_LAUNCH(k_job_recode, b.n_jobs, b, w);
+}
+
+static void launch_batch_sig(hipStream_t st, const dev_batch& b, const dev_work& w, const uint32_t* skip) {
+  if (!b.n_jobs) return;
+  g2j* reg[2] = {w.win_tmp, w.win_tmp + 16u * tail_region1(b.n_jobs, WIN_FAN)};
+  const g2j* src = w.msm_win;
+  uint32_t n = b.n_jobs, lvl = 0;
+  do {
+    const uint32_t groups = tail_groups(n, WIN_FAN);
+    g2j* dst = reg[lvl & 1u];
+    BGV_LAUNCH(k_win_fold, groups * 16u, w, src, n, dst, lvl == 0 ? 1u : 0u, skip);
+    src = dst;
+    n = groups;
+    lvl++;
+  } while (n > 1);
+  BGV_LAUNCH(k_msm_job, 16u, b, w, MSM_JOB_BATCH, src, skip);
+  launch_miller_coop(st, b.job_lanes, b, w, b.n_sets + b.n_jobs, 1u, skip);
+}
+
+void launch_batch_sig_redo(hipStream_t st, const dev_batch& b, const dev_work& w) {
+  launch_batch_sig(st, b, w, w.flags + FLAG_CODES_KEPT);
 }
 
 void launch_stage(hipStream_t st, int stage, const dev_batch& b, const dev_work& w) {
@@ -1048,8 +1117,8 @@
         if (b.msm == 2) BGV_LAUNCH(k_msm_window, b.n_jobs * 16u, b, w);
         if ((b.msm == 4 && BGV_MSM_JOB_COOP) || (b.msm == 2 && BGV_MSM_JOB_COOP_BULK))
           launch_msm_job_coop(st, b, w);
-        else
-          BGV_LAUNCH(k_msm_job, b.n_jobs * 16u, b, w);
+        else if (!b.batch_tail)
+          BGV_LAUNCH(k_msm_job, b.n_jobs * 16u, b, w, MSM_JOB_ALL, (const g2j*)nullptr, (const uint32_t*)nullptr);
         break;
       }
       if (b.msm == 1) {
@@ -1084,7 +1153,8 @@
       else launch_miller(st, b, w);
       break;
     case ST_MILLER_JOBS:
-      if (b.n_jobs)
+      if (b.batch_tail) launch_batch_sig(st, b, w, nullptr);
+      else if (b.n_jobs)
         launch_miller_coop(st, b.job_lanes, b, w, b.n_sets, b.n_jobs);
       break;
     case ST_F_TREE:
@@ -1094,6 +1164,13 @@
       launch_fp12_tail(st, stage, b, w);
       break;
     case ST_BATCH_FINAL:
+      launch_fp12_tail(st, stage, b, w);
+      if (b.batch_tail && b.n_jobs) {
+        BGV_LAUNCH(k_msm_job, b.n_jobs * 16u, b, w, MSM_JOB_HORNER, (const g2j*)nullptr, (const uint32_t*)w.flags);
+        launch_miller_coop(st, b.job_lanes, b, w, b.n_sets, b.n_jobs, w.flags);
+        launch_job_chain_retry(st, b, w);
+      }
+      break;
     case ST_JOB_FINAL: launch_fp12_tail(st, stage, b, w); break;
     case ST_SET_CODES: BGV_LAUNCH(k_set_codes, b.n_sets, b, w); break;
     default: break;
diff --git a/lodestar_amd/csrc/bgv_tail.hip b/lodestar_amd/csrc/bgv_tail.hip
--- a/lodestar_amd/csrc/bgv_tail.hip
+++ b/lodestar_amd/csrc/bgv_tail.hip
@@ -79,10 +79,11 @@
   c_store(w.f_batch[j], &acc);
 }
 
-__global__ void COOP_LB k_job_chain(dev_batch b, dev_work w) {
+__global__ void COOP_LB k_job_chain(dev_batch b, dev_work w, const uint32_t* skip) {
   __shared__ cscratch s;
   __shared__ wfp12 acc, x, y;
   __shared__ uint32_t bad_pk;
+  if (skip && *skip) return;
   const uint32_t j = blockIdx.x;
   const uint32_t beg = b.job_off[j], end = b.job_off[j + 1];
   const uint32_t t0 = w.item_off[j], t1 = w.item_off[j + 1];
@@ -132,7 +133,6 @@
   c_store(w.f_batch[j], &acc);
 }
 
-constexpr uint32_t FOLD_FAN = 8;
 __global__ void COOP_LB k_fold(const fp12_t* src, uint32_t n, fp12_t* dst) {
   __shared__ cscratch s;
   __shared__ wfp12 acc, x;
@@ -143,6 +143,49 @@
     c_mul(&acc, &acc, &x, &s);
   }
   c_store(dst[blockIdx.x], &acc);
+}
+
+__global__ void COOP_LB k_step_fold(dev_batch b, dev_work w, const fp12_t* src, uint32_t n, fp12_t* dst, uint32_t level0) {
+  __shared__ cscratch s;
+  __shared__ wfp12 acc, x;
+  const uint32_t g = blockIdx.x, k = blockIdx.y;
+  const uint32_t live = level0 ? min(n, w.item_off[b.n_jobs]) : n;
+  const uint32_t beg = g * FOLD_FAN, end = min(live, beg + FOLD_FAN);
+  bool have = false;
+  for (uint32_t t = beg; t < end; t++) {
+    if (level0 && w.job_code[w.item_job[t]] != C_OK) continue;
+    if (!have) {
+      c_load(&acc, src[(size_t)t * MILLER_STEPS + k]);
+      have = true;
+    } else {
+      c_load(&x, src[(size_t)t * MILLER_STEPS + k]);
+      c_mul(&acc, &acc, &x, &s);
+    }
+  }
+  if (!have) c_set_one(&acc);
+  c_store(dst[(size_t)g * MILLER_STEPS + k], &acc);
+}
+
+__global__ void COOP_LB k_batch_chain(dev_batch b, dev_work w, const fp12_t* steps) {
+  __shared__ cscratch s;
+  __shared__ wfp12 acc, x;
+  uint32_t k = 0;
+  for (int bit = 62; bit >= 0; bit--) {
+    const int sub = ((BLS_X_ABS >> bit) & 1ull) ? 2 : 1;
+    for (int a = 0; a < sub; a++, k++) {
+      c_load(&x, steps[k]);
+      if (k == 0) {
+        c_copy(&acc, &x);
+      } else {
+        if (a == 0) c_mul(&acc, &acc, &acc, &s);
+        c_mul(&acc, &acc, &x, &s);
+      }
+    }
+  }
+  c_conj(&acc, &acc);
+  c_load(&x, w.f_set[b.n_sets + b.n_jobs]);
+  c_mul(&acc, &acc, &x, &s);
+  c_store(w.f_batch[0], &acc);
 }
 
 __global__ void COOP_LB k_batch_final(dev_batch b, dev_work w) {
@@ -193,14 +236,38 @@
 
 #undef gtid
 
+static void launch_batch_chain(hipStream_t st, const dev_batch& b, const dev_work& w) {
+  const dim3 ct(COOP_THREADS);
+  uint32_t n = miller_items_bound(b, b.steps_slice), lvl = 0;
+  fp12_t* reg[2] = {w.f_fold, w.f_fold + tail_region1(n, FOLD_FAN) * MILLER_STEPS};
+  const fp12_t* src = w.f_step;
+  do {
+    const uint32_t groups = tail_groups(n, FOLD_FAN);
+    fp12_t* dst = reg[lvl & 1u];
+    hipLaunchKernelGGL(k_step_fold, dim3(groups, MILLER_STEPS), ct, 0, st, b, w, src, n, dst, lvl == 0 ? 1u : 0u);
+    src = dst;
+    n = groups;
+    lvl++;
+  } while (n > 1);
+  hipLaunchKernelGGL(k_batch_chain, dim3(1), ct, 0, st, b, w, src);
+}
+
+void launch_job_chain_retry(hipStream_t st, const dev_batch& b, const dev_work& w) {
+  if (b.n_jobs) hipLaunchKernelGGL(k_job_chain, dim3(b.n_jobs), dim3(COOP_THREADS), 0, st, b, w, (const uint32_t*)w.flags);
+}
+
 void launch_fp12_tail(hipStream_t st, int stage, const dev_batch& b, const dev_work& w) {
   const uint32_t span = 1u << b.span_log2;
   auto grid = [](uint32_t n) { return dim3((n + 63u) / 64u); };
   const dim3 ct(COOP_THREADS);
   if (stage == ST_F_TREE) {
     if (!b.n_jobs) return;
+    if (b.batch_tail) {
+      launch_batch_chain(st, b, w);
+      return;
+    }
     if (b.steps_slice) {
-      hipLaunchKernelGGL(k_job_chain, dim3(b.n_jobs), ct, 0, st, b, w);
+      hipLaunchKernelGGL(k_job_chain, dim3(b.n_jobs), ct, 0, st, b, w, (const uint32_t*)nullptr);
       return;
     }
     if (span <= 256) {
@@ -216,6 +283,7 @@
       for (uint32_t s = 1; s < span; s *= 2) hipLaunchKernelGGL(k_f_level, grid(b.n_sets), dim3(64), 0, st, b, w, s);
     hipLaunchKernelGGL(k_job_f, grid(b.n_jobs), dim3(64), 0, st, b, w, span);
   } else if (stage == ST_BATCH_PROD) {
+    if (b.batch_tail) return;
     uint32_t n = b.n_jobs;
     fp12_t* src = w.f_batch;
     while (n > FOLD_FAN) {
diff --git a/lodestar_amd/native.py b/lodestar_amd/native.py
--- a/lodestar_amd/native.py
+++ b/lodestar_amd/native.py
@@ -53,6 +53,7 @@
     "bgv_hash_stats", "bgv_miller_path_stats",
     "bgv_verify_same_message_aggregate", "bgv_sm_agg_check", "bgv_sm_agg_ms",
     "bgv_pair_merge", "bgv_pair_stats", "bgv_debug_pair_classes",
+    "bgv_batch_tail", "bgv_tail_stats",
 ]
 MAX_INDEX_LISTS = 8
 SRC_EXPLICIT = 0xFFFFFFFF
@@ -257,6 +258,13 @@
 
 class BgvMillerPath(ctypes.Structure):
     _fields_ = [("steps", ctypes.c_uint32), ("slice_sets", ctypes.c_uint32), ("items", ctypes.c_uint32)]
+
+    def as_dict(self) -> dict:
+        return {k: int(getattr(self, k)) for k, _ in self._fields_}
+
+
+class BgvTailPath(ctypes.Structure):
+    _fields_ = [("batch_first", ctypes.c_uint32), ("retried", ctypes.c_uint32)]
 
     def as_dict(self) -> dict:
         return {k: int(getattr(self, k)) for k, _ in self._fields_}
@@ -361,6 +369,8 @@
             "bgv_miller_path_stats": ([P, ctypes.POINTER(BgvMillerPath)], ctypes.c_int),
             "bgv_pair_merge": ([P, ctypes.c_int32], ctypes.c_int),
             "bgv_pair_stats": ([P, ctypes.POINTER(BgvPairPath)], ctypes.c_int),
+            "bgv_batch_tail": ([P, ctypes.c_int32], ctypes.c_int),
+            "bgv_tail_stats": ([P, ctypes.POINTER(BgvTailPath)], ctypes.c_int),
             "bgv_debug_pair_classes": ([P, ctypes.POINTER(BgvBatch), P, P, P, P, P, P, P], ctypes.c_int),
             "bgv_bits_plan": ([ctypes.POINTER(BgvBitsBatch), P, P, P, ctypes.POINTER(ctypes.c_uint64)], ctypes.c_int),
             "bgv_debug_bits_keys": ([P, ctypes.POINTER(BgvBitsBatch), P, P, P], ctypes.c_int),
@@ -775,6 +785,14 @@
         self._check(self.lib.bgv_pair_stats(self.h, ctypes.byref(out)))
         return out.as_dict()
 
+    def batch_tail(self, mode) -> None:
+        self._check(self.lib.bgv_batch_tail(self.h, int(mode)))
+
+    def tail_path(self) -> dict:
+        out = BgvTailPath()
+        self._check(self.lib.bgv_tail_stats(self.h, ctypes.byref(out)))
+        return out.as_dict()
+
     def debug_pair_classes(self, arrays: dict, on_device: bool = False) -> dict:
         b = self.make_batch(arrays, on_device)
         n, J = b.n_sets, b.n_jobs
```

Measured after the change: 3.581 million sets/s (median of 6 runs). 1.05x the previous value.
